# The-African-Research-Collective/karanta-ocr

Hardware: AMD Instinct MI355X
Metric: pages_per_sec (higher is better)
Workload: dtype bf16; 1 GPU; Qwen2-VL-2B bf16 greedy, batch=8 synthetic 1024x1024 pages per GPU, max_pixels=1003520 (grid 70x70, 1225 image tokens), prompt P=1394 tokens, T_out=1024 (ignore_eos), random-init weights; global_batch=8, parallelism=dp1, decode=hipGraph replay

## Files before the change

include/karanta_hip.h:

```cpp
#ifndef KARANTA_HIP_H
#define KARANTA_HIP_H

#include <stddef.h>
#include <stdint.h>

#ifdef __cplusplus
extern "C" {
#endif

typedef void* kr_stream;
typedef uint16_t kr_bf16;

#define KR_ABI_VERSION 412

#define KR_OK 0
#define KR_ERR_ARG (-1)
#define KR_ERR_HIP (-2)
#define KR_ERR_RCCL (-3)
#define KR_ERR_STATE (-4)

#define KR_EPI_NONE 0
#define KR_EPI_QUICK_GELU 1
#define KR_EPI_GELU_ERF 2
#define KR_EPI_SILU_MUL 3
#define KR_EPI_SILU_MUL8 4

int kr_version(void);
const char* kr_last_error(void);
int kr_device_info(int device, char* name64, int* compute_units, size_t* total_mem);
int kr_set_device(int device);
int kr_stream_synchronize(kr_stream s);
int kr_stream_create_cu_mask(kr_stream* out, int cus_enabled);
int kr_stream_create_cu_range(kr_stream* out, int first_cu, int n_cus);
int kr_stream_destroy(kr_stream s);

int kr_event_create(void** ev);
int kr_event_destroy(void* ev);
int kr_event_record(void* ev, kr_stream s);
int kr_stream_wait_event(kr_stream s, void* ev);
int kr_event_synchronize(void* ev);
int kr_event_elapsed_ms(void* start, void* stop, float* ms);

int kr_graph_begin_capture(kr_stream s);
int kr_graph_end_capture(kr_stream s, void** graph_exec);
int kr_graph_launch(void* graph_exec, kr_stream s);
int kr_graph_destroy(void* graph_exec);


int kr_cast_pad_f32_bf16(const float* src, kr_bf16* dst, int64_t rows, int k, int k_pad, kr_stream s);

int kr_layernorm(const kr_bf16* x, const kr_bf16* w, const kr_bf16* b, kr_bf16* y,
                 int64_t rows, int d, float eps, kr_stream s);

int kr_rmsnorm(const kr_bf16* x, int64_t ldx, const kr_bf16* w, kr_bf16* y,
               int64_t rows, int d, float eps, kr_stream s);


int kr_gemm_bf16(const kr_bf16* A, int64_t lda, const kr_bf16* W, const kr_bf16* bias,
                 const kr_bf16* residual, int64_t ldr, kr_bf16* C, int64_t ldc,
                 int64_t M, int N, int K, int epilogue, int w_packed, kr_stream s);

#define KR_GEMM_SCRATCH_BYTES ((size_t)512 * 65536)
int kr_gemm_bf16_ws(const kr_bf16* A, int64_t lda, const kr_bf16* W, const kr_bf16* bias,
                    const kr_bf16* residual, int64_t ldr, kr_bf16* C, int64_t ldc,
                    int64_t M, int N, int K, int epilogue, int w_packed, float* scratch, size_t scratch_bytes, kr_stream s);

int kr_gemm_fp8(const kr_bf16* A, int64_t lda, const uint8_t* w_packed_fp8, const float* w_scale, const kr_bf16* bias,
                const kr_bf16* residual, int64_t ldr, kr_bf16* C, int64_t ldc, int64_t M, int N, int K, int epilogue,
                kr_stream s);

int kr_quantize_rows_fp8(const kr_bf16* x, int64_t ldx, uint8_t* q, int64_t ldq, float* scale, int64_t rows, int K, kr_stream s);
int kr_gemm_fp8a(const uint8_t* A8, int64_t lda, const float* a_scale, const uint8_t* w_packed_fp8, const float* w_scale,
                 const kr_bf16* bias, const kr_bf16* residual, int64_t ldr, kr_bf16* C, int64_t ldc, int64_t M, int N, int K,
                 int epilogue, kr_stream s);

int kr_gemv_bf16(const kr_bf16* x, int64_t ldx, const kr_bf16* W, const kr_bf16* bias,
                 const kr_bf16* residual, int64_t ldr, kr_bf16* out, float* out_f32, int64_t ldc,
                 int M, int N, int K, int epilogue,
                 const kr_bf16* norm_w, float norm_eps, kr_stream s);


int kr_qkv_prep(const kr_bf16* qkv, int64_t ld_qkv, int q_off, int k_off, int v_off,
                const float* cos, const float* sin,
                const int32_t* blk_tok0, const int32_t* blk_ntok,
                const int64_t* blk_k_row0, const int64_t* blk_vt_blk, int n_blk,
                kr_bf16* q_out, int64_t q_head_stride, kr_bf16* k_out, int64_t k_head_stride,
                kr_bf16* vt_out, int64_t vt_head_stride, int q_heads, int kv_heads, int hd,
                kr_stream s);

int kr_rope2d_vision(kr_bf16* x, const float* cos, const float* sin, int64_t n, int heads, int hd,
                     int64_t row_stride, kr_stream s);

int kr_attn_varlen(const kr_bf16* q, const kr_bf16* k, const kr_bf16* vt, kr_bf16* out,
                   const int32_t* qblk, const int32_t* qblk_len, int n_qblk,
                   int64_t nq_total, int q_heads, int kv_heads, int hd,
                   int64_t k_head_stride, int64_t vt_head_stride, float scale, int causal,
                   kr_stream s);
int kr_attn_varlen_q(const kr_bf16* q, const kr_bf16* k, const kr_bf16* vt, kr_bf16* out,
                     const int32_t* qblk, const int32_t* qblk_len, int n_qblk,
                     int64_t nq_total, int q_heads, int kv_heads, int hd,
                     int64_t k_head_stride, int64_t vt_head_stride, float scale, int causal,
                     int q_block, kr_stream s);


int kr_embed_scatter(const int32_t* src, const kr_bf16* table, const kr_bf16* image_embeds,
                     kr_bf16* out, int64_t rows, int d, kr_stream s);


int kr_mrope(kr_bf16* x, const float* cos, const float* sin, int64_t n, int heads, int hd,
             int64_t row_stride, kr_stream s);
int kr_kv_append(const kr_bf16* k, const kr_bf16* v, int64_t row_stride,
                 const int32_t* tok_seq, const int32_t* tok_pos,
                 kr_bf16* kcache, kr_bf16* vtcache,
                 int64_t n, int kv_heads, int hd, int layer, int batch, int s_max, kr_stream s);

int kr_decode_qkv_prep(const kr_bf16* qkv, const float* inv_freq, const int32_t* ctx_len,
                       const int32_t* rope_delta, kr_bf16* q_out, kr_bf16* kcache, kr_bf16* vtcache,
                       int batch, int heads, int kv_heads, int hd, int layer, int s_max, kr_stream s);

int kr_attn_decode_gqa(const kr_bf16* q, const kr_bf16* kcache, const kr_bf16* vtcache,
                       const int32_t* ctx_len, kr_bf16* out, float* workspace,
                       int batch, int heads, int kv_heads, int hd, int layer, int s_max,
                       int n_split, float scale, kr_stream s);

int kr_argmax_embed(const float* logits, int64_t ld_logits, int vocab,
                    const kr_bf16* embed_table, int d,
                    int32_t* tokens_out, int32_t* history, int32_t* step_ptr, int32_t* ctx_len,
                    int32_t* finished, const int32_t* eos, int n_eos, int pad_id, int ignore_eos,
                    kr_bf16* x_next, int batch, int hist_stride, kr_stream s);

int kr_argmax(const float* logits, int64_t ld_logits, int vocab, int32_t* out, int batch, kr_stream s);

#define KR_DEC_PLAIN 0
#define KR_DEC_SILU 1
#define KR_DEC_ROPE_KV 2
#define KR_DEC_ARGMAX 3
#define KR_DEC_SILU8 4
#define KR_DEC_OUT_XP 0x100
int kr_linear_decode(int mode, const kr_bf16* x, int64_t ldx, const kr_bf16* w_packed, const kr_bf16* bias,
                     const kr_bf16* norm_w, float norm_eps, const kr_bf16* residual, int64_t ldr,
                     kr_bf16* out, float* out_f32, int64_t ldc, int M, int N, int K, int waves, int max_blocks, int ksplit,
                     float* ws, int32_t* counters, const float* attn_partials, int attn_split,
                     const float* cs_table, int cs_stride, const int32_t* prompt_len, const int32_t* ctx_len,
                     kr_bf16* q_out, kr_bf16* kcache, kr_bf16* vtcache, int heads, int kv_heads, int s_max,
                     float* amax_val, int32_t* amax_idx, kr_stream s);

int kr_linear_decode_wide(int mode, const kr_bf16* x, int64_t ldx, const kr_bf16* w_packed, const kr_bf16* bias,
                          const kr_bf16* norm_w, float norm_eps, const kr_bf16* residual, int64_t ldr,
                          kr_bf16* out, float* out_f32, int64_t ldc, int M, int N, int K, int blocks, int waves,
                          float* amax_val, int32_t* amax_idx, kr_stream s);

typedef struct kr_narrow_opts {
    float* zero_ptr;
    uint64_t zero_bytes;
    int32_t atomic_out;
    int32_t part_rows;
    int32_t w_resident;
} kr_narrow_opts;

int kr_linear_decode_narrow(int mode, const kr_bf16* x, int64_t ldx, const float* part_in, int n_part_in,
                            kr_bf16* x_out, int64_t ldxo, const kr_bf16* w_packed, const kr_bf16* bias,
                            const kr_bf16* norm_w, float norm_eps, const kr_bf16* residual, int64_t ldr,
                            kr_bf16* out, float* out_f32, int64_t ldc, int M, int N, int K, int waves, int ksplit,
                            const float* cs_table, int cs_stride, const int32_t* prompt_len, const int32_t* ctx_len,
                            kr_bf16* q_out, kr_bf16* kcache, kr_bf16* vtcache, int heads, int kv_heads, int s_max,
                            const kr_narrow_opts* opts, kr_stream s);

int kr_decode_resnorm(const kr_bf16* x, int64_t ldx, const float* part_in, int n_part_in, int part_rows, kr_bf16* x_out,
                      int64_t ldxo, const kr_bf16* norm_w, float norm_eps, kr_bf16* h, int64_t ldh, int M, int K, kr_stream s);

int kr_linear_decode_wide_fp8(int mode, const kr_bf16* x, int64_t ldx, const uint8_t* w_packed_fp8, const float* w_scale,
                              const kr_bf16* bias, const kr_bf16* norm_w, float norm_eps, const kr_bf16* residual,
                              int64_t ldr, kr_bf16* out, float* out_f32, int64_t ldc, int M, int N, int K, int blocks,
                              int waves, float* amax_val, int32_t* amax_idx, kr_stream s);
int kr_linear_decode_narrow_fp8(int mode, const kr_bf16* x, int64_t ldx, const float* part_in, int n_part_in,
                                kr_bf16* x_out, int64_t ldxo, const uint8_t* w_packed_fp8, const float* w_scale,
                                const kr_bf16* bias, const kr_bf16* norm_w, float norm_eps, const kr_bf16* residual,
                                int64_t ldr, kr_bf16* out, float* out_f32, int64_t ldc, int M, int N, int K, int waves,
                                int ksplit, const float* cs_table, int cs_stride, const int32_t* prompt_len,
                                const int32_t* ctx_len, kr_bf16* q_out, kr_bf16* kcache, kr_bf16* vtcache, int heads,
                                int kv_heads, int s_max, const kr_narrow_opts* opts, kr_stream s);
int kr_pack_rows32(const kr_bf16* x, int64_t ldx, int M, int K, kr_bf16* xp, kr_stream s);

typedef struct kr_dec32 {
    const kr_bf16* xp;
    const void* w_packed;
    const float* w_scale;
    const kr_bf16* bias;
    const kr_bf16* residual;
    int64_t ldr;
    kr_bf16* out;
    float* out_f32;
    int64_t ldc;
    int32_t M, N, K;
    int32_t waves_ref, ksplit;
    int32_t atomic_out;
    int32_t tiles_per_wg;
    int32_t group_split;
    int32_t reserved0;
    float* zero_ptr;
    uint64_t zero_bytes;
    const float* cs_table; int32_t cs_stride; const int32_t* prompt_len; const int32_t* ctx_len;
    kr_bf16* q_out; kr_bf16* kcache; kr_bf16* vtcache; int32_t heads, kv_heads, s_max;
} kr_dec32;
int kr_linear_decode32(int mode, const kr_dec32* args, kr_stream s);

int kr_decode_resnorm32(const kr_bf16* x, int64_t ldx, const float* part_in, int n_part_in, int part_rows, kr_bf16* x_out,
                        int64_t ldxo, const kr_bf16* norm_w, float norm_eps, kr_bf16* h_xp, int M, int K, int sum_slabs_first,
                        kr_stream s);

int kr_fp8_to_bf16(const uint8_t* src, kr_bf16* dst, int64_t n, kr_stream s);

int kr_attn_decode_fused(const kr_bf16* q, const kr_bf16* kcache, const kr_bf16* vtcache,
                         const int32_t* ctx_len, kr_bf16* out, float* workspace, int32_t* counters,
                         int batch, int heads, int kv_heads, int hd, int s_max, int n_split,
                         float scale, kr_stream s);
int kr_attn_decode_slots(const kr_bf16* q, const kr_bf16* kcache, const kr_bf16* vtcache, const int32_t* ctx_len,
                         const int32_t* finished, float* workspace, int batch, int heads, int kv_heads, int hd, int s_max,
                         int n_split, float scale, kr_stream s);

int kr_attn_decode_merge(const float* workspace, kr_bf16* out, int batch, int heads, int hd, int n_split,
                         kr_stream s);

int kr_attn_decode_merge32(const float* workspace, kr_bf16* out_xp, int batch, int heads, int hd, int n_split,
                           kr_stream s);

int kr_image_resize_bicubic_u8(const uint8_t* src, int h, int w, uint8_t* dst, int rh, int rw, uint8_t* tmp,
                               const int32_t* h_bounds, const int32_t* h_coeffs, int h_ksize,
                               const int32_t* v_bounds, const int32_t* v_coeffs, int v_ksize, kr_stream s);
int kr_image_normalize_patchify(const uint8_t* img, int rh, int rw, const float* mean3, const float* std3,
                                int patch, int merge, int temporal, float* out, kr_stream s);

int kr_gumbel_argmax(const float* logits, int64_t ld_logits, int vocab, const float* temperature,
                     const uint32_t* seed, const int32_t* ctx_len, const int32_t* prompt_len, float* amax_val,
                     int32_t* amax_idx, int n_part, int batch, kr_stream s);

int kr_guide_build_masks(const uint16_t* trans, const uint8_t* accept, int n_states, const int32_t* vocab_off,
                         const uint8_t* vocab_bytes, int vocab, const int32_t* eos, int n_eos, uint32_t* masks,
                         int mask_words, kr_stream s);

int kr_gumbel_argmax_guided(const float* logits, int64_t ld_logits, int vocab, const float* temperature,
                            const uint32_t* seed, const int32_t* ctx_len, const int32_t* prompt_len, float* amax_val,
                            int32_t* amax_idx, int n_part, int batch, const uint64_t* guide_masks,
                            const int32_t* guide_state, int mask_words, int fallback_token, kr_stream s);

int kr_sample_threshold(const float* logits, int64_t ld_logits, int vocab, const float* temperature, const float* params,
                        const int32_t* counts, int64_t ld_counts, const uint32_t* prompt_bits, int bits_words,
                        const uint64_t* guide_masks, const int32_t* guide_state, int mask_words, const int32_t* finished,
                        int ignore_eos, float* work, int64_t ld_work, uint32_t* threshold, int32_t* live, int batch,
                        kr_stream s);

int kr_gumbel_argmax_processed(const float* logits, int64_t ld_logits, int vocab, const float* temperature,
                               const uint32_t* seed, const int32_t* ctx_len, const int32_t* prompt_len, float* amax_val,
                               int32_t* amax_idx, int n_part, int batch, const uint64_t* guide_masks,
                               const int32_t* guide_state, int mask_words, int fallback_token, const float* params,
                               const int32_t* counts, int64_t ld_counts, const uint32_t* prompt_bits, int bits_words,
                               const uint32_t* threshold, kr_stream s);

int kr_sample_count(const int32_t* tokens, const int32_t* live, int32_t* counts, int64_t ld_counts, int vocab, int batch,
                    kr_stream s);

int kr_sample_threshold_rows(const float* logits, int64_t ld_logits, int vocab, const float* temperature, const float* params,
                             const int32_t* counts, int64_t ld_counts, const uint32_t* prompt_bits, int bits_words,
                             const uint64_t* guide_masks, const int32_t* guide_state, int mask_words, const int32_t* finished,
                             int ignore_eos, float* work, int64_t ld_work, uint32_t* threshold, int32_t* live, int batch,
                             const int32_t* row_slot, const int32_t* depth, const int32_t* draft_tok, int k, int slots, kr_stream s);
int kr_gumbel_argmax_processed_rows(const float* logits, int64_t ld_logits, int vocab, const float* temperature,
                                    const uint32_t* seed, const int32_t* ctx_len, const int32_t* prompt_len, float* amax_val,
                                    int32_t* amax_idx, int n_part, int batch, const uint64_t* guide_masks,
                                    const int32_t* guide_state, int mask_words, int fallback_token, const float* params,
                                    const int32_t* counts, int64_t ld_counts, const uint32_t* prompt_bits, int bits_words,
                                    const uint32_t* threshold, const int32_t* row_slot, const int32_t* depth,
                                    const int32_t* draft_tok, int k, int slots, kr_stream s);

#define KR_ADJ_CAP 320
int kr_logits_adjust(float* logits, int64_t ld_logits, int vocab, const int32_t* adj_ids, const float* adj_val,
                     const int32_t* adj_flag, const int32_t* adj_meta, const int32_t* ctx_len, const int32_t* prompt_len,
                     float* saved, int batch, kr_stream s);

int kr_logits_adjust_rows(float* logits, int64_t ld_logits, int vocab, const int32_t* adj_ids, const float* adj_val,
                          const int32_t* adj_flag, const int32_t* adj_meta, const int32_t* ctx_len, const int32_t* prompt_len,
                          float* saved, int batch, const int32_t* row_slot, int slots, kr_stream s);

int kr_logits_restore(float* logits, int64_t ld_logits, int vocab, const int32_t* adj_ids, const int32_t* adj_meta,
                      const float* saved, int batch, kr_stream s);

int kr_stop_tokens(const int32_t* tokens, const int32_t* adj_ids, const int32_t* adj_flag, const int32_t* adj_meta,
                   int32_t* finished, int ignore_eos, int batch, kr_stream s);

int kr_guide_advance(const int32_t* tokens, const int32_t* finished, const uint64_t* guide_trans, int32_t* guide_state,
                     const int32_t* vocab_off, const uint8_t* vocab_bytes, int vocab, int batch, kr_stream s);

int kr_logprobs_topk(const float* logits, int64_t ld_logits, int vocab, int k, int n_part, float* part_val,
                     int32_t* part_idx, float* part_ms, const int32_t* tokens, const int32_t* ctx_len,
                     const int32_t* prompt_len, const int32_t* finished, float* out_lp, int32_t* out_idx, int hist_len,
                     int hist_batch, int k_stride, int batch, kr_stream s);

#define KR_FORK_MAX_GROUPS 32
#define KR_FORK_MAX_SLOTS 32
typedef struct kr_fork_group {
    int32_t src;
    int32_t n_tokens;
    int32_t n_dst;
    int32_t dst[KR_FORK_MAX_SLOTS];
} kr_fork_group;
typedef struct kr_fork_plan {
    int32_t n_groups;
// ... 160 lines not shown
```

karanta_ocr_amd/_lib.py:

```python
from __future__ import annotations

import ctypes as C
import os
from typing import Optional

_HERE = os.path.dirname(os.path.abspath(__file__))
LIB_PATH = os.path.join(_HERE, "libkaranta_hip.so")

c_p = C.c_void_p
i32, i64, f32 = C.c_int, C.c_int64, C.c_float


class KarantaHipError(RuntimeError):
    pass


SIGNATURES = {
    "kr_version": [],
    "kr_last_error": [],
    "kr_device_info": [i32, C.c_char_p, C.POINTER(i32), C.POINTER(C.c_size_t)],
    "kr_set_device": [i32],
    "kr_stream_synchronize": [c_p],
    "kr_stream_create_cu_mask": [C.POINTER(c_p), i32],
    "kr_stream_create_cu_range": [C.POINTER(c_p), i32, i32],
    "kr_stream_destroy": [c_p],
    "kr_event_create": [C.POINTER(c_p)],
    "kr_event_destroy": [c_p],
    "kr_event_record": [c_p, c_p],
    "kr_event_synchronize": [c_p],
    "kr_stream_wait_event": [c_p, c_p],
    "kr_event_elapsed_ms": [c_p, c_p, C.POINTER(f32)],
    "kr_graph_begin_capture": [c_p],
    "kr_graph_end_capture": [c_p, C.POINTER(c_p)],
    "kr_graph_launch": [c_p, c_p],
    "kr_graph_destroy": [c_p],
    "kr_cast_pad_f32_bf16": [c_p, c_p, i64, i32, i32, c_p],
    "kr_layernorm": [c_p, c_p, c_p, c_p, i64, i32, f32, c_p],
    "kr_rmsnorm": [c_p, i64, c_p, c_p, i64, i32, f32, c_p],
    "kr_gemm_bf16": [c_p, i64, c_p, c_p, c_p, i64, c_p, i64, i64, i32, i32, i32, i32, c_p],
    "kr_decode_resnorm": [c_p, i64, c_p, i32, i32, c_p, i64, c_p, f32, c_p, i64, i32, i32, c_p],
    "kr_decode_resnorm32": [c_p, i64, c_p, i32, i32, c_p, i64, c_p, f32, c_p, i32, i32, i32, c_p],
    "kr_pack_rows32": [c_p, i64, i32, i32, c_p, c_p],
    "kr_linear_decode32": [i32, c_p, c_p],
    "kr_attn_decode_merge32": [c_p, c_p, i32, i32, i32, i32, c_p],
    "kr_quantize_rows_fp8": [c_p, i64, c_p, i64, c_p, i64, i32, c_p],
    "kr_gemm_fp8a": [c_p, i64, c_p, c_p, c_p, c_p, c_p, i64, c_p, i64, i64, i32, i32, i32, c_p],
    "kr_gemm_bf16_ws": [c_p, i64, c_p, c_p, c_p, i64, c_p, i64, i64, i32, i32, i32, i32, c_p, C.c_size_t, c_p],
    "kr_gemv_bf16": [c_p, i64, c_p, c_p, c_p, i64, c_p, c_p, i64, i32, i32, i32, i32, c_p, f32, c_p],
    "kr_qkv_prep": [c_p, i64, i32, i32, i32, c_p, c_p, c_p, c_p, c_p, c_p, i32, c_p, i64, c_p, i64, c_p, i64,
                    i32, i32, i32, c_p],
    "kr_rope2d_vision": [c_p, c_p, c_p, i64, i32, i32, i64, c_p],
    "kr_attn_varlen": [c_p, c_p, c_p, c_p, c_p, c_p, i32, i64, i32, i32, i32, i64, i64, f32, i32, c_p],
    "kr_attn_varlen_q": [c_p, c_p, c_p, c_p, c_p, c_p, i32, i64, i32, i32, i32, i64, i64, f32, i32, i32, c_p],
    "kr_embed_scatter": [c_p, c_p, c_p, c_p, i64, i32, c_p],
    "kr_mrope": [c_p, c_p, c_p, i64, i32, i32, i64, c_p],
    "kr_kv_append": [c_p, c_p, i64, c_p, c_p, c_p, c_p, i64, i32, i32, i32, i32, i32, c_p],
    "kr_decode_qkv_prep": [c_p, c_p, c_p, c_p, c_p, c_p, c_p, i32, i32, i32, i32, i32, i32, c_p],
    "kr_attn_decode_gqa": [c_p, c_p, c_p, c_p, c_p, c_p, i32, i32, i32, i32, i32, i32, i32, f32, c_p],
    "kr_argmax_embed": [c_p, i64, i32, c_p, i32, c_p, c_p, c_p, c_p, c_p, c_p, i32, i32, i32, c_p, i32, i32, c_p],
    "kr_argmax": [c_p, i64, i32, c_p, i32, c_p],
    "kr_linear_decode": [i32, c_p, i64, c_p, c_p, c_p, f32, c_p, i64, c_p, c_p, i64, i32, i32, i32, i32, i32, i32, c_p, c_p,
                         c_p, i32, c_p, i32, c_p, c_p, c_p, c_p, c_p, i32, i32, i32, c_p, c_p, c_p],
    "kr_linear_decode_wide": [i32, c_p, i64, c_p, c_p, c_p, f32, c_p, i64, c_p, c_p, i64, i32, i32, i32, i32, i32, c_p, c_p, c_p],
    "kr_image_resize_bicubic_u8": [c_p, i32, i32, c_p, i32, i32, c_p, c_p, c_p, i32, c_p, c_p, i32, c_p],
    "kr_image_normalize_patchify": [c_p, i32, i32, c_p, c_p, i32, i32, i32, c_p, c_p],
    "kr_linear_decode_wide_fp8": [i32, c_p, i64, c_p, c_p, c_p, c_p, f32, c_p, i64, c_p, c_p, i64, i32, i32, i32, i32, i32, c_p, c_p, c_p],
    "kr_linear_decode_narrow_fp8": [i32, c_p, i64, c_p, i32, c_p, i64, c_p, c_p, c_p, c_p, f32, c_p, i64, c_p, c_p, i64,
                                    i32, i32, i32, i32, i32, c_p, i32, c_p, c_p, c_p, c_p, c_p, i32, i32, i32, c_p, c_p],
    "kr_fp8_to_bf16": [c_p, c_p, i64, c_p],
    "kr_gemm_fp8": [c_p, i64, c_p, c_p, c_p, c_p, i64, c_p, i64, i64, i32, i32, i32, c_p],
    "kr_gumbel_argmax": [c_p, i64, i32, c_p, c_p, c_p, c_p, c_p, c_p, i32, i32, c_p],
    "kr_gumbel_argmax_guided": [c_p, i64, i32, c_p, c_p, c_p, c_p, c_p, c_p, i32, i32, c_p, c_p, i32, i32, c_p],
    "kr_guide_build_masks": [c_p, c_p, i32, c_p, c_p, i32, c_p, i32, c_p, i32, c_p],
    "kr_sample_threshold": [c_p, i64, i32, c_p, c_p, c_p, i64, c_p, i32, c_p, c_p, i32, c_p, i32, c_p, i64, c_p, c_p, i32, c_p],
    "kr_gumbel_argmax_processed": [c_p, i64, i32, c_p, c_p, c_p, c_p, c_p, c_p, i32, i32, c_p, c_p, i32, i32, c_p, c_p, i64, c_p,
                                   i32, c_p, c_p],
    "kr_sample_threshold_rows": [c_p, i64, i32, c_p, c_p, c_p, i64, c_p, i32, c_p, c_p, i32, c_p, i32, c_p, i64, c_p, c_p, i32, c_p, c_p,
                                 c_p, i32, i32, c_p],
    "kr_gumbel_argmax_processed_rows": [c_p, i64, i32, c_p, c_p, c_p, c_p, c_p, c_p, i32, i32, c_p, c_p, i32, i32, c_p, c_p, i64, c_p,
                                        i32, c_p, c_p, c_p, c_p, i32, i32, c_p],
    "kr_sample_count": [c_p, c_p, c_p, i64, i32, i32, c_p],
    "kr_logits_adjust": [c_p, i64, i32, c_p, c_p, c_p, c_p, c_p, c_p, c_p, i32, c_p],
    "kr_logits_adjust_rows": [c_p, i64, i32, c_p, c_p, c_p, c_p, c_p, c_p, c_p, i32, c_p, i32, c_p],
    "kr_logits_restore": [c_p, i64, i32, c_p, c_p, c_p, i32, c_p],
    "kr_stop_tokens": [c_p, c_p, c_p, c_p, c_p, i32, i32, c_p],
    "kr_guide_advance": [c_p, c_p, c_p, c_p, c_p, c_p, i32, i32, c_p],
    "kr_kv_fork": [c_p, c_p, i64, i64, i64, i64, i64, i64, i32, i32, i32, i32, i32, c_p, c_p],
    "kr_logprobs_topk": [c_p, i64, i32, i32, i32, c_p, c_p, c_p, c_p, c_p, c_p, c_p, c_p, c_p, i32, i32, i32, i32, c_p],
    "kr_linear_decode_narrow": [i32, c_p, i64, c_p, i32, c_p, i64, c_p, c_p, c_p, f32, c_p, i64, c_p, c_p, i64,
                                i32, i32, i32, i32, i32, c_p, i32, c_p, c_p, c_p, c_p, c_p, i32, i32, i32, c_p, c_p],
    "kr_attn_decode_fused": [c_p, c_p, c_p, c_p, c_p, c_p, c_p, i32, i32, i32, i32, i32, i32, f32, c_p],
    "kr_attn_decode_slots": [c_p, c_p, c_p, c_p, c_p, c_p, i32, i32, i32, i32, i32, i32, f32, c_p],
    "kr_attn_decode_merge": [c_p, c_p, i32, i32, i32, i32, c_p],
    "kr_sample_greedy": [c_p, c_p, i32, c_p, i32, c_p, c_p, i32, c_p, c_p, c_p, c_p, i32, i32, i32, c_p, i32, c_p],
    "kr_spec_propose": [c_p, c_p],
    "kr_spec_accept": [c_p, c_p, c_p, i32, c_p, c_p, i32, i32, c_p],
    "kr_spec_lookup": [c_p, c_p, c_p],
    "kr_spec_deal": [c_p, c_p, c_p, c_p],
    "kr_spec_accept_rows": [c_p, c_p, c_p, c_p, i32, c_p, c_p, i32, i32, c_p],
    "kr_spec_guide_trim": [c_p, c_p, c_p, c_p],
    "kr_spec_guide_rows": [c_p, c_p, c_p, c_p],
    "kr_spec_guide_advance": [c_p, c_p, c_p],
    "kr_spec_controls_trim": [c_p, c_p, c_p, c_p],
    "kr_spec_controls_rows": [c_p, c_p, c_p, c_p],
    "kr_spec_controls_count": [c_p, c_p, c_p],
    "kr_repeat_detect": [c_p, c_p],
    "kr_linear_decode32_rows": [i32, c_p, c_p, c_p],
    "kr_attn_decode_rows": [c_p, c_p, c_p, c_p, c_p, c_p, c_p, i32, i32, i32, i32, i32, i32, f32, c_p],
    "kr_kv_quantize": [c_p, c_p, c_p, i32, i32, i32, i32, c_p, c_p, c_p],
    "kr_kv_absmax": [c_p, c_p, i32, i32, i32, i32, c_p, f32, f32, c_p, c_p, c_p],
    "kr_kv_fork8": [c_p, c_p, i64, i64, i64, i64, i64, i64, i32, i32, i32, i32, i32, c_p, c_p],
    "kr_attn_decode_slots_kv8": [c_p, c_p, c_p, c_p, c_p, i32, i32, i32, i32, i32, i32, f32, c_p],
    "kr_attn_decode_rows_kv8": [c_p, c_p, c_p, c_p, c_p, c_p, i32, i32, i32, i32, i32, i32, f32, c_p],
    "kr_linear_decode_narrow_kv8": [c_p, i64, c_p, i32, c_p, i64, c_p, c_p, c_p, c_p, f32, i32, i32, i32, i32, c_p, i32, c_p, c_p,
                                    c_p, c_p, i32, i32, i32, c_p, c_p],
    "kr_linear_decode32_kv8": [c_p, c_p, c_p, c_p],
    "kr_comm_unique_id": [c_p],
    "kr_comm_init": [C.POINTER(c_p), i32, i32, c_p],
    "kr_comm_count": [c_p, C.POINTER(i32)],
    "kr_comm_destroy": [c_p],
    "kr_rccl_version": [C.POINTER(i32)],
    "kr_bcast_weights": [c_p, c_p, C.c_size_t, i32, c_p],
    "kr_selftest_mfma": [c_p],
    "kr_probe_launch_floor": [c_p, i32, i32, i32, C.POINTER(f32)],
    "kr_probe_stream_read": [c_p, C.c_size_t, i32, i32, c_p, C.POINTER(f32)],
    "kr_launch_null": [c_p],
}
_RESTYPES = {"kr_last_error": C.c_char_p}

EXPERIMENT_SIGNATURES = {
    "kr_linear_decode_narrow_x32": [i32, c_p, i64, c_p, i32, c_p, i64, c_p, i64, c_p, c_p, c_p, c_p, f32, c_p, i64, c_p, c_p, i64,
                                    i32, i32, i32, i32, i32, c_p, i32, c_p, c_p, c_p, c_p, c_p, i32, i32, i32, c_p,
                                    c_p, C.c_size_t, i32, c_p],
    "kr_oproj_heads": [c_p, i32, c_p, c_p, c_p, i64, i32, i32, i32, c_p],
    "kr_linear_decode_wide_x32": [i32, c_p, i64, c_p, i64, c_p, c_p, c_p, f32, c_p, c_p, i64, i32, i32, i32, i32, i32, c_p, c_p, c_p],
    "kr_prefetch": [c_p, C.c_size_t, i32, c_p],
}


class NarrowOpts(C.Structure):
    _fields_ = [("zero_ptr", c_p), ("zero_bytes", C.c_uint64), ("atomic_out", C.c_int32), ("part_rows", C.c_int32),
                ("w_resident", C.c_int32)]


def narrow_opts(zero_ptr: int = 0, zero_bytes: int = 0, atomic_out: bool = False, part_rows: int = 0, w_resident: bool = False):
    if not (zero_bytes or atomic_out or part_rows or w_resident):
        return None
    return C.byref(NarrowOpts(zero_ptr or None, int(zero_bytes), 1 if atomic_out else 0, int(part_rows), 1 if w_resident else 0))

class Dec32(C.Structure):
    _fields_ = [("xp", c_p), ("w_packed", c_p), ("w_scale", c_p), ("bias", c_p), ("residual", c_p), ("ldr", C.c_int64),
                ("out", c_p), ("out_f32", c_p), ("ldc", C.c_int64), ("M", C.c_int32), ("N", C.c_int32), ("K", C.c_int32),
                ("waves_ref", C.c_int32), ("ksplit", C.c_int32), ("atomic_out", C.c_int32), ("tiles_per_wg", C.c_int32),
                ("group_split", C.c_int32), ("reserved0", C.c_int32), ("zero_ptr", c_p), ("zero_bytes", C.c_uint64),
                ("cs_table", c_p), ("cs_stride", C.c_int32), ("prompt_len", c_p), ("ctx_len", c_p),
                ("q_out", c_p), ("kcache", c_p), ("vtcache", c_p), ("heads", C.c_int32), ("kv_heads", C.c_int32), ("s_max", C.c_int32)]


class Spec(C.Structure):
    _fields_ = [("slots", C.c_int32), ("k", C.c_int32), ("rows", C.c_int32), ("ngram_min", C.c_int32), ("ngram_max", C.c_int32),
                ("s_max", C.c_int32), ("prompt_ids", c_p), ("prompt_stride", C.c_int64), ("history", c_p), ("hist_stride", C.c_int32),
                ("hist_rows", C.c_int32), ("script", c_p), ("script_len", c_p), ("row_slot", c_p), ("ctx_len", c_p),
                ("prompt_len", c_p), ("finished", c_p), ("temperature", c_p), ("seed", c_p), ("n_draft", c_p), ("draft_tok", c_p),
                ("embed_table", c_p), ("d", C.c_int32), ("pad_id", C.c_int32), ("vocab", C.c_int32), ("x", c_p), ("ldx", C.c_int64),
                ("proposed", c_p), ("accepted", c_p)]


class SpecGuide(C.Structure):
    _fields_ = [("guide_trans", c_p), ("guide_masks", c_p), ("guide_state", c_p), ("mask_words", C.c_int32), ("vocab_off", c_p),
                ("vocab_bytes", c_p), ("draft_state", c_p), ("ctx_before", c_p)]


class SpecControls(C.Structure):
    _fields_ = [("adj_ids", c_p), ("adj_flag", c_p), ("adj_meta", c_p), ("counts", c_p), ("ld_counts", C.c_int64), ("depth", c_p),
                ("ctx_before", c_p)]


REP_MAX_PERIOD = 1024


class Repeat(C.Structure):
    _fields_ = [("slots", C.c_int32), ("history", c_p), ("hist_stride", C.c_int32), ("hist_rows", C.c_int32), ("ctx_len", c_p),
                ("prompt_len", c_p), ("finished", c_p), ("cfg", c_p), ("run", c_p), ("seen", c_p), ("rep_at", c_p),
                ("flags", C.c_int32)]


class Kv8(C.Structure):
    _fields_ = [("k", c_p), ("vt", c_p), ("scale", c_p)]


def kv8(k: int, vt: int, scale: int):
    return C.byref(Kv8(k, vt, scale))


KVQ_MAX_ROWS = 32


class KvqPlan(C.Structure):
    _fields_ = [("n", C.c_int32), ("slot", C.c_int32 * KVQ_MAX_ROWS), ("len", C.c_int32 * KVQ_MAX_ROWS)]


def kvq_plan(rows):
    p = KvqPlan()
    p.n = len(rows) if len(rows) <= KVQ_MAX_ROWS else -1
    for i, (slot, n) in enumerate(list(rows)[:KVQ_MAX_ROWS]):
        p.slot[i], p.len[i] = int(slot), int(n)
    return C.byref(p)


FORK_MAX_GROUPS = FORK_MAX_SLOTS = 32


class ForkGroup(C.Structure):
    _fields_ = [("src", C.c_int32), ("n_tokens", C.c_int32), ("n_dst", C.c_int32), ("dst", C.c_int32 * FORK_MAX_SLOTS)]


class ForkPlan(C.Structure):
    _fields_ = [("n_groups", C.c_int32), ("groups", ForkGroup * FORK_MAX_GROUPS)]


def fork_plan(groups):
    p = ForkPlan()
    p.n_groups = len(groups) if len(groups) <= FORK_MAX_GROUPS else -1
    for g, (src, n_tokens, dst) in zip(p.groups, groups):
        g.src, g.n_tokens = int(src), int(n_tokens)
        g.n_dst = len(dst) if len(dst) <= FORK_MAX_SLOTS else -1
        for i, j in enumerate(list(dst)[:FORK_MAX_SLOTS]):
            g.dst[i] = int(j)
    return C.byref(p)


ABI_MAJOR = 4
DEC_OUT_XP = 0x100
ADJ_CAP = 320
EPI_NONE, EPI_QUICK_GELU, EPI_GELU_ERF, EPI_SILU_MUL, EPI_SILU_MUL8 = 0, 1, 2, 3, 4
DEC_PLAIN, DEC_SILU, DEC_ROPE_KV, DEC_ARGMAX, DEC_SILU8 = 0, 1, 2, 3, 4


class _Lib:
    def __init__(self, path: str):
        if not os.path.exists(path):
            raise KarantaHipError(
                f"{path} not found: build it with `python -m karanta_ocr_amd.build` "
                "(the MI355X engine has no CPU fallback)")
        import torch

        try:
            self._dll = C.CDLL(path, mode=C.RTLD_GLOBAL)
        except OSError as e:
            raise KarantaHipError(f"cannot load {path}: {e}") from e
        self.path = path
        for name, argtypes in SIGNATURES.items():
            try:
                fn = getattr(self._dll, name)
            except AttributeError as e:
                raise KarantaHipError(f"{path} does not export {name}") from e
            fn.argtypes = argtypes
            fn.restype = _RESTYPES.get(name, C.c_int)
            if name in ("kr_version", "kr_last_error"):
                setattr(self, name, fn)
            else:
                setattr(self, name, self._checked(name, fn))
        if self.kr_version() // 100 != ABI_MAJOR:
            raise KarantaHipError(f"{path} reports kr_version() = {self.kr_version()}, this binding is written against ABI major "
                                  f"{ABI_MAJOR} (include/karanta_hip.h): rebuild with `python -m karanta_ocr_amd.build`")
        self.experiments = hasattr(self._dll, "kr_oproj_heads")
        for name, argtypes in EXPERIMENT_SIGNATURES.items():
            if self.experiments:
                fn = getattr(self._dll, name)
                fn.argtypes, fn.restype = argtypes, C.c_int
                setattr(self, name, self._checked(name, fn))
            else:
                setattr(self, name, self._absent(name))

    @staticmethod
    def _absent(name):
        def call(*_):
            raise KarantaHipError(f"{name} is an experiment entry point (include/karanta_hip_experiments.h): this library was built "
                                  "without -DKR_EXPERIMENTS (csrc/tools/build_variant.py; load it through KARANTA_HIP_LIB)")
        call.__name__ = name
        return call

    def _checked(self, name, fn):
        def call(*args):
            rc = fn(*args)
            if rc != 0:
                msg = self._dll.kr_last_error()
                raise KarantaHipError(f"{name} -> {rc}: {msg.decode() if msg else ''}")
            return rc

        call.__name__ = name
        call.raw = fn
        return call


_LIB: Optional[_Lib] = None


def lib() -> _Lib:
    global _LIB
    if _LIB is None:
        _LIB = _Lib(os.environ.get("KARANTA_HIP_LIB", LIB_PATH))
    return _LIB


def ptr(t) -> int:
    return 0 if t is None else t.data_ptr()
```

karanta_ocr_amd/csrc/kr_attn_decode.hip:

```cpp
#include "kr_decode_common.h"

namespace {

#ifndef KR_ATTN_DEC_LD
#define KR_ATTN_DEC_LD ld8_nt
#endif
template <bool KV8> struct KvElem { using T = kr_bf16; };
template <> struct KvElem<true> { using T = uint8_t; };

template <int WAVES, bool ROWS = false, bool KV8 = false>
__global__ void __launch_bounds__(WAVES * 64) attn_decode2_kernel(const kr_bf16* __restrict__ q, const typename KvElem<KV8>::T* __restrict__ kcache,
                                                                  const typename KvElem<KV8>::T* __restrict__ vtcache,
                                                                  const int32_t* __restrict__ ctx_len,
                                                                  const int32_t* __restrict__ finished, int heads, int kv_heads,
                                                                  int group, int n_split, int s_max, float scale_log2e,
                                                                  kr_bf16* __restrict__ out, float* __restrict__ ws,
                                                                  int* __restrict__ counters, int ws_bytes,
                                                                  const int32_t* __restrict__ row_slot,
                                                                  const float* __restrict__ kv_scale) {
    constexpr int HD = 128, DT = HD / 16, REC = HD + 4;
    __shared__ __attribute__((aligned(16))) float o_s[WAVES][16][HD];
    __shared__ float m_s[WAVES][16], l_s[WAVES][16];
    __shared__ int last_s;
    const int tid = threadIdx.x, lane = tid & 63, wave = __builtin_amdgcn_readfirstlane(tid >> 6);
// ... 190 lines not shown
            }
        }
    }
    auto store_out = [&](int t, const f32x4& a, float l) {
        const float inv = l > 0.f ? 1.0f / l : 0.f;
        bf16x4 ov;
#pragma unroll
        for (int j = 0; j < 4; ++j) ov[j] = f2bf(a[j] * inv);
        *reinterpret_cast<bf16x4*>(out + (int64_t)(bh0 + (t >> 5)) * HD + ((t & 31) << 2)) = ov;
    };
    auto rec_of = [&](int t) { return ((int64_t)(bh0 + (t >> 5)) * n_split) * REC; };
    if (n_split == 1 && out) {
#pragma unroll
        for (int it = 0; it < IT; ++it)
            if (tid + it * NTHR < nq) store_out(tid + it * NTHR, acc4[it], ll[it]);
        return;
    }
    if (!KR_EXP || !out) {
#pragma unroll
        for (int it = 0; it < IT; ++it) {
            const int t = tid + it * NTHR, d4 = (t & 31) << 2;
            if (t < nq) {
                float* w = ws + rec_of(t) + (int64_t)split * REC;
                *reinterpret_cast<f32x4*>(w + d4) = acc4[it];
                if (d4 == 0) *reinterpret_cast<f32x4*>(w + HD) = (f32x4){mm[it], ll[it], 0.f, 0.f};
            }
        }
        return;
    }
    const auto rsrc = __builtin_amdgcn_make_buffer_rsrc(ws, 0, ws_bytes, 0x00020000);
#pragma unroll
    for (int it = 0; it < IT; ++it) {
        const int t = tid + it * NTHR, d4 = (t & 31) << 2;
        if (t < nq) {
            const int off = (int)((rec_of(t) + (int64_t)split * REC + d4) * 4);
            __builtin_amdgcn_raw_buffer_store_b128(__builtin_bit_cast(u32x4, acc4[it]), rsrc, off, 0, 16);
            if (d4 == 0)
                __builtin_amdgcn_raw_buffer_store_b128(__builtin_bit_cast(u32x4, (f32x4){mm[it], ll[it], 0.f, 0.f}), rsrc,
                                                       (int)((rec_of(t) + (int64_t)split * REC + HD) * 4), 0, 16);
        }
    }
    asm volatile("s_waitcnt vmcnt(0)" ::: "memory");
    __syncthreads();
    if (tid == 0) {
        const int old = __hip_atomic_fetch_add(counters + b * kv_heads + kvh, 1, __ATOMIC_RELAXED, __HIP_MEMORY_SCOPE_AGENT);
        last_s = (old == n_split - 1);
        if (old == n_split - 1) __hip_atomic_store(counters + b * kv_heads + kvh, 0, __ATOMIC_RELAXED, __HIP_MEMORY_SCOPE_AGENT);
    }
    __syncthreads();
    if (!last_s) return;
    constexpr int MAXS = 16;
    for (int it = 0; it < IT; ++it) {
        const int t = tid + it * NTHR, d4 = (t & 31) << 2;
        if (t >= nq) continue;
        u32x4 ro[MAXS], rm[MAXS];
#pragma unroll
        for (int p = 0; p < MAXS; ++p) {
            if (p < n_split) {
                ro[p] = __builtin_amdgcn_raw_buffer_load_b128(rsrc, (int)((rec_of(t) + (int64_t)p * REC + d4) * 4), 0, 16);
                rm[p] = __builtin_amdgcn_raw_buffer_load_b128(rsrc, (int)((rec_of(t) + (int64_t)p * REC + HD) * 4), 0, 16);
            }
        }
        float mt = -1e30f;
#pragma unroll
        for (int p = 0; p < MAXS; ++p)
            if (p < n_split) mt = fmaxf(mt, __builtin_bit_cast(f32x4, rm[p])[0]);
        f32x4 at = {0.f, 0.f, 0.f, 0.f};
        float lt = 0.f;
#pragma unroll
        for (int p = 0; p < MAXS; ++p) {
            if (p < n_split) {
                const f32x4 mlp = __builtin_bit_cast(f32x4, rm[p]), op = __builtin_bit_cast(f32x4, ro[p]);
                const float sc = __builtin_amdgcn_exp2f(mlp[0] - mt);
#pragma unroll
                for (int j = 0; j < 4; ++j) at[j] += op[j] * sc;
                lt += mlp[1] * sc;
            }
        }
        store_out(t, at, lt);
    }
}

template <int NS>
__global__ void __launch_bounds__(128) attn_merge_kernel(const float* __restrict__ ws, kr_bf16* __restrict__ out, int n_split, int heads_xp) {
    constexpr int HD = 128, REC = HD + 4;
    const int bh = blockIdx.x, d = threadIdx.x;
    float acc = 0.f, ll = 0.f;
    if constexpr (NS > 0) {
        const float* w = ws + (int64_t)bh * NS * REC;
        float m[NS], l[NS], o[NS];
#pragma unroll
        for (int p = 0; p < NS; ++p) {
            m[p] = w[p * REC + HD];
            l[p] = w[p * REC + HD + 1];
            o[p] = w[p * REC + d];
        }
        float mm = -1e30f;
#pragma unroll
        for (int p = 0; p < NS; ++p) mm = fmaxf(mm, m[p]);
#pragma unroll
        for (int p = 0; p < NS; ++p) {
            const float sc = __builtin_amdgcn_exp2f(m[p] - mm);
            acc += o[p] * sc;
            ll += l[p] * sc;
        }
    } else {
        const float* w = ws + (int64_t)bh * n_split * REC;
        float mm = -1e30f;
        for (int p = 0; p < n_split; ++p) mm = fmaxf(mm, w[p * REC + HD]);
        for (int p = 0; p < n_split; ++p) {
            const float sc = __builtin_amdgcn_exp2f(w[p * REC + HD] - mm);
            acc += w[p * REC + d] * sc;
            ll += w[p * REC + HD + 1] * sc;
        }
    }
    const kr_bf16 r = __builtin_bit_cast(kr_bf16, f2bf(ll > 0.f ? acc / ll : 0.f));
    if (heads_xp > 0) {
        const int b = bh / heads_xp, hh = bh - b * heads_xp;
        *reinterpret_cast<kr_bf16*>(reinterpret_cast<char*>(out) + kr_xp_byte_offset(b, hh * HD + d)) = r;
    } else {
        out[(int64_t)bh * HD + d] = r;
    }
}

}

template <bool ROWS = false, bool KV8 = false>
static int attn_decode_impl(const kr_bf16* q, const typename KvElem<KV8>::T* kcache, const typename KvElem<KV8>::T* vtcache,
                            const int32_t* ctx_len, const int32_t* finished, kr_bf16* out, float* workspace, int32_t* counters,
                            int batch, int heads, int kv_heads, int hd, int s_max, int n_split, float scale, kr_stream s,
                            const int32_t* row_slot = nullptr, const float* kv_scale = nullptr) {
    KR_CHECK_ARG(q && kcache && vtcache && ctx_len && (out || workspace), "kr_attn_decode_fused: null pointer");
    KR_CHECK_ARG(hd == 128, "kr_attn_decode_fused: hd=%d (only 128)", hd);
    KR_CHECK_ARG(heads % kv_heads == 0 && heads / kv_heads <= 16, "kr_attn_decode_fused: GQA group must be <= 16");
    KR_CHECK_ARG(batch > 0 && n_split > 0 && s_max % 64 == 0, "kr_attn_decode_fused: bad sizes");
    KR_CHECK_ARG(KR_EXP || !out || n_split == 1,
                 "kr_attn_decode_fused: the in-launch merge (out != NULL with n_split > 1) is an experiment build (-DKR_EXPERIMENTS); "
                 "pass out = NULL and run kr_attn_decode_merge");
    KR_CHECK_ARG(!out || n_split <= 16, "kr_attn_decode_fused: the in-launch merge takes at most 16 splits");
    KR_CHECK_ARG(!out || n_split == 1 || (workspace && counters), "kr_attn_decode_fused: split needs workspace + counters");
    KR_CHECK_ARG(workspace || n_split == 1, "kr_attn_decode_fused: the split partials need a workspace");
    static const int waves_env = [] { const char* e = getenv("KARANTA_ATTN_WAVES"); return e ? atoi(e) : 0; }();
    const int waves = waves_env ? waves_env : (n_split <= 8 ? 8 : n_split <= 16 ? 4 : 2);
    KR_CHECK_ARG(waves == 2 || waves == 4 || waves == 8, "kr_attn_decode_fused: KARANTA_ATTN_WAVES=%d (2, 4 or 8)", waves);
    const int64_t ws_bytes = (int64_t)batch * heads * n_split * (hd + 4) * 4;
    KR_CHECK_ARG(ws_bytes < ((int64_t)1 << 31), "kr_attn_decode_fused: workspace of %lld bytes", (long long)ws_bytes);
    const dim3 grid(n_split, kv_heads, batch);
    const float sl2 = scale * 1.4426950408889634f;
    const int group = heads / kv_heads;
    if (waves == 8)
        attn_decode2_kernel<8, ROWS, KV8><<<grid, 512, 0, kr_hs(s)>>>(q, kcache, vtcache, ctx_len, finished, heads, kv_heads, group, n_split, s_max,
                                                                      sl2, out, workspace, counters, (int)ws_bytes, row_slot, kv_scale);
    else if (waves == 4)
        attn_decode2_kernel<4, ROWS, KV8><<<grid, 256, 0, kr_hs(s)>>>(q, kcache, vtcache, ctx_len, finished, heads, kv_heads, group, n_split, s_max,
                                                                      sl2, out, workspace, counters, (int)ws_bytes, row_slot, kv_scale);
    else
        attn_decode2_kernel<2, ROWS, KV8><<<grid, 128, 0, kr_hs(s)>>>(q, kcache, vtcache, ctx_len, finished, heads, kv_heads, group, n_split, s_max,
                                                                      sl2, out, workspace, counters, (int)ws_bytes, row_slot, kv_scale);
    KR_CHECK_LAUNCH();
    return KR_OK;
}

extern "C" int kr_attn_decode_fused(const kr_bf16* q, const kr_bf16* kcache, const kr_bf16* vtcache, const int32_t* ctx_len,
                                    kr_bf16* out, float* workspace, int32_t* counters, int batch, int heads, int kv_heads,
                                    int hd, int s_max, int n_split, float scale, kr_stream s) {
    return attn_decode_impl(q, kcache, vtcache, ctx_len, nullptr, out, workspace, counters, batch, heads, kv_heads, hd, s_max, n_split, scale, s);
}

extern "C" int kr_attn_decode_slots(const kr_bf16* q, const kr_bf16* kcache, const kr_bf16* vtcache, const int32_t* ctx_len,
                                    const int32_t* finished, float* workspace, int batch, int heads, int kv_heads, int hd, int s_max,
                                    int n_split, float scale, kr_stream s) {
    KR_CHECK_ARG(finished && workspace, "kr_attn_decode_slots: null pointer");
    return attn_decode_impl(q, kcache, vtcache, ctx_len, finished, nullptr, workspace, nullptr, batch, heads, kv_heads, hd, s_max, n_split, scale, s);
}

extern "C" int kr_attn_decode_rows(const kr_bf16* q, const kr_bf16* kcache, const kr_bf16* vtcache, const int32_t* ctx_len,
                                   const int32_t* finished, const int32_t* row_slot, float* workspace, int rows, int heads, int kv_heads,
                                   int hd, int s_max, int n_split, float scale, kr_stream s) {
    KR_CHECK_ARG(finished && workspace && row_slot, "kr_attn_decode_rows: null pointer");
    return attn_decode_impl<true>(q, kcache, vtcache, ctx_len, finished, nullptr, workspace, nullptr, rows, heads, kv_heads, hd, s_max, n_split,
                                  scale, s, row_slot);
}

extern "C" int kr_attn_decode_slots_kv8(const kr_bf16* q, const kr_kv8* kv, const int32_t* ctx_len, const int32_t* finished,
                                        float* workspace, int batch, int heads, int kv_heads, int hd, int s_max, int n_split,
                                        float scale, kr_stream s) {
    KR_CHECK_ARG(finished && workspace && kv && kv->k && kv->vt && kv->scale, "kr_attn_decode_slots_kv8: null pointer");
    KR_CHECK_ARG((((uintptr_t)kv->k | (uintptr_t)kv->vt) & 15) == 0, "kr_attn_decode_slots_kv8: the cache must be 16-byte aligned");
    return attn_decode_impl<false, true>(q, kv->k, kv->vt, ctx_len, finished, nullptr, workspace, nullptr, batch, heads, kv_heads, hd,
                                         s_max, n_split, scale, s, nullptr, kv->scale);
}

extern "C" int kr_attn_decode_rows_kv8(const kr_bf16* q, const kr_kv8* kv, const int32_t* ctx_len, const int32_t* finished,
                                       const int32_t* row_slot, float* workspace, int rows, int heads, int kv_heads, int hd,
                                       int s_max, int n_split, float scale, kr_stream s) {
    KR_CHECK_ARG(finished && workspace && row_slot && kv && kv->k && kv->vt && kv->scale, "kr_attn_decode_rows_kv8: null pointer");
    KR_CHECK_ARG((((uintptr_t)kv->k | (uintptr_t)kv->vt) & 15) == 0, "kr_attn_decode_rows_kv8: the cache must be 16-byte aligned");
    return attn_decode_impl<true, true>(q, kv->k, kv->vt, ctx_len, finished, nullptr, workspace, nullptr, rows, heads, kv_heads, hd,
                                        s_max, n_split, scale, s, row_slot, kv->scale);
}

static int merge_impl(const float* workspace, kr_bf16* out, int batch, int heads, int hd, int n_split, int xp, kr_stream s) {
    KR_CHECK_ARG(workspace && out && batch > 0 && heads > 0 && n_split > 0, "kr_attn_decode_merge: bad args");
    KR_CHECK_ARG(hd == 128, "kr_attn_decode_merge: hd=%d (only 128)", hd);
    KR_CHECK_ARG(!xp || (batch <= 32 && ((uintptr_t)out & 15) == 0), "kr_attn_decode_merge32: batch=%d (<= 32)", batch);
    const int hx = xp ? heads : 0;
    switch (n_split) {
        case 4: attn_merge_kernel<4><<<batch * heads, 128, 0, kr_hs(s)>>>(workspace, out, n_split, hx); break;
        case 8: attn_merge_kernel<8><<<batch * heads, 128, 0, kr_hs(s)>>>(workspace, out, n_split, hx); break;
        case 16: attn_merge_kernel<16><<<batch * heads, 128, 0, kr_hs(s)>>>(workspace, out, n_split, hx); break;
        case 32: attn_merge_kernel<32><<<batch * heads, 128, 0, kr_hs(s)>>>(workspace, out, n_split, hx); break;
        default: attn_merge_kernel<0><<<batch * heads, 128, 0, kr_hs(s)>>>(workspace, out, n_split, hx);
    }
    KR_CHECK_LAUNCH();
    return KR_OK;
}

extern "C" int kr_attn_decode_merge(const float* workspace, kr_bf16* out, int batch, int heads, int hd, int n_split,
                                    kr_stream s) {
    return merge_impl(workspace, out, batch, heads, hd, n_split, 0, s);
}

extern "C" int kr_attn_decode_merge32(const float* workspace, kr_bf16* out_xp, int batch, int heads, int hd, int n_split,
                                      kr_stream s) {
    return merge_impl(workspace, out_xp, batch, heads, hd, n_split, 1, s);
}

namespace {

__global__ void __launch_bounds__(256) decode_qkv_prep_kernel(const kr_bf16* __restrict__ qkv,
                                                              const float* __restrict__ inv_freq,
                                                              const int32_t* __restrict__ ctx_len,
                                                              const int32_t* __restrict__ rope_delta,
                                                              kr_bf16* __restrict__ q_out, kr_bf16* __restrict__ kcache,
                                                              kr_bf16* __restrict__ vtcache, int heads, int kv_heads,
                                                              int hd, int layer, int batch, int s_max) {
    const int b = blockIdx.x;
    const int pos = ctx_len[b];
    const float rp = (float)(pos + rope_delta[b]);
    const int half = hd >> 1;
    const int qkv_dim = (heads + 2 * kv_heads) * hd;
    const kr_bf16* row = qkv + (int64_t)b * qkv_dim;
    const int64_t kv_base = ((int64_t)layer * batch + b) * kv_heads;
    for (int e = threadIdx.x; e < (heads + kv_heads) * half; e += blockDim.x) {
        const int h = e / half, i = e - h * half;
        const float ang = rp * inv_freq[i];
        const float c = bfround(cosf(ang)), s = bfround(sinf(ang));
        const float x0 = bfbits2f(row[h * hd + i]), x1 = bfbits2f(row[h * hd + i + half]);
        const __bf16 y0 = f2bf(x0 * c - x1 * s), y1 = f2bf(x1 * c + x0 * s);
        kr_bf16* dst;
        if (h < heads) {
            dst = q_out + ((int64_t)b * heads + h) * hd;
        } else {
            dst = kcache + ((kv_base + (h - heads)) * s_max + pos) * hd;
        }
        dst[i] = __builtin_bit_cast(kr_bf16, y0);
        dst[i + half] = __builtin_bit_cast(kr_bf16, y1);
    }
    const kr_bf16* vrow = row + (heads + kv_heads) * hd;
    for (int e = threadIdx.x; e < kv_heads * hd; e += blockDim.x) {
        const int h = e / hd, d = e - h * hd;
        vtcache[((kv_base + h) * (s_max >> 6) + (pos >> 6)) * (hd * 64) + kr_vt_off(d, pos & 63, hd)] = vrow[e];
    }
}

template <int HD>
__global__ void __launch_bounds__(256) attn_decode_kernel(const kr_bf16* __restrict__ q, const kr_bf16* __restrict__ kcache,
                                                          const kr_bf16* __restrict__ vtcache,
                                                          const int32_t* __restrict__ ctx_len, float* __restrict__ ws,
                                                          int heads, int kv_heads, int layer, int batch, int s_max,
                                                          float scale_log2e) {
    constexpr int DT = HD / 16;
    const int lane = threadIdx.x & 63, wave = threadIdx.x >> 6;
    const int fr = lane & 15, fg = lane >> 4;
    const int kvh = blockIdx.y, b = blockIdx.z;
    const int group = heads / kv_heads;
    const int n_part = gridDim.x * 4;
    const int part = blockIdx.x * 4 + wave;
    const int ctx = ctx_len[b] + 1;
    const int nb = (ctx + 63) >> 6;

    const int g = fr < group ? fr : 0;
    const kr_bf16* qp = q + ((int64_t)b * heads + kvh * group + g) * HD + fg * 32;
    bf16x8 qf[4];
#pragma unroll
    for (int i = 0; i < 4; ++i) qf[i] = ld8(qp + i * 8);

    const int64_t kv_base = ((int64_t)layer * batch + b) * kv_heads + kvh;
    const kr_bf16* kc = kcache + kv_base * s_max * HD;
    const kr_bf16* vc = vtcache + kv_base * (int64_t)(s_max >> 6) * (HD * 64);

    f32x4 o[DT];
#pragma unroll
    for (int t = 0; t < DT; ++t) o[t] = (f32x4){0.f, 0.f, 0.f, 0.f};
    float m_run = -1e30f, l_run = 0.f;

    for (int blk = part; blk < nb; blk += n_part) {
#pragma unroll
        for (int hf = 0; hf < 2; ++hf) {
            const int key0 = blk * 64 + hf * 32;
            if (key0 >= ctx) break;
            bf16x8 kf[2][4];
#pragma unroll
            for (int kt = 0; kt < 2; ++kt) {
                const kr_bf16* kp = kc + (int64_t)(key0 + 8 * (fr >> 2) + 4 * kt + (fr & 3)) * HD + fg * 32;
#pragma unroll
                for (int i = 0; i < 4; ++i) kf[kt][i] = ld8_nt(kp + i * 8);
            }
// ... 134 lines not shown
```

karanta_ocr_amd/csrc/kr_common.h:

```cpp
#pragma once
#include <hip/hip_runtime.h>
#include <stdint.h>
#include <stdio.h>

#include "../../include/karanta_hip.h"
#ifdef KR_EXPERIMENTS
#include "../../include/karanta_hip_experiments.h"
#endif

typedef __attribute__((ext_vector_type(8))) __bf16 bf16x8;
typedef __attribute__((ext_vector_type(4))) __bf16 bf16x4;
typedef __attribute__((ext_vector_type(2))) __bf16 bf16x2;
typedef __attribute__((ext_vector_type(4))) float f32x4;
typedef __attribute__((ext_vector_type(8))) float f32x8;
typedef __attribute__((ext_vector_type(16))) float f32x16;
typedef __attribute__((ext_vector_type(4))) unsigned int u32x4;
typedef __attribute__((ext_vector_type(2))) unsigned int u32x2;

#define KR_WAVE 64

void kr_set_error(const char* fmt, ...);

#define KR_CHECK_ARG(cond, ...)                 \
    do {                                        \
        if (!(cond)) {                          \
            kr_set_error(__VA_ARGS__);          \
            return KR_ERR_ARG;                  \
        }                                       \
    } while (0)

#define KR_CHECK_HIP(expr)                                                              \
    do {                                                                                \
        hipError_t _e = (expr);                                                         \
        if (_e != hipSuccess) {                                                         \
            kr_set_error("%s failed: %s (%s:%d)", #expr, hipGetErrorString(_e), __FILE__, __LINE__); \
            return KR_ERR_HIP;                                                          \
        }                                                                               \
    } while (0)

#define KR_CHECK_LAUNCH()                                                               \
    do {                                                                                \
        hipError_t _e = hipGetLastError();                                              \
        if (_e != hipSuccess) {                                                         \
            kr_set_error("kernel launch failed: %s (%s:%d)", hipGetErrorString(_e), __FILE__, __LINE__); \
            return KR_ERR_HIP;                                                          \
        }                                                                               \
    } while (0)

static inline hipStream_t kr_hs(kr_stream s) { return reinterpret_cast<hipStream_t>(s); }

#define KR_MAX_DEVICES 64
struct KrPerDeviceOnce {
    bool done[KR_MAX_DEVICES] = {};
    bool need() {
        int dev = 0;
        if (hipGetDevice(&dev) != hipSuccess || dev < 0 || dev >= KR_MAX_DEVICES) return true;
        if (done[dev]) return false;
        done[dev] = true;
        return true;
    }
};

__device__ __forceinline__ float bf2f(__bf16 v) { return (float)v; }
__device__ __forceinline__ __bf16 f2bf(float v) { return (__bf16)v; }
__device__ __forceinline__ float bfbits2f(unsigned short b) { return __uint_as_float(((unsigned int)b) << 16); }
__device__ __forceinline__ float bfround(float v) { return (float)((__bf16)v); }

__device__ __forceinline__ bf16x8 ld8(const kr_bf16* p) { return *reinterpret_cast<const bf16x8*>(p); }
__device__ __forceinline__ void st8(kr_bf16* p, bf16x8 v) { *reinterpret_cast<bf16x8*>(p) = v; }
__device__ __forceinline__ bf16x8 ld8_nt(const kr_bf16* p) {
    return __builtin_nontemporal_load(reinterpret_cast<const bf16x8*>(p));
}

__host__ __device__ __forceinline__ int64_t kr_xp_byte_offset(int b, int k) {
    return (int64_t)(k >> 6) * 4096 + (b >> 4) * 2048 + ((k >> 5) & 1) * 1024 + ((((k >> 3) & 3) * 16 + (b & 15)) * 16) + (k & 7) * 2;
}

__host__ __device__ __forceinline__ int kr_vt_off(int d, int key, int hd) { return ((key >> 5) * hd + d) * 32 + (key & 31); }

__device__ __forceinline__ float wave_sum(float v) {
#pragma unroll
    for (int o = 32; o > 0; o >>= 1) v += __shfl_xor(v, o, 64);
    return v;
}
__device__ __forceinline__ float wave_max(float v) {
#pragma unroll
    for (int o = 32; o > 0; o >>= 1) v = fmaxf(v, __shfl_xor(v, o, 64));
    return v;
}

__device__ __forceinline__ float act_quick_gelu(float x) { return x * __builtin_amdgcn_rcpf(1.0f + __expf(-1.702f * x)); }
__device__ __forceinline__ float act_gelu_erf(float x) { return 0.5f * x * (1.0f + erff(x * 0.70710678118654752f)); }
__device__ __forceinline__ float act_silu(float x) { return x * __builtin_amdgcn_rcpf(1.0f + __expf(-x)); }

__device__ __forceinline__ unsigned xcd_remap(unsigned bid, unsigned nwg) {
    const unsigned q = nwg >> 3, r = nwg & 7u, xcd = bid & 7u;
    const unsigned base = xcd < r ? xcd * (q + 1) : r * (q + 1) + (xcd - r) * q;
    return base + (bid >> 3);
}
```

karanta_ocr_amd/csrc/kr_decode.hip:

```cpp
#include "kr_decode_common.h"

namespace {

struct DecLinArgs {
    const kr_bf16* x; int64_t ldx;
    const kr_bf16* wp;
    const kr_bf16* bias;
    const kr_bf16* norm_w; float norm_eps;
    const kr_bf16* residual; int64_t ldr;
    kr_bf16* out; float* out_f32; int64_t ldc;
    int M, N, K, ksplit;
    int groups;
    float* ws; int* counters;
    const float* attn_ws; int attn_split;
    int xmode;
    const float* cs_table;
    const int32_t* prompt_len; int cs_stride;
    const int32_t* ctx_len;
    kr_bf16* q_out; kr_bf16* kcache; kr_bf16* vtcache;
    int heads, kv_heads, s_max;
    float* amax_val; int32_t* amax_idx;
    int wide_blocks, wide_waves;
    const float* part_in; kr_bf16* x_out; int64_t ldxo;
    const float* w_scale;
    float* x_out_f32; int64_t ldxf;
    kr_bf16* wide_x_out; int64_t wide_ldxo;
    int x_is_f32;
    const char* pf_ptr; int64_t pf_bytes; int pf_blocks;
    int part_rows;
    int n_part;
    int part_atomic;
    float* zero_ptr; int zero_n16;
    int w_resident;
    int out_xp;
    Kv8 kv8;
};

template <int NT, int EPI, int WAVES>
__global__ void __launch_bounds__(WAVES * 64) dec_linear_kernel(const DecLinArgs a) {
    extern __shared__ __attribute__((aligned(16))) char smem[];
    constexpr int U = (WAVES == 16 ? 4 : 8) / NT;
    constexpr int NTHR = WAVES * 64;
    const int tid = threadIdx.x, lane = tid & 63;
    const int wave = __builtin_amdgcn_readfirstlane(tid >> 6);
    const int fr = lane & 15, fg = lane >> 4;
    const int ks = blockIdx.y;
    const int M = a.M, K = a.K;
    const int nchunks = K >> 6, ntiles = a.N >> 4;
    const int cpb = (nchunks + a.ksplit - 1) / a.ksplit;
    const int cb0 = min(ks * cpb, nchunks), cb1 = min(cb0 + cpb, nchunks);
    const int nblk = cb1 - cb0;
    const int per = (nblk + WAVES - 1) / WAVES;
    const int c0 = min(cb0 + wave * per, cb1), c1 = min(c0 + per, cb1);

    int tile[NT];
    const kr_bf16* wp[NT];
    bf16x8 wbuf[U][NT][2];
    auto set_item = [&](int g) {
        if (EPI == DEPI_ROPE_KV) {
            tile[0] = (g >> 2) * 8 + (g & 3);
            tile[NT - 1] = tile[0] + 4;
        } else {
#pragma unroll
            for (int t = 0; t < NT; ++t) tile[t] = g * NT + t;
        }
#pragma unroll
        for (int t = 0; t < NT; ++t) {
            const int tt = tile[t] < ntiles ? tile[t] : ntiles - 1;
            wp[t] = a.wp + ((int64_t)tt * nchunks) * 1024 + lane * 8;
        }
#pragma unroll
        for (int u = 0; u < U; ++u) {
            const int c = c0 + u;
            if (c < c1) {
#pragma unroll
                for (int t = 0; t < NT; ++t) {
                    wbuf[u][t][0] = ld8_nt(wp[t] + (int64_t)c * 1024);
                    wbuf[u][t][1] = ld8_nt(wp[t] + (int64_t)c * 1024 + 512);
                }
            }
        }
    };
    int g = blockIdx.x;
    set_item(g);

    const bool xlds = a.xmode != 0;
    const int xrow = nblk * 128 + 16;
    float* red = reinterpret_cast<float*>(smem + (xlds ? ((M * xrow + 127) & ~127) : 0));
    if (a.xmode == 2) {
        const int kc = K >> 3;
        for (int b = wave; b < M; b += WAVES) {
            bf16x8 v[8];
            float ss = 0.f;
#pragma unroll
            for (int i = 0; i < 8; ++i) {
                const int c = lane + i * 64;
                if (c < kc) {
                    v[i] = ld8(a.x + (int64_t)b * a.ldx + c * 8);
#pragma unroll
                    for (int j = 0; j < 8; ++j) ss += bf2f(v[i][j]) * bf2f(v[i][j]);
                }
            }
            ss = wave_sum(ss);
            const float rs = rsqrtf(ss / (float)K + a.norm_eps);
#pragma unroll
            for (int i = 0; i < 8; ++i) {
                const int c = lane + i * 64;
                if (c < kc && c >= cb0 * 8 && c < cb1 * 8) {
                    const bf16x8 nw = ld8(a.norm_w + c * 8);
                    bf16x8 o;
#pragma unroll
                    for (int j = 0; j < 8; ++j) o[j] = f2bf(bf2f(nw[j]) * bfround(bf2f(v[i][j]) * rs));
                    *reinterpret_cast<bf16x8*>(smem + b * xrow + (c - cb0 * 8) * 16) = o;
                }
            }
        }
        __syncthreads();
// ... 393 lines not shown
        ss = wave_sum(ss);
        const float rs = h.norm_w ? rsqrtf(ss / (float)K + h.norm_eps) : 1.f;
#pragma unroll
        for (int i = 0; i < RL; ++i) {
            const int c = lane + i * 64;
            if (c < kc) {
                bf16x8 o = v[i];
                if (h.norm_w) {
                    const bf16x8 nw = ld8(h.norm_w + c * 8);
#pragma unroll
                    for (int j = 0; j < 8; ++j) o[j] = f2bf(bf2f(nw[j]) * bfround(bf2f(v[i][j]) * rs));
                }
                *reinterpret_cast<bf16x8*>(smem + b * xrow + c * 16) = o;
            }
        }
    }
    __syncthreads();
    if (!ACTIVE) {
        if (EPI == DEPI_ARGMAX && fg == 0) {
#pragma unroll
            for (int mt = 0; mt < MT; ++mt) {
                const int b = fr + 16 * mt;
                if (b < M) {
                    a.amax_val[(int64_t)b * stride + t] = -INFINITY;
                    a.amax_idx[(int64_t)b * stride + t] = 0x7fffffff;
                }
            }
        }
        return;
    }
    const char* xl[MT];
#pragma unroll
    for (int mt = 0; mt < MT; ++mt) xl[mt] = smem + min(fr + 16 * mt, M - 1) * xrow;
    const int pidx = t;
    float rbv[MT];
    int rbi[MT];
#pragma unroll
    for (int mt = 0; mt < MT; ++mt) {
        rbv[mt] = -INFINITY;
        rbi[mt] = 0x7fffffff;
    }

    for (; t < ntiles; t += stride) {
        const int tn = t + stride;
        const bool more = tn < ntiles;
        const char* wpn = wbase + ((int64_t)(more ? tn : t) * nchunks) * WC::BYTES;
        f32x4 acc[MT];
#pragma unroll
        for (int mt = 0; mt < MT; ++mt) acc[mt] = (f32x4){0.f, 0.f, 0.f, 0.f};
        for (int cc = 0; cc < nchunks; cc += U) {
#pragma unroll
            for (int u = 0; u < U; ++u) {
                const int c = cc + u;
                if ((u & (MT == 1 ? 3 : 1)) == 0) __builtin_amdgcn_sched_barrier(0);
                const bf16x8 w0 = wbuf[u].frag(0), w1 = wbuf[u].frag(1);
#pragma unroll
                for (int mt = 0; mt < MT; ++mt) {
                    const bf16x8 x0 = *reinterpret_cast<const bf16x8*>(xl[mt] + c * 128 + WC::x_byte(0, fg));
                    const bf16x8 x1 = *reinterpret_cast<const bf16x8*>(xl[mt] + c * 128 + WC::x_byte(1, fg));
                    acc[mt] = __builtin_amdgcn_mfma_f32_16x16x32_bf16(w0, x0, acc[mt], 0, 0, 0);
                    acc[mt] = __builtin_amdgcn_mfma_f32_16x16x32_bf16(w1, x1, acc[mt], 0, 0, 0);
                }
                const int cn = c + U;
                if (cn < nchunks) {
                    wbuf[u].load(wp, cn);
                } else if (more) {
                    wbuf[u].load(wpn, cn - nchunks);
                }
            }
        }
        wp = wpn;
#pragma unroll
        for (int mt = 0; mt < MT; ++mt) {
            const int b = fr + 16 * mt;
            apply_w_scale(a.w_scale, t * 16 + fg * 4, acc[mt]);
            if (EPI == DEPI_SILU8) {
                float u4[4];
#pragma unroll
                for (int j = 0; j < 4; ++j) u4[j] = __shfl_xor(acc[mt][j], 32, 64);
                if (b < M && fg < 2) {
                    bf16x4 o;
#pragma unroll
                    for (int j = 0; j < 4; ++j) o[j] = f2bf(act_silu(acc[mt][j]) * u4[j]);
                    if (MT == 2 && a.out_xp)
                        *reinterpret_cast<bf16x4*>(reinterpret_cast<char*>(a.out) + kr_xp_byte_offset(b, t * 8 + fg * 4)) = o;
                    else
                        *reinterpret_cast<bf16x4*>(a.out + (int64_t)b * a.ldc + t * 8 + fg * 4) = o;
                }
            } else if (EPI == DEPI_ARGMAX) {
                const int n = t * 16 + fg * 4;
#pragma unroll
                for (int j = 0; j < 4; ++j) better(rbv[mt], rbi[mt], acc[mt][j], n + j);
                if (a.out_f32 && b < M) *reinterpret_cast<f32x4*>(a.out_f32 + (int64_t)b * a.ldc + n) = acc[mt];
            } else if (b < M) {
                const int n = t * 16 + fg * 4;
                float v[4];
#pragma unroll
                for (int j = 0; j < 4; ++j) v[j] = acc[mt][j];
                if (a.bias) {
                    const bf16x4 bv = *reinterpret_cast<const bf16x4*>(a.bias + n);
#pragma unroll
                    for (int j = 0; j < 4; ++j) v[j] += bf2f(bv[j]);
                }
                if (a.residual) {
                    const bf16x4 rv = *reinterpret_cast<const bf16x4*>(a.residual + (int64_t)b * a.ldr + n);
#pragma unroll
                    for (int j = 0; j < 4; ++j) v[j] += bf2f(rv[j]);
                }
                if (a.out_f32) {
                    *reinterpret_cast<f32x4*>(a.out_f32 + (int64_t)b * a.ldc + n) = (f32x4){v[0], v[1], v[2], v[3]};
                } else {
                    bf16x4 o;
#pragma unroll
                    for (int j = 0; j < 4; ++j) o[j] = f2bf(v[j]);
                    *reinterpret_cast<bf16x4*>(a.out + (int64_t)b * a.ldc + n) = o;
                }
            }
        }
    }
    if (EPI == DEPI_ARGMAX) {
#pragma unroll
        for (int mt = 0; mt < MT; ++mt) {
            const int b = fr + 16 * mt;
#pragma unroll
            for (int o = 16; o < 64; o <<= 1) {
                const float ov = __shfl_xor(rbv[mt], o, 64);
                const int oi = __shfl_xor(rbi[mt], o, 64);
                better(rbv[mt], rbi[mt], ov, oi);
            }
            if (fg == 0 && b < M) {
                a.amax_val[(int64_t)b * stride + pidx] = rbv[mt];
                a.amax_idx[(int64_t)b * stride + pidx] = rbi[mt];
            }
        }
    }
}

template <int EPI, int NCH, bool W8, int MT, bool XF32>
__global__ void __launch_bounds__(512) dec_wide_kernel(const kr_bf16* x, const kr_bf16* wp, const kr_bf16* norm_w, int64_t ldx, int M,
                                                       int N, int wide_blocks, int wide_waves, float norm_eps, const DecLinArgs a) {
    extern __shared__ __attribute__((aligned(16))) char smem[];
    const WideHot h{x, wp, norm_w, ldx, M, N, wide_blocks, wide_waves, norm_eps};
    const int wave = __builtin_amdgcn_readfirstlane(threadIdx.x >> 6);
    if ((int)blockIdx.x + wide_blocks * wave < (N >> 4)) dec_wide_body<EPI, NCH, true, W8, MT, XF32>(h, a, smem);
    else dec_wide_body<EPI, NCH, false, W8, MT, XF32>(h, a, smem);
}

template <int EPI, int NCH, bool W8, int MT, bool XF32>
int launch_wide_x(DecLinArgs& a, int blocks, int waves, kr_stream s) {
    const size_t lds = (size_t)a.M * (a.K * 2 + 16);
    KR_CHECK_ARG(lds <= 160 * 1024, "kr_linear_decode_wide: x (%d rows, K=%d) needs %zu bytes of LDS", a.M, a.K, lds);
    auto fn = &dec_wide_kernel<EPI, NCH, W8, MT, XF32>;
    static KrPerDeviceOnce attr;
    if (attr.need()) {
        KR_CHECK_HIP(hipFuncSetAttribute(reinterpret_cast<const void*>(fn), hipFuncAttributeMaxDynamicSharedMemorySize, 160 * 1024));
    }
    fn<<<blocks, waves * 64, lds, kr_hs(s)>>>(a.x, a.wp, a.norm_w, a.ldx, a.M, a.N, a.wide_blocks, a.wide_waves, a.norm_eps, a);
    KR_CHECK_LAUNCH();
    return KR_OK;
}

template <int EPI, int NCH, bool W8, int MT>
int launch_wide_m(DecLinArgs& a, int blocks, int waves, kr_stream s) {
    if (a.x_is_f32) {
        if constexpr (KR_EXP && (EPI == DEPI_SILU8 || EPI == DEPI_ARGMAX)) {
            return launch_wide_x<EPI, NCH, W8, MT, true>(a, blocks, waves, s);
        } else {
            kr_set_error("kr_linear_decode_wide: f32 x rows (experiment builds: SILU8 and ARGMAX modes only)");
// ... 176 lines not shown
                        *reinterpret_cast<bf16x4*>(reinterpret_cast<char*>(a.out) + kr_xp_byte_offset(b, t * 8 + fg * 4)) = o;
                    else
                        *reinterpret_cast<bf16x4*>(a.out + (int64_t)b * a.ldc + t * 8 + fg * 4) = o;
                }
            } else {
                const int n = t * 16 + fg * 4;
#pragma unroll
                for (int j = 0; j < 4; ++j) better(rbv[mt], rbi[mt], acc[i][mt][j], n + j);
                if (a.out_f32 && b < M) *reinterpret_cast<f32x4*>(a.out_f32 + (int64_t)b * a.ldc + n) = acc[i][mt];
            }
        }
    }
    if (EPI == DEPI_ARGMAX) {
#pragma unroll
        for (int mt = 0; mt < MT; ++mt) {
            const int b = fr + 16 * mt;
#pragma unroll
            for (int o = 16; o < 64; o <<= 1) {
                const float ov = __shfl_xor(rbv[mt], o, 64);
                const int oi = __shfl_xor(rbi[mt], o, 64);
                better(rbv[mt], rbi[mt], ov, oi);
            }
            if (fg == 0 && b < M) {
                a.amax_val[(int64_t)b * stride + t0] = rbv[mt];
                a.amax_idx[(int64_t)b * stride + t0] = rbi[mt];
            }
        }
    }
}

template <int EPI, bool W8>
int launch_wide_kh(DecLinArgs& a, int blocks, int waves, kr_stream s) {
    if constexpr (EPI == DEPI_SILU8 || EPI == DEPI_ARGMAX) {
        KR_CHECK_ARG(waves == 8, "kr_linear_decode_wide: 17..32 rows at K = 3584 run 8 waves per workgroup (got %d)", waves);
        const int tiles_per_wave = ((a.N >> 4) + blocks * waves - 1) / (blocks * waves);
        KR_CHECK_ARG(tiles_per_wave <= 5, "kr_linear_decode_wide: %d tiles over %d x %d waves is more than 5 tiles per wave", a.N >> 4,
                     blocks, waves);
        KR_CHECK_ARG(!a.x_is_f32 && !a.bias && !a.residual, "kr_linear_decode_wide: K-halves take bf16 x, no bias / residual");
        const size_t lds = (size_t)32 * (28 * 64 * 2 + 16);
        auto fn = tiles_per_wave <= 2 ? &dec_wide_kh_kernel<EPI, W8, true> : &dec_wide_kh_kernel<EPI, W8, false>;
        static KrPerDeviceOnce attr;
        if (attr.need()) {
            KR_CHECK_HIP(hipFuncSetAttribute(reinterpret_cast<const void*>(&dec_wide_kh_kernel<EPI, W8, true>),
                                             hipFuncAttributeMaxDynamicSharedMemorySize, 160 * 1024));
            KR_CHECK_HIP(hipFuncSetAttribute(reinterpret_cast<const void*>(&dec_wide_kh_kernel<EPI, W8, false>),
                                             hipFuncAttributeMaxDynamicSharedMemorySize, 160 * 1024));
        }
        fn<<<blocks, 512, lds, kr_hs(s)>>>(a.x, a.wp, a.norm_w, a.ldx, a.M, a.N, a.wide_blocks, a.wide_waves, a.norm_eps, a);
        KR_CHECK_LAUNCH();
        return KR_OK;
    } else {
        kr_set_error("kr_linear_decode_wide: M=%d > 16 at K = 3584 is built for the SILU8 and ARGMAX modes", a.M);
        return KR_ERR_ARG;
    }
}

template <int EPI, int NCH, bool W8>
int launch_wide_w(DecLinArgs& a, int blocks, int waves, kr_stream s) {
    if (a.M > 16) {
        if constexpr (NCH == 56) {
            return launch_wide_kh<EPI, W8>(a, blocks, waves, s);
        } else {
            return launch_wide_m<EPI, NCH, W8, 2>(a, blocks, waves, s);
        }
    }
    return launch_wide_m<EPI, NCH, W8, 1>(a, blocks, waves, s);
}

template <int EPI, int NCH>
int launch_wide_n(DecLinArgs& a, int blocks, int waves, kr_stream s) {
    return a.w_scale ? launch_wide_w<EPI, NCH, true>(a, blocks, waves, s) : launch_wide_w<EPI, NCH, false>(a, blocks, waves, s);
}

template <int EPI>
int launch_wide(DecLinArgs& a, int blocks, int waves, kr_stream s) {
    switch (a.K >> 6) {
        case 24: return launch_wide_n<EPI, 24>(a, blocks, waves, s);
        case 32: return launch_wide_n<EPI, 32>(a, blocks, waves, s);
        case 56: return launch_wide_n<EPI, 56>(a, blocks, waves, s);
        default: return launch_wide_n<EPI, 0>(a, blocks, waves, s);
    }
}

template <int NCH> struct NarrowCfg { static constexpr int RL = 8; };
template <> struct NarrowCfg<24> { static constexpr int RL = 3; };
template <> struct NarrowCfg<32> { static constexpr int RL = 4; };
template <> struct NarrowCfg<56> { static constexpr int RL = 7; };

template <int NT, int EPI, int WAVES, int NCH, int PKS, bool NORM, int U, bool W8, int MT, bool RES>
__global__ void __launch_bounds__(WAVES * 64) dec_narrow_kernel(const kr_bf16* hx, const kr_bf16* hwp, const kr_bf16* hnorm_w, const float* hpart_in,
                                                                int64_t hldx, int hM, int hN, int hK, int hcpb, float hnorm_eps,
                                                                int hprows, const DecLinArgs a) {
    extern __shared__ __attribute__((aligned(16))) char smem[];
    using WC = WChunk<W8>;
    constexpr int RL = NarrowCfg<NCH>::RL;
    constexpr bool FULL = NCH != 0;
    const int tid = threadIdx.x, lane = tid & 63;
    const int wave = __builtin_amdgcn_readfirstlane(tid >> 6);
    const int fr = lane & 15, fg = lane >> 4;
    const int g = blockIdx.x, ks = blockIdx.y;
    if (KR_EXP && a.pf_blocks > 0 && (int)blockIdx.x >= (int)gridDim.x - a.pf_blocks) {
        const int pb = blockIdx.x - ((int)gridDim.x - a.pf_blocks);
        const int64_t n16 = a.pf_bytes >> 4, stride = (int64_t)a.pf_blocks * (WAVES * 64);
        const u32x4* p = reinterpret_cast<const u32x4*>(a.pf_ptr);
        u32x4 acc = {0u, 0u, 0u, 0u};
        int64_t i = (int64_t)pb * (WAVES * 64) + threadIdx.x;
        for (; i + 15 * stride < n16; i += 16 * stride) {
            u32x4 v[16];
#pragma unroll
            for (int k = 0; k < 16; ++k) v[k] = p[i + k * stride];
#pragma unroll
            for (int k = 0; k < 16; ++k) acc ^= v[k];
        }
        for (; i < n16; i += stride) acc ^= p[i];
        asm volatile("" ::"v"(acc[0] ^ acc[1] ^ acc[2] ^ acc[3]));
        return;
    }
    const int M = hM, K = hK;
    const int nchunks = NCH ? NCH : (K >> 6), ntiles = hN >> 4, kc = K >> 3;
    const int cpb = hcpb;
    const int cb0 = min(ks * cpb, nchunks), cb1 = min(cb0 + cpb, nchunks);
    const int nblk = cb1 - cb0;
    const int c0 = cb0 + (wave * nblk) / WAVES, c1 = cb0 + ((wave + 1) * nblk) / WAVES;
    const int xrow = nblk * 128 + 16;
    float* red = reinterpret_cast<float*>(smem + (NORM ? ((M * xrow + 127) & ~127) : 0));

    int tile[NT];
    if (depi_rope(EPI)) {
        tile[0] = (g >> 2) * 8 + (g & 3);
        tile[NT - 1] = tile[0] + 4;
    } else {
#pragma unroll
        for (int t = 0; t < NT; ++t) tile[t] = g * NT + t;
    }
    const char* wp[NT];
#pragma unroll
    for (int t = 0; t < NT; ++t)
        wp[t] = reinterpret_cast<const char*>(hwp) + ((int64_t)min(tile[t], ntiles - 1) * nchunks) * WC::BYTES + lane * 16;
    int rb[MT];
#pragma unroll
    for (int mt = 0; mt < MT; ++mt) rb[mt] = min(fr + 16 * mt, M - 1);

    bf16x8 xv[NORM ? RL : 1], nwv[NORM ? RL : 1];
    f32x4 pv[PKS ? PKS : 1][NORM ? RL : 1][2];
    bf16x8 xf[NORM ? 1 : U][MT][2];
    const char* xg[MT];
#pragma unroll
    for (int mt = 0; mt < MT; ++mt) xg[mt] = reinterpret_cast<const char*>(hx + (int64_t)rb[mt] * hldx);
    if (NORM) {
        const int b = wave < M ? wave : 0;
#pragma unroll
        for (int i = 0; i < RL; ++i) {
            const int c = lane + i * 64;
            if (FULL || c < kc) {
                xv[i] = ld8(hx + (int64_t)b * hldx + c * 8);
#pragma unroll
                for (int k = 0; k < PKS; ++k) {
                    const float* pp = hpart_in + ((int64_t)k * hprows + b) * K + c * 8;
                    pv[k][i][0] = *reinterpret_cast<const f32x4*>(pp);
                    pv[k][i][1] = *reinterpret_cast<const f32x4*>(pp + 4);
                }
                nwv[i] = ld8(hnorm_w + c * 8);
            }
        }
    } else {
#pragma unroll
        for (int u = 0; u < U; ++u) {
            const int c = min(max(min(c0 + u, c1 - 1), cb0), nchunks - 1);
#pragma unroll
            for (int mt = 0; mt < MT; ++mt) {
                xf[u][mt][0] = *reinterpret_cast<const bf16x8*>(xg[mt] + c * 128 + WC::x_byte(0, fg));
                xf[u][mt][1] = *reinterpret_cast<const bf16x8*>(xg[mt] + c * 128 + WC::x_byte(1, fg));
            }
        }
    }
    int pos[MT], plen[MT];
#pragma unroll
    for (int mt = 0; mt < MT; ++mt) {
        pos[mt] = plen[mt] = 0;
        if (depi_rope(EPI)) {
            pos[mt] = a.ctx_len[rb[mt]];
            plen[mt] = a.prompt_len[rb[mt]];
        }
    }
    WC wbuf[U][NT];
#pragma unroll
    for (int u = 0; u < U; ++u) {
        const int c = min(max(min(c0 + u, c1 - 1), cb0), nchunks - 1);
#pragma unroll
        for (int t = 0; t < NT; ++t) wbuf[u][t].template load<RES>(wp[t], c);
    }
    __builtin_amdgcn_sched_barrier(0);
    if (a.zero_ptr) {
        const int zgx = (int)gridDim.x - (KR_EXP ? a.pf_blocks : 0);
        const int zstep = zgx * (int)gridDim.y * (WAVES * 64);
        for (int zi = ((int)blockIdx.y * zgx + (int)blockIdx.x) * (WAVES * 64) + tid; zi < a.zero_n16; zi += zstep)
            reinterpret_cast<f32x4*>(a.zero_ptr)[zi] = (f32x4){0.f, 0.f, 0.f, 0.f};
    }

    if constexpr (NORM) {
        auto norm_row = [&](const int b, bf16x8 (&xr)[RL], const bf16x8 (&nw)[RL]) {
            float ss = 0.f;
#pragma unroll
            for (int i = 0; i < RL; ++i) {
                if (FULL || lane + i * 64 < kc) {
#pragma unroll
                    for (int j = 0; j < 8; ++j) ss += bf2f(xr[i][j]) * bf2f(xr[i][j]);
                }
            }
            ss = wave_sum(ss);
            const float rs = rsqrtf(ss / (float)K + hnorm_eps);
#pragma unroll
            for (int i = 0; i < RL; ++i) {
                const int c = lane + i * 64;
                if ((FULL || c < kc) && c >= cb0 * 8 && c < cb1 * 8) {
                    bf16x8 o;
#pragma unroll
                    for (int j = 0; j < 8; ++j) o[j] = f2bf(bf2f(nw[i][j]) * bfround(bf2f(xr[i][j]) * rs));
                    *reinterpret_cast<bf16x8*>(smem + b * xrow + (c - cb0 * 8) * 16) = o;
                }
            }
        };
        if (PKS) {
#pragma unroll
            for (int i = 0; i < RL; ++i) {
                if (FULL || lane + i * 64 < kc) {
#pragma unroll
                    for (int j = 0; j < 8; ++j) {
                        float v = bf2f(xv[i][j]);
#pragma unroll
                        for (int k = 0; k < PKS; ++k) v += pv[k][i][j >> 2][j & 3];
                        xv[i][j] = f2bf(v);
                    }
                    if (g == 0 && ks == 0 && wave < M)
                        *reinterpret_cast<bf16x8*>(a.x_out + (int64_t)wave * a.ldxo + (lane + i * 64) * 8) = xv[i];
                }
            }
        }
        if (KR_EXP && a.x_out_f32 && g == 0 && ks == 0 && wave < M) {
#pragma unroll
            for (int i = 0; i < RL; ++i) {
                if (FULL || lane + i * 64 < kc) {
                    float* xo = a.x_out_f32 + (int64_t)wave * a.ldxf + (lane + i * 64) * 8;
                    *reinterpret_cast<f32x4*>(xo) = (f32x4){bf2f(xv[i][0]), bf2f(xv[i][1]), bf2f(xv[i][2]), bf2f(xv[i][3])};
                    *reinterpret_cast<f32x4*>(xo + 4) = (f32x4){bf2f(xv[i][4]), bf2f(xv[i][5]), bf2f(xv[i][6]), bf2f(xv[i][7])};
                }
            }
        }
        if (wave < M) norm_row(wave, xv, nwv);
        for (int b = wave + WAVES; b < M; b += WAVES) {
            bf16x8 v[RL];
#pragma unroll
            for (int i = 0; i < RL; ++i) {
                const int c = lane + i * 64;
                if (FULL || c < kc) {
// ... 19 lines not shown
                    if (KR_EXP && a.x_out_f32 && g == 0 && ks == 0) {
                        float* xo = a.x_out_f32 + (int64_t)b * a.ldxf + c * 8;
                        *reinterpret_cast<f32x4*>(xo) = (f32x4){bf2f(v[i][0]), bf2f(v[i][1]), bf2f(v[i][2]), bf2f(v[i][3])};
                        *reinterpret_cast<f32x4*>(xo + 4) = (f32x4){bf2f(v[i][4]), bf2f(v[i][5]), bf2f(v[i][6]), bf2f(v[i][7])};
                    }
                }
            }
            norm_row(b, v, nwv);
        }
        __syncthreads();
    }
    float csv[MT][8];
    bf16x4 bias0 = {}, bias1 = {};
#pragma unroll
    for (int mt = 0; mt < MT; ++mt)
#pragma unroll
        for (int j = 0; j < 8; ++j) csv[mt][j] = 0.f;
    if (depi_rope(EPI)) {
        const int i0 = (tile[0] & 7) * 16 + fg * 4;
#pragma unroll
        for (int mt = 0; mt < MT; ++mt) {
            const float* cs = a.cs_table + ((int64_t)rb[mt] * a.cs_stride + (pos[mt] - plen[mt])) * 128;
            const f32x4 cv = *reinterpret_cast<const f32x4*>(cs + i0), sv = *reinterpret_cast<const f32x4*>(cs + 64 + i0);
#pragma unroll
            for (int j = 0; j < 4; ++j) {
                csv[mt][j] = cv[j];
                csv[mt][4 + j] = sv[j];
            }
        }
        bias0 = *reinterpret_cast<const bf16x4*>(a.bias + tile[0] * 16 + fg * 4);
        bias1 = *reinterpret_cast<const bf16x4*>(a.bias + tile[NT - 1] * 16 + fg * 4);
    }

    bf16x4 res_pre[MT][NT], bias_pre[NT];
    if (EPI == DEPI_PLAIN) {
#pragma unroll
        for (int t = 0; t < NT; ++t) {
            const int n = min(tile[t], ntiles - 1) * 16 + fg * 4;
            bias_pre[t] = *reinterpret_cast<const bf16x4*>(a.bias ? a.bias + n : hx);
#pragma unroll
            for (int mt = 0; mt < MT; ++mt)
                res_pre[mt][t] = *reinterpret_cast<const bf16x4*>(a.residual ? a.residual + (int64_t)rb[mt] * a.ldr + n : hx);
        }
    }

    const char* xl[MT];
#pragma unroll
    for (int mt = 0; mt < MT; ++mt) xl[mt] = smem + rb[mt] * xrow;
    f32x4 acc[MT][NT];
#pragma unroll
    for (int mt = 0; mt < MT; ++mt)
#pragma unroll
        for (int t = 0; t < NT; ++t) acc[mt][t] = (f32x4){0.f, 0.f, 0.f, 0.f};
    for (int cc = c0; cc < c1; cc += U) {
#pragma unroll
        for (int u = 0; u < U; ++u) {
            const int c = cc + u;
            if (c < c1) {
                bf16x8 x0[MT], x1[MT];
#pragma unroll
                for (int mt = 0; mt < MT; ++mt) {
                    if (NORM) {
                        x0[mt] = *reinterpret_cast<const bf16x8*>(xl[mt] + (c - cb0) * 128 + WC::x_byte(0, fg));
                        x1[mt] = *reinterpret_cast<const bf16x8*>(xl[mt] + (c - cb0) * 128 + WC::x_byte(1, fg));
                    } else {
                        x0[mt] = xf[u][mt][0];
                        x1[mt] = xf[u][mt][1];
                    }
                }
#pragma unroll
                for (int t = 0; t < NT; ++t) {
                    const bf16x8 w0 = wbuf[u][t].frag(0), w1 = wbuf[u][t].frag(1);
#pragma unroll
                    for (int mt = 0; mt < MT; ++mt) {
                        acc[mt][t] = __builtin_amdgcn_mfma_f32_16x16x32_bf16(w0, x0[mt], acc[mt][t], 0, 0, 0);
                        acc[mt][t] = __builtin_amdgcn_mfma_f32_16x16x32_bf16(w1, x1[mt], acc[mt][t], 0, 0, 0);
                    }
                }
                const int cn = c + U;
                if (cn < c1) {
                    if (!NORM) {
#pragma unroll
                        for (int mt = 0; mt < MT; ++mt) {
                            xf[u][mt][0] = *reinterpret_cast<const bf16x8*>(xg[mt] + cn * 128 + WC::x_byte(0, fg));
                            xf[u][mt][1] = *reinterpret_cast<const bf16x8*>(xg[mt] + cn * 128 + WC::x_byte(1, fg));
                        }
                    }
#pragma unroll
                    for (int t = 0; t < NT; ++t) wbuf[u][t].template load<RES>(wp[t], cn);
                }
            }
        }
    }
    auto epilogue = [&](const int mt, f32x4 (&sum)[NT]) {
        const int b = fr + 16 * mt;
        if (b >= M) return;
#pragma unroll
        for (int t = 0; t < NT; ++t) apply_w_scale(a.w_scale, min(tile[t], ntiles - 1) * 16 + fg * 4, sum[t]);
        if (depi_rope(EPI)) {
            const int hh = tile[0] >> 3;
            const int i0 = (tile[0] & 7) * 16 + fg * 4;
            float lo[4], hi[4];
#pragma unroll
            for (int j = 0; j < 4; ++j) {
                lo[j] = bfround(sum[0][j] + bf2f(bias0[j]));
                hi[j] = bfround(sum[NT - 1][j] + bf2f(bias1[j]));
            }
            if (hh < a.heads + a.kv_heads) {
                bf16x4 o0, o1;
#pragma unroll
                for (int j = 0; j < 4; ++j) {
                    o0[j] = f2bf(lo[j] * csv[mt][j] - hi[j] * csv[mt][4 + j]);
                    o1[j] = f2bf(hi[j] * csv[mt][j] + lo[j] * csv[mt][4 + j]);
                }
                if (EPI == DEPI_ROPE_KV8 && hh >= a.heads) {
                    const int kh = hh - a.heads;
                    kv8_append_k(a.kv8.k + ((int64_t)b * a.kv_heads + kh) * a.s_max * 128, pos[mt], i0, o0, o1, a.kv8.scale[kh]);
                    return;
                }
                kr_bf16* dst = hh < a.heads
                                   ? a.q_out + ((int64_t)b * a.heads + hh) * 128
                                   : a.kcache + (((int64_t)b * a.kv_heads + (hh - a.heads)) * a.s_max + pos[mt]) * 128;
                *reinterpret_cast<bf16x4*>(dst + i0) = o0;
                *reinterpret_cast<bf16x4*>(dst + 64 + i0) = o1;
            } else {
                const int kvh = hh - a.heads - a.kv_heads;
                if (EPI == DEPI_ROPE_KV8) {
                    kv8_append_v(a.kv8.vt + ((int64_t)b * a.kv_heads + kvh) * a.s_max * 128, pos[mt], i0, lo, hi, a.kv8.scale[a.kv_heads + kvh]);
                    return;
                }
                kr_bf16* vt = a.vtcache + (((int64_t)b * a.kv_heads + kvh) * (a.s_max >> 6) + (pos[mt] >> 6)) * (128 * 64) + kr_vt_off(0, pos[mt] & 63, 128);
#pragma unroll
                for (int j = 0; j < 4; ++j) {
                    vt[(i0 + j) * 32] = __builtin_bit_cast(kr_bf16, f2bf(lo[j]));
                    vt[(64 + i0 + j) * 32] = __builtin_bit_cast(kr_bf16, f2bf(hi[j]));
                }
            }
            return;
        }
#pragma unroll
        for (int t = 0; t < NT; ++t) {
            if (tile[t] >= ntiles) continue;
            const int n = tile[t] * 16 + fg * 4;
            if (EPI == DEPI_PARTIAL) {
                if (a.part_atomic) {
                    float* acc = a.out_f32 + (int64_t)b * a.ldc + n;
#pragma unroll
                    for (int j = 0; j < 4; ++j) atomicAdd(acc + j, sum[t][j]);
                } else {
                    *reinterpret_cast<f32x4*>(a.out_f32 + ((int64_t)ks * M + b) * a.ldc + n) = sum[t];
                }
                continue;
            }
            float v[4];
#pragma unroll
            for (int j = 0; j < 4; ++j) v[j] = sum[t][j];
            if (a.bias) {
                const bf16x4 bv = EPI == DEPI_PLAIN ? bias_pre[t] : *reinterpret_cast<const bf16x4*>(a.bias + n);
#pragma unroll
                for (int j = 0; j < 4; ++j) v[j] += bf2f(bv[j]);
            }
            if (a.residual) {
                const bf16x4 rv = EPI == DEPI_PLAIN ? res_pre[mt][t]
                                                    : *reinterpret_cast<const bf16x4*>(a.residual + (int64_t)b * a.ldr + n);
#pragma unroll
                for (int j = 0; j < 4; ++j) v[j] += bf2f(rv[j]);
            }
            if (a.out_f32) {
                *reinterpret_cast<f32x4*>(a.out_f32 + (int64_t)b * a.ldc + n) = (f32x4){v[0], v[1], v[2], v[3]};
            } else {
                bf16x4 o;
#pragma unroll
                for (int j = 0; j < 4; ++j) o[j] = f2bf(v[j]);
                *reinterpret_cast<bf16x4*>(a.out + (int64_t)b * a.ldc + n) = o;
            }
        }
    };
#pragma unroll
    for (int mt = 0; mt < MT; ++mt) {
        if (mt > 0) __syncthreads();
#pragma unroll
        for (int t = 0; t < NT; ++t) *reinterpret_cast<f32x4*>(red + ((wave * NT + t) * 64 + lane) * 4) = acc[mt][t];
        __syncthreads();
        if (wave == 0) {
            f32x4 sum[NT];
#pragma unroll
            for (int t = 0; t < NT; ++t) {
                f32x4 half[2];
#pragma unroll
                for (int hfi = 0; hfi < 2; ++hfi) {
                    half[hfi] = (f32x4){0.f, 0.f, 0.f, 0.f};
#pragma unroll
                    for (int w = hfi * (WAVES / 2); w < (hfi + 1) * (WAVES / 2); ++w) {
                        const f32x4 p = *reinterpret_cast<const f32x4*>(red + ((w * NT + t) * 64 + lane) * 4);
#pragma unroll
                        for (int j = 0; j < 4; ++j) half[hfi][j] += p[j];
                    }
                }
#pragma unroll
                for (int j = 0; j < 4; ++j) sum[t][j] = half[0][j] + half[1][j];
            }
            epilogue(mt, sum);
        }
    }
}

template <int NT, int EPI, int WAVES, int NCH, int PKS, bool NORM, int U, bool W8, int MT, bool RES>
int launch_narrow_m(DecLinArgs& a, int groups, kr_stream s) {
    const int nchunks = a.K >> 6, cpb = (nchunks + a.ksplit - 1) / a.ksplit;
    const size_t xbytes = NORM ? (((size_t)a.M * (cpb * 128 + 16) + 127) & ~(size_t)127) : 0;
    const size_t lds = xbytes + (size_t)WAVES * NT * 256 * 4;
    KR_CHECK_ARG(lds <= 160 * 1024, "kr_linear_decode_narrow: M=%d K=%d needs %zu bytes of LDS", a.M, a.K, lds);
    auto fn = &dec_narrow_kernel<NT, EPI, WAVES, NCH, PKS, NORM, U, W8, MT, RES>;
    static KrPerDeviceOnce attr;
    if (attr.need()) {
        KR_CHECK_HIP(hipFuncSetAttribute(reinterpret_cast<const void*>(fn), hipFuncAttributeMaxDynamicSharedMemorySize, 160 * 1024));
    }
    KR_CHECK_ARG(a.pf_blocks == 0 || a.ksplit == 1, "kr_linear_decode_narrow: prefetch workgroups need ksplit 1");
    fn<<<dim3(groups + a.pf_blocks, a.ksplit), WAVES * 64, lds, kr_hs(s)>>>(a.x, a.wp, a.norm_w, a.part_in, a.ldx, a.M, a.N, a.K, cpb,
                                                                            a.norm_eps, a.part_rows > 0 ? a.part_rows : a.M, a);
    KR_CHECK_LAUNCH();
    return KR_OK;
}

template <int NT, int EPI, int WAVES, int NCH, int PKS, bool NORM, int U, bool W8, bool RES>
int launch_narrow_w(DecLinArgs& a, int groups, kr_stream s) {
    if (a.M > 16) {
        if constexpr (WAVES == 8 && NCH != 56) {
            return launch_narrow_m<NT, EPI, WAVES, NCH, PKS, NORM, U, W8, 2, RES>(a, groups, s);
        } else {
            kr_set_error("kr_linear_decode_narrow: M=%d > 16 needs 8-wave workgroups and K != 3584", a.M);
            return KR_ERR_ARG;
        }
    }
    return launch_narrow_m<NT, EPI, WAVES, NCH, PKS, NORM, U, W8, 1, RES>(a, groups, s);
}

template <int NT, int EPI, int WAVES, int NCH, int PKS, bool NORM, int U>
int launch_narrow_u(DecLinArgs& a, int groups, kr_stream s) {
    if (a.w_resident)
        return a.w_scale ? launch_narrow_w<NT, EPI, WAVES, NCH, PKS, NORM, U, true, true>(a, groups, s)
                         : launch_narrow_w<NT, EPI, WAVES, NCH, PKS, NORM, U, false, true>(a, groups, s);
    return a.w_scale ? launch_narrow_w<NT, EPI, WAVES, NCH, PKS, NORM, U, true, false>(a, groups, s)
                     : launch_narrow_w<NT, EPI, WAVES, NCH, PKS, NORM, U, false, false>(a, groups, s);
}

inline int narrow_share(const DecLinArgs& a, int waves) {
    const int nchunks = a.K >> 6, cpb = (nchunks + a.ksplit - 1) / a.ksplit;
    return (cpb + waves - 1) / waves;
}

template <int EPI, int WAVES>
int launch_narrow_direct(DecLinArgs& a, int groups, kr_stream s) {
    const int share = narrow_share(a, WAVES);
    if constexpr (EPI == DEPI_PARTIAL) {
        const char* e = getenv("KARANTA_NARROW_NT2");
        const bool nt2 = e ? atoi(e) != 0 : groups >= 192;
        if (nt2 && (groups & 1) == 0 && (a.M <= 16 || WAVES == 8)) {
            if constexpr (WAVES == 16) return launch_narrow_u<2, EPI, WAVES, 0, 0, false, 3>(a, groups / 2, s);
            else return launch_narrow_u<2, EPI, WAVES, 0, 0, false, 5>(a, groups / 2, s);
        }
    }
    if (share <= 3) return launch_narrow_u<1, EPI, WAVES, 0, 0, false, 3>(a, groups, s);
    if constexpr (WAVES == 16) {
        return launch_narrow_u<1, EPI, WAVES, 0, 0, false, 5>(a, groups, s);
    } else {
        if (share <= 5) return launch_narrow_u<1, EPI, WAVES, 0, 0, false, 5>(a, groups, s);
        return launch_narrow_u<1, EPI, WAVES, 0, 0, false, 8>(a, groups, s);
    }
}

template <int NT, int EPI, int NCH, int PKS>
int launch_narrow_norm_u(DecLinArgs& a, int groups, kr_stream s) {
    if (narrow_share(a, 8) <= 3) return launch_narrow_u<NT, EPI, 8, NCH, PKS, true, 3>(a, groups, s);
    return launch_narrow_u<NT, EPI, 8, NCH, PKS, true, 8 / NT>(a, groups, s);
}

template <int NT, int EPI>
int launch_narrow_norm(DecLinArgs& a, int groups, kr_stream s) {
    const int nch = a.K >> 6;
    if (a.part_in && a.n_part == 1) {
        if (nch == 24) return launch_narrow_norm_u<NT, EPI, 24, 1>(a, groups, s);
        if (nch == 32) return launch_narrow_norm_u<NT, EPI, 32, 1>(a, groups, s);
        if (nch == 56) return launch_narrow_norm_u<NT, EPI, 56, 1>(a, groups, s);
        kr_set_error("kr_linear_decode_narrow: deferred partial sums need K = 1536, 2048 or 3584 (K=%d)", a.K);
        return KR_ERR_ARG;
    }
    if (a.part_in) {
        if (nch == 24) return launch_narrow_norm_u<NT, EPI, 24, 2>(a, groups, s);
        if (nch == 32) return launch_narrow_norm_u<NT, EPI, 32, 2>(a, groups, s);
        if (nch == 56) return launch_narrow_norm_u<NT, EPI, 56, 2>(a, groups, s);
        kr_set_error("kr_linear_decode_narrow: deferred partial sums need K = 1536, 2048 or 3584 (K=%d)", a.K);
        return KR_ERR_ARG;
    }
    if (nch == 24) return launch_narrow_norm_u<NT, EPI, 24, 0>(a, groups, s);
    if (nch == 32) return launch_narrow_norm_u<NT, EPI, 32, 0>(a, groups, s);
    if (nch == 56) return launch_narrow_norm_u<NT, EPI, 56, 0>(a, groups, s);
    return launch_narrow_norm_u<NT, EPI, 0, 0>(a, groups, s);
}

#ifdef KR_EXPERIMENTS
template <bool W8, int TI, int NS>
__global__ void __launch_bounds__(512) dec_oproj_heads_kernel(const float* __restrict__ ws, const char* __restrict__ wp,
                                                              const float* __restrict__ w_scale, float* __restrict__ x_acc,
                                                              int64_t ld_acc, int M, int heads, int n_split, int tw) {
    extern __shared__ __attribute__((aligned(16))) char smem[];
    using WC = WChunk<W8>;
    constexpr int HD = 128, REC = HD + 4, XROW = HD * 2 + 16;
    const int tid = threadIdx.x, lane = tid & 63;
    const int wave = __builtin_amdgcn_readfirstlane(tid >> 6);
    const int fr = lane & 15, fg = lane >> 4;
    const int tg = blockIdx.x, h = blockIdx.y;
    const int nchunks = heads * 2;
    float* outs = reinterpret_cast<float*>(smem + ((32 * XROW + 127) & ~127));

    const int ns = NS ? NS : n_split;
    constexpr int MAXS = NS ? NS : 16;
    const int b0 = tid >> 5, d4 = (tid & 31) << 2;
    f32x4 ro[2][MAXS], rm[2][MAXS];
#pragma unroll
    for (int mt = 0; mt < 2; ++mt) {
        const int b = b0 + 16 * mt;
        if (mt == 0 || M > 16) {
            const float* rec = ws + ((int64_t)(b < M ? b : 0) * heads + h) * ns * REC;
#pragma unroll
            for (int p = 0; p < MAXS; ++p) {
                if (p < ns) {
                    ro[mt][p] = *reinterpret_cast<const f32x4*>(rec + p * REC + d4);
                    rm[mt][p] = *reinterpret_cast<const f32x4*>(rec + p * REC + HD);
                }
            }
        }
    }
    WC wb[TI][2];
    int tile[TI];
#pragma unroll
    for (int i = 0; i < TI; ++i) {
        const int tl = wave + 8 * i;
        tile[i] = tg * tw + (tl < tw ? tl : tw - 1);
        const char* p = wp + ((int64_t)tile[i] * nchunks) * WC::BYTES + lane * 16;
        wb[i][0].load(p, 2 * h);
        wb[i][1].load(p, 2 * h + 1);
    }
    __builtin_amdgcn_sched_barrier(0);
#pragma unroll
    for (int mt = 0; mt < 2; ++mt) {
        const int b = b0 + 16 * mt;
        if ((mt == 0 || M > 16) && b < M) {
            float mm = -1e30f;
#pragma unroll
            for (int p = 0; p < MAXS; ++p)
                if (p < ns) mm = fmaxf(mm, rm[mt][p][0]);
// ... 96 lines not shown
    }
}

}

extern "C" int kr_linear_decode(int mode, const kr_bf16* x, int64_t ldx, const kr_bf16* w_packed, const kr_bf16* bias,
                                const kr_bf16* norm_w, float norm_eps, const kr_bf16* residual, int64_t ldr, kr_bf16* out,
                                float* out_f32, int64_t ldc, int M, int N, int K, int waves, int max_blocks, int ksplit, float* ws,
                                int32_t* counters, const float* attn_partials, int attn_split, const float* cs_table,
                                int cs_stride, const int32_t* prompt_len, const int32_t* ctx_len, kr_bf16* q_out,
                                kr_bf16* kcache, kr_bf16* vtcache, int heads, int kv_heads, int s_max, float* amax_val,
                                int32_t* amax_idx, kr_stream s) {
    KR_CHECK_ARG(w_packed && (x || attn_partials), "kr_linear_decode: null pointer");
    KR_CHECK_ARG(M >= 1 && M <= 16, "kr_linear_decode: M=%d must be in 1..16", M);
    KR_CHECK_ARG(N > 0 && N % 16 == 0 && K > 0 && K % 64 == 0, "kr_linear_decode: N=%d K=%d (N%%16, K%%64)", N, K);
    KR_CHECK_ARG(attn_partials || (ldx >= K && (ldx & 7) == 0), "kr_linear_decode: ldx");
    KR_CHECK_ARG(ksplit >= 1 && ksplit <= (K >> 6), "kr_linear_decode: ksplit=%d", ksplit);
    KR_CHECK_ARG(ksplit == 1 || (ws && counters), "kr_linear_decode: split-K needs workspace and counters");
    KR_CHECK_ARG(!norm_w || K <= 4096, "kr_linear_decode: fused RMSNorm supports K <= 4096");
    KR_CHECK_ARG(!(norm_w && attn_partials), "kr_linear_decode: norm and attention-merge prologues are exclusive");
    KR_CHECK_ARG(!attn_partials || (K % 128 == 0 && attn_split >= 1 && ksplit == 1),
                 "kr_linear_decode: attention merge needs K = heads*128, ksplit 1");
    DecLinArgs a{};
    a.x = x; a.ldx = ldx; a.wp = w_packed; a.bias = bias; a.norm_w = norm_w; a.norm_eps = norm_eps;
    a.residual = residual; a.ldr = ldr; a.out = out; a.out_f32 = out_f32; a.ldc = ldc;
    a.M = M; a.N = N; a.K = K; a.ksplit = ksplit; a.ws = ws; a.counters = counters;
    a.attn_ws = attn_partials; a.attn_split = attn_split;
    a.xmode = attn_partials ? 3 : norm_w ? 2 : 1;
    a.cs_table = cs_table; a.cs_stride = cs_stride; a.prompt_len = prompt_len; a.ctx_len = ctx_len;
    a.q_out = q_out; a.kcache = kcache; a.vtcache = vtcache;
    a.heads = heads; a.kv_heads = kv_heads; a.s_max = s_max; a.amax_val = amax_val; a.amax_idx = amax_idx;
    const int ntiles = N >> 4;
    switch (mode) {
        case DEPI_PLAIN: {
            KR_CHECK_ARG((out || out_f32) && ldc >= N && (ldc & 3) == 0, "kr_linear_decode: PLAIN output");
            KR_CHECK_ARG(!residual || (ldr & 3) == 0, "kr_linear_decode: ldr");
            if (ntiles >= 1024) return launch_dec_w<2, DEPI_PLAIN>(a, (ntiles + 1) / 2, waves, max_blocks, s);
            return launch_dec_w<1, DEPI_PLAIN>(a, ntiles, waves, max_blocks, s);
        }
        case DEPI_SILU:
            KR_CHECK_ARG(out && N % 32 == 0 && ldc >= N / 2 && (ldc & 3) == 0, "kr_linear_decode: SILU output");
            return launch_dec_w<2, DEPI_SILU>(a, ntiles / 2, waves, max_blocks, s);
        case DEPI_SILU8:
            KR_CHECK_ARG(out && ldc >= N / 2 && (ldc & 3) == 0, "kr_linear_decode: SILU8 output");
            return launch_dec_w<1, DEPI_SILU8>(a, ntiles, waves, max_blocks, s);
        case DEPI_ROPE_KV:
            KR_CHECK_ARG(bias && cs_table && prompt_len && ctx_len && q_out && kcache && vtcache && cs_stride > 0,
                         "kr_linear_decode: ROPE_KV pointers");
            KR_CHECK_ARG(N == (heads + 2 * kv_heads) * 128 && s_max % 64 == 0, "kr_linear_decode: ROPE_KV needs head_dim 128");
            return launch_dec_w<2, DEPI_ROPE_KV>(a, ntiles / 2, waves, max_blocks, s);
        case DEPI_ARGMAX:
            KR_CHECK_ARG(amax_val && amax_idx && ksplit == 1, "kr_linear_decode: ARGMAX pointers / ksplit");
            KR_CHECK_ARG(!out_f32 || ldc >= N, "kr_linear_decode: ARGMAX logits ldc");
            return launch_dec_w<2, DEPI_ARGMAX>(a, (ntiles + 1) / 2, waves, max_blocks, s);
        default:
            kr_set_error("kr_linear_decode: unknown mode %d", mode);
            return KR_ERR_ARG;
    }
}

static int wide_impl(int mode, const kr_bf16* x, int64_t ldx, const void* w_packed, const float* w_scale, const kr_bf16* bias,
                     const kr_bf16* norm_w, float norm_eps, const kr_bf16* residual, int64_t ldr,
                     kr_bf16* out, float* out_f32, int64_t ldc, int M, int N, int K, int blocks, int waves,
                     float* amax_val, int32_t* amax_idx, kr_stream s, bool x_is_f32 = false, kr_bf16* x_out = nullptr,
                     int64_t ldxo = 0) {
    KR_CHECK_ARG(x && w_packed, "kr_linear_decode_wide: null pointer");
    KR_CHECK_ARG(M >= 1 && M <= 32, "kr_linear_decode_wide: M=%d must be in 1..32", M);
    KR_CHECK_ARG(N > 0 && N % 16 == 0 && K > 0 && K % 512 == 0 && K <= 4096,
                 "kr_linear_decode_wide: N=%d K=%d (N%%16, K%%512, K<=4096)", N, K);
    KR_CHECK_ARG(ldx >= K && (ldx & 7) == 0, "kr_linear_decode_wide: ldx");
    KR_CHECK_ARG(blocks > 0 && waves >= 1 && waves <= 8, "kr_linear_decode_wide: blocks=%d waves=%d", blocks, waves);
    DecLinArgs a{};
    a.x_is_f32 = x_is_f32 ? 1 : 0; a.wide_x_out = x_out; a.wide_ldxo = ldxo;
    a.x = x; a.ldx = ldx; a.wp = reinterpret_cast<const kr_bf16*>(w_packed); a.w_scale = w_scale; a.bias = bias;
    a.norm_w = norm_w; a.norm_eps = norm_eps;
    a.residual = residual; a.ldr = ldr; a.out = out; a.out_f32 = out_f32; a.ldc = ldc;
    a.M = M; a.N = N; a.K = K; a.ksplit = 1; a.amax_val = amax_val; a.amax_idx = amax_idx;
    a.wide_blocks = blocks; a.wide_waves = waves;
    if (mode & KR_DEC_OUT_XP) {
        KR_CHECK_ARG((mode & ~KR_DEC_OUT_XP) == DEPI_SILU8 && M > 16 && (N / 2) % 64 == 0 && ((uintptr_t)out & 15) == 0,
                     "kr_linear_decode_wide: KR_DEC_OUT_XP is for SILU8 at 17..32 rows, N/2 %% 64 == 0");
        a.out_xp = 1;
        mode &= ~KR_DEC_OUT_XP;
    }
    switch (mode) {
        case DEPI_PLAIN:
            KR_CHECK_ARG((out || out_f32) && ldc >= N && (ldc & 3) == 0 && (!residual || (ldr & 3) == 0), "kr_linear_decode_wide: PLAIN output");
            return launch_wide<DEPI_PLAIN>(a, blocks, waves, s);
        case DEPI_SILU8:
            KR_CHECK_ARG(out && ldc >= N / 2 && (ldc & 3) == 0, "kr_linear_decode_wide: SILU8 output");
            return launch_wide<DEPI_SILU8>(a, blocks, waves, s);
        case DEPI_ARGMAX:
            KR_CHECK_ARG(amax_val && amax_idx && (!out_f32 || ldc >= N), "kr_linear_decode_wide: ARGMAX pointers");
            return launch_wide<DEPI_ARGMAX>(a, blocks, waves, s);
        default:
            kr_set_error("kr_linear_decode_wide: mode %d not supported (PLAIN, SILU8, ARGMAX)", mode);
            return KR_ERR_ARG;
    }
}

extern "C" int kr_linear_decode_wide(int mode, const kr_bf16* x, int64_t ldx, const kr_bf16* w_packed, const kr_bf16* bias,
                                     const kr_bf16* norm_w, float norm_eps, const kr_bf16* residual, int64_t ldr,
                                     kr_bf16* out, float* out_f32, int64_t ldc, int M, int N, int K, int blocks, int waves,
                                     float* amax_val, int32_t* amax_idx, kr_stream s) {
    return wide_impl(mode, x, ldx, w_packed, nullptr, bias, norm_w, norm_eps, residual, ldr, out, out_f32, ldc, M, N, K, blocks,
                     waves, amax_val, amax_idx, s);
}

extern "C" int kr_linear_decode_wide_fp8(int mode, const kr_bf16* x, int64_t ldx, const uint8_t* w_packed_fp8,
                                         const float* w_scale, const kr_bf16* bias, const kr_bf16* norm_w, float norm_eps,
                                         const kr_bf16* residual, int64_t ldr, kr_bf16* out, float* out_f32, int64_t ldc,
                                         int M, int N, int K, int blocks, int waves, float* amax_val, int32_t* amax_idx,
                                         kr_stream s) {
    KR_CHECK_ARG(w_scale, "kr_linear_decode_wide_fp8: w_scale is NULL");
    return wide_impl(mode, x, ldx, w_packed_fp8, w_scale, bias, norm_w, norm_eps, residual, ldr, out, out_f32, ldc, M, N, K,
                     blocks, waves, amax_val, amax_idx, s);
}

static int narrow_impl(int mode, const kr_bf16* x, int64_t ldx, const float* part_in, int n_part_in,
                                       kr_bf16* x_out, int64_t ldxo, const void* w_packed, const float* w_scale, const kr_bf16* bias,
                                       const kr_bf16* norm_w, float norm_eps, const kr_bf16* residual, int64_t ldr,
                                       kr_bf16* out, float* out_f32, int64_t ldc, int M, int N, int K, int waves, int ksplit,
                                       const float* cs_table, int cs_stride, const int32_t* prompt_len, const int32_t* ctx_len,
                                       kr_bf16* q_out, kr_bf16* kcache, kr_bf16* vtcache, int heads, int kv_heads, int s_max,
                                       const kr_narrow_opts* opts, kr_stream s, float* x_out_f32 = nullptr, int64_t ldxf = 0,
                                       const void* pf_ptr = nullptr, size_t pf_bytes = 0, int pf_blocks = 0,
                                       const kr_kv8* kv8 = nullptr) {
    KR_CHECK_ARG(x && w_packed, "kr_linear_decode_narrow: null pointer");
    const kr_narrow_opts o = opts ? *opts : kr_narrow_opts{};
    KR_CHECK_ARG((o.zero_ptr || o.zero_bytes == 0) && ((uintptr_t)o.zero_ptr & 15) == 0 && (o.zero_bytes & 15) == 0 && o.zero_bytes < (1u << 30),
                 "kr_linear_decode_narrow: opts zero range");
    KR_CHECK_ARG(o.part_rows >= 0 && o.part_rows <= 32, "kr_linear_decode_narrow: opts part_rows=%d", o.part_rows);
    KR_CHECK_ARG(M >= 1 && M <= 32, "kr_linear_decode_narrow: M=%d must be in 1..32", M);
    KR_CHECK_ARG(N > 0 && N % 16 == 0 && K > 0 && K % 64 == 0, "kr_linear_decode_narrow: N=%d K=%d (N%%16, K%%64)", N, K);
    KR_CHECK_ARG(ldx >= K && (ldx & 7) == 0, "kr_linear_decode_narrow: ldx");
    KR_CHECK_ARG(waves == 8 || waves == 16, "kr_linear_decode_narrow: waves=%d (8 or 16)", waves);
    KR_CHECK_ARG(ksplit >= 1 && ksplit <= 8 && ksplit <= (K >> 6), "kr_linear_decode_narrow: ksplit=%d", ksplit);
    KR_CHECK_ARG(!norm_w || K <= 4096, "kr_linear_decode_narrow: fused RMSNorm supports K <= 4096");
    KR_CHECK_ARG(!part_in || (norm_w && (n_part_in == 1 || n_part_in == 2) && x_out && x_out != x && ldxo >= K && (ldxo & 7) == 0),
                 "kr_linear_decode_narrow: partial sums need the norm prologue, 1 or 2 slabs and a separate x_out");
    DecLinArgs a{};
    a.x = x; a.ldx = ldx; a.wp = reinterpret_cast<const kr_bf16*>(w_packed); a.w_scale = w_scale; a.bias = bias;
    a.norm_w = norm_w; a.norm_eps = norm_eps;
    a.residual = residual; a.ldr = ldr; a.out = out; a.out_f32 = out_f32; a.ldc = ldc;
    a.M = M; a.N = N; a.K = K; a.ksplit = ksplit;
    a.part_in = part_in; a.x_out = x_out; a.ldxo = ldxo;
    a.x_out_f32 = x_out_f32; a.ldxf = ldxf;
    a.part_rows = o.part_rows;
    a.n_part = part_in ? n_part_in : 0;
    a.zero_ptr = o.zero_bytes ? o.zero_ptr : nullptr; a.zero_n16 = (int)(o.zero_bytes >> 4); a.part_atomic = o.atomic_out ? 1 : 0;
    a.w_resident = o.w_resident ? 1 : 0;
    KR_CHECK_ARG(!a.part_atomic || (ksplit == 2 && mode == DEPI_PLAIN), "kr_linear_decode_narrow: atomic_out is for ksplit 2 (order-free sum)");
    KR_CHECK_ARG(a.part_rows == 0 || (part_in && a.part_rows >= M), "kr_linear_decode_narrow: part rows %d < M %d", a.part_rows, M);
    if (KR_EXP && pf_blocks > 0) {
        KR_CHECK_ARG(ksplit == 1 && pf_ptr && ((uintptr_t)pf_ptr & 15) == 0 && pf_blocks <= 1024, "kr_linear_decode_narrow_pf: bad args");
        a.pf_ptr = reinterpret_cast<const char*>(pf_ptr); a.pf_bytes = (int64_t)pf_bytes; a.pf_blocks = pf_bytes >= 16 ? pf_blocks : 0;
    }
    a.cs_table = cs_table; a.cs_stride = cs_stride; a.prompt_len = prompt_len; a.ctx_len = ctx_len;
    a.q_out = q_out; a.kcache = kcache; a.vtcache = vtcache;
    a.heads = heads; a.kv_heads = kv_heads; a.s_max = s_max;
    const int ntiles = N >> 4;
    switch (mode) {
        case DEPI_PLAIN:
            KR_CHECK_ARG(ldc >= N && (ldc & 3) == 0 && (!residual || (ldr & 3) == 0), "kr_linear_decode_narrow: PLAIN ldc / ldr");
            if (ksplit > 1) {
                KR_CHECK_ARG(out_f32 && !out && !bias && !residual && !norm_w,
                             "kr_linear_decode_narrow: split-K writes f32 slabs only (no bias / residual / norm)");
                return waves == 16 ? launch_narrow_direct<DEPI_PARTIAL, 16>(a, ntiles, s)
                                   : launch_narrow_direct<DEPI_PARTIAL, 8>(a, ntiles, s);
            }
            KR_CHECK_ARG(out || out_f32, "kr_linear_decode_narrow: PLAIN output");
            if (norm_w) return launch_narrow_norm<1, DEPI_PLAIN>(a, ntiles, s);
            return waves == 16 ? launch_narrow_direct<DEPI_PLAIN, 16>(a, ntiles, s)
                               : launch_narrow_direct<DEPI_PLAIN, 8>(a, ntiles, s);
        case DEPI_ROPE_KV:
            if (kv8) {
                KR_CHECK_ARG(bias && cs_table && prompt_len && ctx_len && q_out && kv8->k && kv8->vt && kv8->scale && cs_stride > 0 && norm_w,
                             "kr_linear_decode_narrow_kv8: ROPE_KV8 pointers (norm_w included)");
                KR_CHECK_ARG(N == (heads + 2 * kv_heads) * 128 && s_max % 64 == 0 && ksplit == 1 && (((uintptr_t)kv8->k | (uintptr_t)kv8->vt) & 3) == 0,
                             "kr_linear_decode_narrow_kv8: ROPE_KV8 needs head_dim 128, ksplit 1, a 4-byte aligned cache");
                a.kv8 = Kv8{kv8->k, kv8->vt, kv8->scale};
                return launch_narrow_norm<2, DEPI_ROPE_KV8>(a, ntiles / 2, s);
            }
            KR_CHECK_ARG(bias && cs_table && prompt_len && ctx_len && q_out && kcache && vtcache && cs_stride > 0,
                         "kr_linear_decode_narrow: ROPE_KV pointers");
            KR_CHECK_ARG(N == (heads + 2 * kv_heads) * 128 && s_max % 64 == 0 && ksplit == 1,
                         "kr_linear_decode_narrow: ROPE_KV needs head_dim 128, ksplit 1");
            if (!norm_w) {
                KR_CHECK_ARG(!part_in && waves == 8, "kr_linear_decode_narrow: ROPE_KV without a norm takes no partial sums, 8 waves");
                if (narrow_share(a, 8) <= 3) return launch_narrow_u<2, DEPI_ROPE_KV, 8, 0, 0, false, 3>(a, ntiles / 2, s);
                return launch_narrow_u<2, DEPI_ROPE_KV, 8, 0, 0, false, 5>(a, ntiles / 2, s);
            }
            return launch_narrow_norm<2, DEPI_ROPE_KV>(a, ntiles / 2, s);
        default:
            kr_set_error("kr_linear_decode_narrow: mode %d not supported (PLAIN, ROPE_KV)", mode);
            return KR_ERR_ARG;
    }
}

extern "C" int kr_linear_decode_narrow(int mode, const kr_bf16* x, int64_t ldx, const float* part_in, int n_part_in,
                                       kr_bf16* x_out, int64_t ldxo, const kr_bf16* w_packed, const kr_bf16* bias,
                                       const kr_bf16* norm_w, float norm_eps, const kr_bf16* residual, int64_t ldr,
                                       kr_bf16* out, float* out_f32, int64_t ldc, int M, int N, int K, int waves, int ksplit,
                                       const float* cs_table, int cs_stride, const int32_t* prompt_len, const int32_t* ctx_len,
                                       kr_bf16* q_out, kr_bf16* kcache, kr_bf16* vtcache, int heads, int kv_heads, int s_max,
                                       const kr_narrow_opts* opts, kr_stream s) {
    return narrow_impl(mode, x, ldx, part_in, n_part_in, x_out, ldxo, w_packed, nullptr, bias, norm_w, norm_eps, residual, ldr, out,
                       out_f32, ldc, M, N, K, waves, ksplit, cs_table, cs_stride, prompt_len, ctx_len, q_out, kcache, vtcache,
                       heads, kv_heads, s_max, opts, s);
}

extern "C" int kr_linear_decode_narrow_fp8(int mode, const kr_bf16* x, int64_t ldx, const float* part_in, int n_part_in,
                                           kr_bf16* x_out, int64_t ldxo, const uint8_t* w_packed_fp8, const float* w_scale,
                                           const kr_bf16* bias, const kr_bf16* norm_w, float norm_eps, const kr_bf16* residual,
                                           int64_t ldr, kr_bf16* out, float* out_f32, int64_t ldc, int M, int N, int K, int waves,
                                           int ksplit, const float* cs_table, int cs_stride, const int32_t* prompt_len,
                                           const int32_t* ctx_len, kr_bf16* q_out, kr_bf16* kcache, kr_bf16* vtcache, int heads,
                                           int kv_heads, int s_max, const kr_narrow_opts* opts, kr_stream s) {
    KR_CHECK_ARG(w_scale, "kr_linear_decode_narrow_fp8: w_scale is NULL");
    return narrow_impl(mode, x, ldx, part_in, n_part_in, x_out, ldxo, w_packed_fp8, w_scale, bias, norm_w, norm_eps, residual, ldr,
                       out, out_f32, ldc, M, N, K, waves, ksplit, cs_table, cs_stride, prompt_len, ctx_len, q_out, kcache, vtcache,
                       heads, kv_heads, s_max, opts, s);
}

extern "C" int kr_linear_decode_narrow_kv8(const kr_bf16* x, int64_t ldx, const float* part_in, int n_part_in, kr_bf16* x_out,
                                           int64_t ldxo, const void* w_packed, const float* w_scale, const kr_bf16* bias,
                                           const kr_bf16* norm_w, float norm_eps, int M, int N, int K, int waves,
                                           const float* cs_table, int cs_stride, const int32_t* prompt_len, const int32_t* ctx_len,
                                           kr_bf16* q_out, const kr_kv8* kv, int heads, int kv_heads, int s_max,
                                           const kr_narrow_opts* opts, kr_stream s) {
    KR_CHECK_ARG(kv, "kr_linear_decode_narrow_kv8: kv is NULL");
    return narrow_impl(DEPI_ROPE_KV, x, ldx, part_in, n_part_in, x_out, ldxo, w_packed, w_scale, bias, norm_w, norm_eps, nullptr, 0,
                       nullptr, nullptr, 0, M, N, K, waves, 1, cs_table, cs_stride, prompt_len, ctx_len, q_out, nullptr, nullptr,
                       heads, kv_heads, s_max, opts, s, nullptr, 0, nullptr, 0, 0, kv);
}

namespace {
template <int RL, int NP>
__global__ void __launch_bounds__(256) dec_resnorm_kernel(const kr_bf16* __restrict__ x, int64_t ldx, const float* __restrict__ parts,
                                                          int n_part, int part_rows, kr_bf16* __restrict__ x_out, int64_t ldxo,
                                                          const kr_bf16* __restrict__ norm_w, float eps, kr_bf16* __restrict__ h,
                                                          int64_t ldh, int M, int K, int h_xp) {
    const int lane = threadIdx.x & 63, b = blockIdx.x * 4 + (threadIdx.x >> 6), kc = K >> 3;
    if (b >= M) return;
    constexpr int NPR = NP > 0 ? NP : 1;
    bf16x8 xv[RL], nw[RL];
    f32x4 pv[NPR][RL][2];
#pragma unroll
    for (int i = 0; i < RL; ++i) {
        const int c = min(lane + i * 64, kc - 1);
        xv[i] = ld8(x + (int64_t)b * ldx + c * 8);
        nw[i] = ld8(norm_w + c * 8);
        if constexpr (NP > 0) {
#pragma unroll
            for (int k = 0; k < NP; ++k) {
                const float* pp = parts + ((int64_t)k * part_rows + b) * K + c * 8;
                pv[k][i][0] = *reinterpret_cast<const f32x4*>(pp);
// ... 159 lines not shown
```

karanta_ocr_amd/csrc/kr_decode_common.h:

```cpp
#pragma once
#include "kr_common.h"

namespace {

#ifdef KR_EXPERIMENTS
constexpr bool KR_EXP = true;
#else
constexpr bool KR_EXP = false;
#endif

constexpr int DEPI_PLAIN = 0, DEPI_SILU = 1, DEPI_ROPE_KV = 2, DEPI_ARGMAX = 3, DEPI_SILU8 = 4;
constexpr int DEPI_PARTIAL = 16;

template <bool W8> struct WChunk;
template <> struct WChunk<false> {
    static constexpr int BYTES = 2048;
    bf16x8 v[2];
    template <bool RES = false> __device__ __forceinline__ void load(const char* p, int64_t c) {
        const kr_bf16* q = reinterpret_cast<const kr_bf16*>(p + c * BYTES);
        v[0] = RES ? ld8(q) : ld8_nt(q);
        v[1] = RES ? ld8(q + 512) : ld8_nt(q + 512);
    }
    __device__ __forceinline__ bf16x8 frag(int h) const { return v[h]; }
    static __device__ __forceinline__ int x_byte(int h, int fg) { return h * 64 + fg * 16; }
    static __device__ __forceinline__ int xp_off(int h, int fr, int fg) { return h * 1024 + (fg * 16 + fr) * 16; }
};
template <> struct WChunk<true> {
    static constexpr int BYTES = 1024;
    u32x4 q;
    template <bool RES = false> __device__ __forceinline__ void load(const char* p, int64_t c) {
        const u32x4* w = reinterpret_cast<const u32x4*>(p + c * BYTES);
        q = RES ? *w : __builtin_nontemporal_load(w);
    }
    __device__ __forceinline__ bf16x8 frag(int h) const {
        u32x4 o;
#pragma unroll
        for (int i = 0; i < 2; ++i) {
            const int w = (int)q[2 * h + i];
            o[2 * i + 0] = __builtin_bit_cast(unsigned, __builtin_amdgcn_cvt_scalef32_pk_bf16_fp8(w, 1.0f, false));
            o[2 * i + 1] = __builtin_bit_cast(unsigned, __builtin_amdgcn_cvt_scalef32_pk_bf16_fp8(w, 1.0f, true));
        }
        return __builtin_bit_cast(bf16x8, o);
    }
    static __device__ __forceinline__ int x_byte(int h, int fg) { return fg * 32 + h * 16; }
    static __device__ __forceinline__ int xp_off(int h, int fr, int fg) { return (fg >> 1) * 1024 + ((((fg & 1) << 1) | h) * 16 + fr) * 16; }
};

__device__ __forceinline__ void apply_w_scale(const float* w_scale, int n, f32x4& acc) {
    if (w_scale) {
        const f32x4 sc = *reinterpret_cast<const f32x4*>(w_scale + n);
#pragma unroll
        for (int j = 0; j < 4; ++j) acc[j] *= sc[j];
    }
}

constexpr int DEPI_ROPE_KV8 = 5;
constexpr bool depi_rope(int epi) { return epi == DEPI_ROPE_KV || epi == DEPI_ROPE_KV8; }

struct Kv8 {
    uint8_t* k; uint8_t* vt; const float* scale;
};

__device__ __forceinline__ float kv8_clamp(float x, float sc, int& clamped) {
    const float y = x / sc;
    const float c = __builtin_amdgcn_fmed3f(y, -448.f, 448.f);
    clamped += (c != y) ? 1 : 0;
    return c;
}
__device__ __forceinline__ unsigned kv8_pack4(float x0, float x1, float x2, float x3, float sc, int& clamped) {
    int w = 0;
    w = __builtin_amdgcn_cvt_pk_fp8_f32(kv8_clamp(x0, sc, clamped), kv8_clamp(x1, sc, clamped), w, false);
    w = __builtin_amdgcn_cvt_pk_fp8_f32(kv8_clamp(x2, sc, clamped), kv8_clamp(x3, sc, clamped), w, true);
    return (unsigned)w;
}
__device__ __forceinline__ uint8_t kv8_code(float x, float sc, int& clamped) {
    return (uint8_t)(__builtin_amdgcn_cvt_pk_fp8_f32(kv8_clamp(x, sc, clamped), 0.f, 0, false) & 0xff);
}
__device__ __forceinline__ bf16x8 kv8_to_bf16x8(unsigned w0, unsigned w1) {
    u32x4 o;
    o[0] = __builtin_bit_cast(unsigned, __builtin_amdgcn_cvt_scalef32_pk_bf16_fp8((int)w0, 1.0f, false));
    o[1] = __builtin_bit_cast(unsigned, __builtin_amdgcn_cvt_scalef32_pk_bf16_fp8((int)w0, 1.0f, true));
    o[2] = __builtin_bit_cast(unsigned, __builtin_amdgcn_cvt_scalef32_pk_bf16_fp8((int)w1, 1.0f, false));
    o[3] = __builtin_bit_cast(unsigned, __builtin_amdgcn_cvt_scalef32_pk_bf16_fp8((int)w1, 1.0f, true));
    return __builtin_bit_cast(bf16x8, o);
}

__device__ __forceinline__ void kv8_append_k(uint8_t* krow0, int pos, int i0, const bf16x4& o0, const bf16x4& o1, float sc) {
    int n = 0;
    uint8_t* dst = krow0 + (int64_t)pos * 128;
    *reinterpret_cast<unsigned*>(dst + i0) = kv8_pack4(bf2f(o0[0]), bf2f(o0[1]), bf2f(o0[2]), bf2f(o0[3]), sc, n);
    *reinterpret_cast<unsigned*>(dst + 64 + i0) = kv8_pack4(bf2f(o1[0]), bf2f(o1[1]), bf2f(o1[2]), bf2f(o1[3]), sc, n);
}
__device__ __forceinline__ void kv8_append_v(uint8_t* vt0, int pos, int i0, const float (&lo)[4], const float (&hi)[4], float sc) {
    int n = 0;
    uint8_t* vt = vt0 + (int64_t)(pos >> 6) * (128 * 64) + kr_vt_off(0, pos & 63, 128);
    const unsigned a = kv8_pack4(lo[0], lo[1], lo[2], lo[3], sc, n), b = kv8_pack4(hi[0], hi[1], hi[2], hi[3], sc, n);
#pragma unroll
    for (int j = 0; j < 4; ++j) {
        vt[(i0 + j) * 32] = (uint8_t)(a >> (8 * j));
        vt[(64 + i0 + j) * 32] = (uint8_t)(b >> (8 * j));
    }
}

__device__ __forceinline__ void better(float& bv, int& bi, float v, int i) {
    if (v > bv || (v == bv && i < bi)) { bv = v; bi = i; }
}

}
```

karanta_ocr_amd/engine.py:

```python
from __future__ import annotations

import ctypes as C
import os
import time
from dataclasses import dataclass, field
from typing import Dict, List, Optional, Sequence, Tuple

import numpy as np
import torch

from . import image_processing as IP
from . import positions as POS
from ._lib import (DEC_ARGMAX, DEC_OUT_XP, DEC_PLAIN, DEC_ROPE_KV, DEC_SILU8, Dec32, EPI_NONE, EPI_SILU_MUL8, KarantaHipError, Spec, lib,
                   narrow_opts, ptr)
from . import kv_cache
from .config import ModelConfig
from .kv_cache import KV_SCALES_FLAG_WINS
from .weights import KV_SCALE_RANGES, kv_cache_dtype_name
from .device_weights import DeviceWeights, _align, narrow_weight_bytes, plan_resident
from .request import GenerateResult, PageRequest, SpecConfig, children
from .sampler import DeviceGuide, Sampler
from .sampling import StepFeatures, has_penalties
from .vision import DevicePlan, VisionTower, device_plan

BF16 = torch.bfloat16
GEMM_SCRATCH_BYTES = 512 * 65536
FP8_ACT_DEFAULT = False
IC_RESIDENT_GAINS: Tuple[Tuple[str, float], ...] = (("qkv", 0.07),)
IC_RESIDENT_MB = 192
IC_RESIDENT_MIN_US = 0.1
SEQUENCE_SWITCHES = ("KARANTA_NARROW", "KARANTA_NARROW_O", "KARANTA_DEFER_DOWN", "KARANTA_WIDE", "KARANTA_ATOMIC_SLAB", "KARANTA_DEC32")

__all__ = ["Engine", "PageRequest", "SpecConfig", "DeviceWeights", "GenerateResult", "children", "SEQUENCE_SWITCHES", "DeviceGuide"]


@dataclass
class Admission:
    B: int
    slots: List[int]
    whole_batch: bool
    lens: List[int]
    M: int
    src: np.ndarray
    cos: np.ndarray
    sin: np.ndarray
    deltas: np.ndarray
    plan: POS.AttnPlan
    last_rows: np.ndarray
    cs: np.ndarray
    n_img: int
    temps: Optional[np.ndarray] = None
    seeds: Optional[np.ndarray] = None
    guides: Optional[list] = None
    procs: Optional[list] = None
    adjs: Optional[list] = None
    reps: Optional[list] = None
    need: StepFeatures = StepFeatures()
    n_pages: int = 0
    rows: list = field(default_factory=list)
    forks: list = field(default_factory=list)
    kvq: list = field(default_factory=list)

    def spans(self, width: int):
        return [(0, 0, width)] if self.whole_batch else [(b, j, 1) for b, j in enumerate(self.slots)]

    def copies(self, rows: np.ndarray, width: int):
        if self.whole_batch:
            rows = np.concatenate([rows[:self.B], np.zeros(width - self.B, rows.dtype)])
        return [(j, rows[b:b + n]) for b, j, n in self.spans(width)]


class Engine:
    def __init__(self, cfg: ModelConfig, device: str = "cuda:0", max_batch: int = 8, s_max: int = 4096,
                 max_patches: int = 8 * 5476, max_prompt_tokens: int = 8 * 2048, decode_splits: int = 16,
                 weight_dtype: str = "bf16", fp8_activations: Optional[bool] = None, admission_cus: Optional[int] = None,
                 speculative: Optional[SpecConfig] = None, ic_resident_mb: Optional[int] = None, kv_cache_dtype: str = "auto",
                 calculate_kv_scales: bool = False, kv_scale_ranges: Tuple[float, float] = KV_SCALE_RANGES):
        if not torch.cuda.is_available():
            raise KarantaHipError("no HIP device: the karanta MI355X engine has no CPU fallback")
        self.L = lib()
        self.cfg = cfg
        self.device = torch.device(device)
        torch.cuda.set_device(self.device)
        self.stream = torch.cuda.Stream(device=self.device)
        self.s = self.stream.cuda_stream
        self.B = max_batch
        if max_batch > 32:
            raise KarantaHipError("max_batch > 32: the decode kernels take at most two 16-row column tiles")
        self.spec = speculative
        if speculative is not None:
            speculative.check(max_batch)
        self.K = int(speculative.num_tokens) if speculative is not None else 0
        self.rows = speculative.rows(max_batch) if speculative is not None else max_batch
        self.share_rows = speculative is not None and bool(speculative.share_rows)
        self.spec_guided = speculative is not None and bool(speculative.guided)
        self.spec_controls = speculative is not None and bool(speculative.controls)
# ... 28 lines not shown
        self.kv_scale_ranges = tuple(float(r) for r in kv_scale_ranges)
        if len(self.kv_scale_ranges) != 2 or not all(np.isfinite(r) and r > 0 for r in self.kv_scale_ranges):
            raise KarantaHipError(f"kv_scale_ranges {kv_scale_ranges!r}: (K range, V range), finite and positive")
        if v.head_dim not in (80, 128) or t.head_dim != 128:
            raise KarantaHipError(f"unsupported head dims vit={v.head_dim} llm={t.head_dim}")
        self.w = DeviceWeights(cfg, self.device, weight_dtype)
        self.fp8 = weight_dtype == "fp8"
        self.set_resident_budget(IC_RESIDENT_MB if ic_resident_mb is None else ic_resident_mb)
        self.fp8_prefill_gemm = os.environ.get("KARANTA_FP8_PREFILL", "1") == "1"
        env = os.environ.get("KARANTA_FP8_ACT")
        self.fp8_act = self.fp8 and self.fp8_prefill_gemm and (bool(fp8_activations) if fp8_activations is not None
                                                              else (env == "1" if env is not None else FP8_ACT_DEFAULT))
        self._graphs: Dict[Tuple[int, bool], int] = {}
        self._prof_on = False
        self._prof_events: List[Tuple[C.c_void_p, C.c_void_p]] = []
        self._prof_next = 0
        self._last_batch = max_batch
        self._alloc()

    def set_resident_budget(self, mb: int, gains: Optional[Sequence[Tuple[str, float]]] = None):
        for g in getattr(self, "_graphs", {}).values():
            self.L.kr_graph_destroy(g)
        getattr(self, "_graphs", {}).clear()
        self.ic_resident_mb = int(mb)
        self.resident = plan_resident(narrow_weight_bytes(self.cfg, self.w.weight_dtype),
                                      IC_RESIDENT_GAINS if gains is None else gains, self.ic_resident_mb * 10 ** 6,
                                      IC_RESIDENT_MIN_US)

    def _refuse_retired_switches(self):
        if type(self) is Engine and any(os.environ.get(k, "0") not in ("", "0") for k in
                                        ("KARANTA_PREFETCH", "KARANTA_FAST_RESIDUAL", "KARANTA_ATTN_FUSED", "KARANTA_MERGE_IN_OPROJ")):
            raise KarantaHipError("KARANTA_PREFETCH / KARANTA_FAST_RESIDUAL / KARANTA_ATTN_FUSED / KARANTA_MERGE_IN_OPROJ are decode "
                                  "experiments: they run on csrc/tools/experiment_engine.ExperimentEngine with a -DKR_EXPERIMENTS "
                                  "library (csrc/tools/build_variant.py, KARANTA_HIP_LIB), not on the product engine")
        if os.environ.get("KARANTA_RESNORM32_QKV", "1") != "1":
            raise KarantaHipError("KARANTA_RESNORM32_QKV is retired: the packed family with the fused row-major qkv launch was "
                                  "measured and dropped (profiles/r04_decode32_chains.txt)")
        moved = [k for k in SEQUENCE_SWITCHES if os.environ.get(k, "1") != "1"] + [k for k in ("KARANTA_RESNORM_QKV",) if k in os.environ]
        if type(self) is Engine and moved:
            raise KarantaHipError(" / ".join(moved) + ": superseded decode launch sequences run on csrc/tools/experiment_engine."
                                  "ExperimentEngine (csrc/tools/decode_ab.py builds it for such a variant), not on the product engine")

    def _alloc(self):
        t, dev = self.cfg.text, self.device
        M, B, R = self.max_tokens, self.B, self.rows
        z = lambda *shape, dtype=BF16: torch.zeros(*shape, dtype=dtype, device=dev)
        self.vision = VisionTower(self)
        self.p_x = z(M, t.hidden_size)
        self.p_h = z(M, t.hidden_size)
        self.p_qkv = z(M, t.qkv_dim)
        self.p_q = z(t.num_heads, M, t.head_dim)
        self.p_o = z(M, t.q_dim)
        self.p_act = z(M, t.intermediate_size)
        self.p_cos = z(M, t.head_dim, dtype=torch.float32)
        self.p_sin = z(M, t.head_dim, dtype=torch.float32)
        self.p_src = z(M, dtype=torch.int32)
        if self.fp8_act:
            self.p_a8 = z(M, (max(t.intermediate_size, t.hidden_size, t.q_dim) + 15) // 16 * 16, dtype=torch.uint8)
            self.p_as = z(M, dtype=torch.float32)
        self.gemm_scratch = z(GEMM_SCRATCH_BYTES // 4, dtype=torch.float32)
        self.kv = kv_cache.make(self)
        self.d_x = z(R, t.hidden_size)
        self.d_x2 = z(R, t.hidden_size)
        self.d_part = z(4 if R > 16 else 2, R, t.hidden_size, dtype=torch.float32)
        if t.hidden_size // 16 >= 192:
            self.down_waves_small = 8
        self.d_qkv = z(B, t.qkv_dim)
        Bp = 32 if R > 16 else B
        self.d_h = z(Bp, t.hidden_size)
        self.d_q = z(R, t.num_heads, t.head_dim)
        self.d_o = z(Bp, t.q_dim)
        self.d_act = z(Bp, t.intermediate_size)
        self.d_logits = z(R, t.vocab_size, dtype=torch.float32)
        self.d_ws = z(R * t.num_heads * self.n_split * (t.head_dim + 4), dtype=torch.float32)
        self.wv_qkv = self._waves(t.hidden_size // 64)
        self.wv_o = self._waves(t.q_dim // 64)
        self.wv_down = self._waves(t.intermediate_size // 64)
        self.wv_wide = 4
        for name in ("qkv", "o", "down", "wide"):
            v_ = os.environ.get("KARANTA_WV_" + name.upper())
            if v_:
                setattr(self, "wv_" + name, int(v_))
        self.defer_down = t.hidden_size in (1536, 2048, 3584)
        self.wide_mode = t.hidden_size % 512 == 0 and t.hidden_size <= 4096
        self.wide_blocks = int(os.environ.get("KARANTA_WIDE_BLOCKS", "256"))
        self.wide_waves = int(os.environ.get("KARANTA_WIDE_WAVES", "0"))
        self.wide_spread32 = os.environ.get("KARANTA_WIDE_SPREAD32", "1") == "1"
        if R > 16 and not (self.wide_mode and t.intermediate_size % 64 == 0):
            raise KarantaHipError("max_batch > 16 needs the wide / narrow decode kernels (hidden_size % 512 == 0) and hidden_size <= 2048 or == 3584")
        self.row_split = self.B > 16 and t.hidden_size > 2048
        self.family32, self.resnorm_qkv = self.B > 16, self.row_split
        self.group_split_down = int(os.environ.get("KARANTA_DOWN_GS", "1"))
        if R > 16 and t.hidden_size > 2048 and t.hidden_size != 3584:
            raise KarantaHipError("max_batch > 16: hidden_size <= 2048 or == 3584 (the 7B width) only")
        if self.fp8 and not self.wide_mode:
            raise KarantaHipError("fp8 weights need the wide / narrow decode kernels: hidden_size % 512 == 0 and <= 4096")
        self.n_amax = (max(self._amax_parts(0), self._amax_parts(32)) if self.wide_mode
                       else (t.vocab_size // 16 + 1) // 2)
        self.d_amax_v = z(R, self.n_amax, dtype=torch.float32)
        self.d_amax_i = z(R, self.n_amax, dtype=torch.int32)
        self.d_plen = z(R, dtype=torch.int32)[:B]
        self.d_cs = None
        self.d_ctx = z(R, dtype=torch.int32)[:B]
        self.d_delta = z(B, dtype=torch.int32)
        self.d_tok = z(B, dtype=torch.int32)
        self.d_fin = z(R, dtype=torch.int32)[:B]
        self._snap_ring, self._snap_next, self._snap_event, self._copy_stream = None, 0, None, None
        self._rep_read = np.full(B, -1, np.int64)
        self.d_temp = z(R, dtype=torch.float32)[:B]
        self.d_seed = z(R, dtype=torch.int32)[:B]
        if self.spec is not None:
            self.d_row_slot = torch.arange(R, dtype=torch.int32, device=dev) % B
            self.d_prompt_ids = z(B, self.s_max, dtype=torch.int32)
            self.d_ndraft = z(B, dtype=torch.int32)
            self.d_draft = z(B, self.K, dtype=torch.int32)
            if self.share_rows:
                self.d_nwant = z(B, dtype=torch.int32)
                self.d_draft_row = torch.full((B, self.K), -1, dtype=torch.int32, device=dev)
            self.d_spec_count = z(2, B, dtype=torch.int32)
            self.d_script = z(B, dtype=torch.int64)
            self.d_script_len = z(B, dtype=torch.int32)
            self._scripts: Dict[int, torch.Tensor] = {}
        self.sampler = Sampler(self)
        self.max_new = 0
        self._req_max_new = 0
        self.d_hist = None
        self.d_eos = torch.tensor(list(self.cfg.eos_token_ids), dtype=torch.int32, device=dev)
        self.d_invfreq = torch.from_numpy(POS.rope_inv_freq(t.head_dim, t.rope_theta)).to(dev)
        self.d_last = z(B, dtype=torch.int32)
        self.d_prompt_x = z(B, t.hidden_size)
        self._slot_plen = [0] * B
        self.pages_prefilled = self.sequences_started = self.sequences_forked = self.sequences_reused = 0
        torch.cuda.synchronize(dev)

    @staticmethod
    def _waves(nchunks: int) -> int:
        return 16 if nchunks >= 64 else 8 if nchunks >= 16 else 4

    def set_kv_scales(self, k, v, source: str = "set_kv_scales"):
        self.kv.set_scales(k, v, source)

    def kv_scales(self) -> np.ndarray:
        return self.kv.scales()

    @property
    def kv_scales_ready(self) -> bool:
        return self.kv.scales_ready

    @property
    def kv_scales_calibrated(self) -> bool:
        return self.kv.calibrated

    @property
    def kv_clamped(self) -> int:
        return self.kv.clamped

    @property
    def kv_scale_source(self) -> str:
        return self.kv.scale_source

    def kv_cache_bytes(self) -> int:
        return self.kv.nbytes()

    kcache = property(lambda self: self.kv.kcache)
    vtcache = property(lambda self: self.kv.vtcache)
    d_kv_scale = property(lambda self: self.kv.d_kv_scale)
    d_kv_work = property(lambda self: self.kv.d_kv_work)

    def load_weights(self, weights: Dict[str, np.ndarray], log=None):
        self.w.load(weights)
        self.kv.load_scales(weights, log)

    def _gemm(self, A, W, C_, M, bias=None, res=None, epi=EPI_NONE, packed=False, w8=None, w_scale=None):
        N, K = W.shape
        if w8 is not None and self.fp8_act:
            ldq = self.p_a8.stride(0)
            self.L.kr_quantize_rows_fp8(ptr(A), A.stride(0), ptr(self.p_a8), ldq, ptr(self.p_as), M, K, self.s)
            self.L.kr_gemm_fp8a(ptr(self.p_a8), ldq, ptr(self.p_as), ptr(w8), ptr(w_scale), ptr(bias), ptr(res),
                                res.stride(0) if res is not None else 0, ptr(C_), C_.stride(0), M, N, K, epi, self.s)
            return
        if w8 is not None and self.fp8_prefill_gemm:
            self.L.kr_gemm_fp8(ptr(A), A.stride(0), ptr(w8), ptr(w_scale), ptr(bias), ptr(res),
                               res.stride(0) if res is not None else 0, ptr(C_), C_.stride(0), M, N, K, epi, self.s)
            return
        self.L.kr_gemm_bf16_ws(ptr(A), A.stride(0), ptr(W), ptr(bias), ptr(res), res.stride(0) if res is not None else 0,
                               ptr(C_), C_.stride(0), M, N, K, epi, 1 if packed else 0, ptr(self.gemm_scratch),
                               self.gemm_scratch.numel() * 4, self.s)

    def _dec(self, mode, x, W, M, out=None, out_f32=None, norm_w=None, waves=4):
        t = self.cfg.text
        N, K = W.shape
        o = out if out is not None else out_f32
        self.L.kr_linear_decode(mode, ptr(x), x.stride(0), ptr(W), 0, ptr(norm_w), t.rms_norm_eps, 0, 0, ptr(out), ptr(out_f32),
                                o.stride(0) if o is not None else 0, M, N, K, waves, self.persist_blocks, 1, 0, 0,
                                0, self.n_split, ptr(self.d_cs), self.max_new, ptr(self.d_plen),
                                ptr(self.d_ctx), ptr(self.d_q), 0, 0, t.num_heads, t.num_kv_heads, self.s_max,
                                ptr(self.d_amax_v), ptr(self.d_amax_i), self.s)

    def _dec_narrow(self, mode, x, W, M, out=None, out_f32=None, bias=None, norm_w=None, res=None, waves=8, ksplit=1,
                    part_in=None, x_out=None, kc=0, vc=0, w8=None, w_scale=None, zero=None, atomic_out=False,
                    resident=False, kv8=None):
        t = self.cfg.text
        N, K = W.shape
        o = out if out is not None else out_f32
        if kv8 is not None:
            self.L.kr_linear_decode_narrow_kv8(
                ptr(x), x.stride(0), ptr(part_in), int(part_in.shape[0]) if part_in is not None else 0, ptr(x_out),
                x_out.stride(0) if x_out is not None else 0, ptr(w8 if w8 is not None else W), ptr(w_scale), ptr(bias), ptr(norm_w),
                t.rms_norm_eps, M, N, K, waves, ptr(self.d_cs), self.max_new, ptr(self.d_plen), ptr(self.d_ctx), ptr(self.d_q),
                kv8, t.num_heads, t.num_kv_heads, self.s_max,
                narrow_opts(ptr(zero), zero.numel() * 4 if zero is not None else 0, atomic_out, w_resident=resident), self.s)
            return
        head = (mode, ptr(x), x.stride(0), ptr(part_in), int(part_in.shape[0]) if part_in is not None else 0, ptr(x_out),
                x_out.stride(0) if x_out is not None else 0)
        args = (ptr(bias), ptr(norm_w), t.rms_norm_eps, ptr(res), res.stride(0) if res is not None else 0, ptr(out),
                ptr(out_f32), o.stride(-2) if o is not None else 0, M, N, K, waves, ksplit, ptr(self.d_cs), self.max_new,
                ptr(self.d_plen), ptr(self.d_ctx), ptr(self.d_q), kc, vc, t.num_heads, t.num_kv_heads, self.s_max,
                narrow_opts(ptr(zero), zero.numel() * 4 if zero is not None else 0, atomic_out, w_resident=resident), self.s)
        if w8 is not None:
            self.L.kr_linear_decode_narrow_fp8(*head, ptr(w8), ptr(w_scale), *args)
        else:
            self.L.kr_linear_decode_narrow(*head, ptr(W), *args)

    def _dec32(self, mode, xp, W, M, waves_ref, out=None, out_f32=None, bias=None, res=None, ksplit=1, atomic_out=False, zero=None,
               kc=0, vc=0, w8=None, w_scale=None, tiles_per_wg=0, group_split=False, row_slot=None, kv8=None):
        t = self.cfg.text
        N, K = W.shape
        o = out if out is not None else out_f32
        a = Dec32(ptr(xp), ptr(w8 if w8 is not None else W), ptr(w_scale), ptr(bias), ptr(res), res.stride(0) if res is not None else 0,
                  ptr(out), ptr(out_f32), o.stride(-2) if o is not None else 0, M, N, K, waves_ref, ksplit, 1 if atomic_out else 0,
                  tiles_per_wg, 1 if group_split else 0, 0, ptr(zero) if zero is not None else None,
                  zero.numel() * 4 if zero is not None else 0,
                  ptr(self.d_cs), self.max_new, ptr(self.d_plen), ptr(self.d_ctx), ptr(self.d_q), kc or None, vc or None,
                  t.num_heads, t.num_kv_heads, self.s_max)
        if kv8 is not None:
            self.L.kr_linear_decode32_kv8(C.byref(a), kv8, ptr(row_slot), self.s)
        elif row_slot is not None:
            self.L.kr_linear_decode32_rows(mode, C.byref(a), ptr(row_slot), self.s)
        else:
            self.L.kr_linear_decode32(mode, C.byref(a), self.s)

    narrow_mode = narrow_o = atomic_slab = resnorm32_qkv = True

    down_waves_small = 16
    down_gs_tiles = 0
    o_waves = 8

    def _w8kw(self, name: str) -> dict:
        w8, sc = self._w8(name)
        return {} if w8 is None else {"w8": w8, "w_scale": sc}

    def _w8(self, name: str):
        if self.fp8 and self.w.has(name + "8"):
            return self.w.view_u8(name + "8"), self.w.view_f32(name[:-1] + "s")
        return None, None

    def _wide_geometry(self, N: int, M: int = 0):
        tiles = N // 16
        if M > 16 and not self.wide_waves and self.wide_spread32:
            own = min(8, -(-tiles // self.wide_blocks))
            return min(self.wide_blocks, -(-tiles // own)), 8
        waves = self.wide_waves or (8 if M > 16 else min(8, -(-tiles // self.wide_blocks)))
        return min(self.wide_blocks, -(-tiles // waves)), waves

    def _amax_parts(self, M: int) -> int:
        wb, ww = self._wide_geometry(self.cfg.text.vocab_size, M)
        return wb * ww

    def _dec_wide(self, mode, x, W, M, out=None, out_f32=None, norm_w=None, w8=None, w_scale=None):
        N, K = W.shape
        blocks, waves = self._wide_geometry(N, M)
        o = out if out is not None else out_f32
        tail = (0, ptr(norm_w), self.cfg.text.rms_norm_eps, 0, 0, ptr(out), ptr(out_f32), o.stride(0) if o is not None else 0,
                M, N, K, blocks, waves, ptr(self.d_amax_v), ptr(self.d_amax_i), self.s)
        if w8 is not None:
            self.L.kr_linear_decode_wide_fp8(mode, ptr(x), x.stride(0), ptr(w8), ptr(w_scale), *tail)
        else:
            self.L.kr_linear_decode_wide(mode, ptr(x), x.stride(0), ptr(W), *tail)

    def _h2d(self, dst: torch.Tensor, arr: np.ndarray):
        src = torch.from_numpy(np.ascontiguousarray(arr))
        dst.view(-1)[:src.numel()].copy_(src.view(-1), non_blocking=False)

    def patches_from_images(self, images, min_pixels: int = IP.MIN_PIXELS, max_pixels: int = IP.MAX_PIXELS_CLASS_DEFAULT, grids=None):
        return self.vision.patches_from_images(images, min_pixels, max_pixels, grids)

    def vit_forward(self, pixel_values, grids: Sequence[Sequence[int]]) -> torch.Tensor:
        return self.vision.vit_forward(pixel_values, grids)

    def set_vocab(self, token_bytes: Sequence[bytes]):
        self.sampler.set_vocab(token_bytes)

    def compile_guide(self, guide) -> DeviceGuide:
        return self.sampler.compile_guide(guide)

    def _attention(self, qkv, k_off, v_off, cos, sin, dp: DevicePlan, q, k, k_stride, vt, vt_stride, out, H, KVH, hd, causal):
        L, s = self.L, self.s
        L.kr_qkv_prep(ptr(qkv), qkv.shape[1], 0, k_off, v_off, ptr(cos), ptr(sin),
                      ptr(dp.blk_tok0), ptr(dp.blk_ntok), ptr(dp.blk_kr), ptr(dp.blk_vb), dp.n_blk,
                      ptr(q), q.stride(0), ptr(k), k_stride, ptr(vt), vt_stride, H, KVH, hd, s)
        L.kr_attn_varlen_q(ptr(q), ptr(k), ptr(vt), ptr(out), ptr(dp.qblk), ptr(dp.qlen), dp.host.qblk.shape[0], q.shape[1],
# ... 113 lines not shown
                self.kv.prefill_layer_done(i, adm)
                self._gemm(self.p_o, w.view(p + "o.w"), self.p_x, M, res=self.p_x, packed=True, **self._w8kw(p + "o.w"))
                L.kr_rmsnorm(ptr(self.p_x), d, ptr(w.view(p + "ln2.w")), ptr(self.p_h), M, d, t.rms_norm_eps, s)
                self._gemm(self.p_h, w.view(p + "gate_up.w"), self.p_act, M, epi=EPI_SILU_MUL8, packed=True, **self._w8kw(p + "gate_up.w"))
                self._gemm(self.p_act, w.view(p + "down.w"), self.p_x, M, res=self.p_x, packed=True, **self._w8kw(p + "down.w"))
            self.kv.prefill_done(adm)
            self.pages_prefilled += adm.n_pages
            if not defer_activation:
                self._fork(adm.forks)
                self._activate(adm, state=False)
        return adm

    def _fork(self, groups):
        if not groups:
            return
        self.kv.fork(groups)
        self.sequences_forked += sum(len(g[2]) for g in groups)

    def _admit_features(self, pages) -> StepFeatures:
        need = StepFeatures.of(pages)
        self.sampler.check_features(need)
        self._step |= need
        return need

    def _activate(self, a: Admission, src_of: Optional[Sequence[int]] = None, state: bool = True, tokens: bool = True):
        if state:
            lens = np.asarray(a.lens, np.int32)
            for j, n in zip(a.slots, a.lens):
                self._slot_plen[j] = int(n)
            self.sequences_started += a.B
            fields = ((self.d_delta, a.deltas), (self.d_ctx, lens - 1), (self.d_plen, lens),
                      (self.d_temp, a.temps), (self.d_seed, a.seeds))
            for dst, rows in fields:
                for j, part in a.copies(rows, self.B):
                    self._h2d(dst[j:], part)
            for b, j, n in a.spans(a.B):
                self._h2d(self.d_cs[j:], a.cs[b:b + n])
            for _, j, n in a.spans(self.B):
                self.d_fin[j:j + n].zero_()
            if self.spec is not None:
                for p, j in zip(a.rows, a.slots):
                    self._h2d(self.d_prompt_ids[j], np.asarray(p.input_ids, np.int64).reshape(-1).astype(np.int32))
            self.sampler.write(a)
        if tokens:
            d = self.cfg.text.hidden_size
            for b, j, n in a.spans(a.B):
                if src_of is None:
                    self.L.kr_embed_scatter(ptr(self.d_last[b:]), ptr(self.p_x), 0, ptr(self.d_x[j:]), n, d, self.s)
                    self.L.kr_embed_scatter(ptr(self.d_last[b:]), ptr(self.p_x), 0, ptr(self.d_prompt_x[j:]), n, d, self.s)
                else:
                    if j != src_of[b]:
                        self.d_prompt_x[j].copy_(self.d_prompt_x[src_of[b]])
                    self.d_x[j].copy_(self.d_prompt_x[j])
                self._lm_head_and_sample(n, slot0=j)

    def _flags(self) -> int:
        return (1 if self._ignore_eos else 0) | (2 if self._freeze_finished else 0)

    def _lm_head(self, B: int, x, j: int = 0):
        w, step = self.w, self._step
        logits = self.d_logits[j:] if (self._want_logits or step.sampling or step.processing or self._logprobs is not None) else None
        if self.wide_mode:
            self._dec_wide(DEC_ARGMAX, x[j:], w.view("llm.lm_head"), B, norm_w=w.view("llm.norm.w"), out_f32=logits)
        else:
            self._dec(DEC_ARGMAX, x[j:], w.view("llm.lm_head"), B, norm_w=w.view("llm.norm.w"), out_f32=logits,
                      waves=self.wv_wide)
        return logits, (self._amax_parts(B) if self.wide_mode else self.n_amax)

    def _lm_head_and_sample(self, B: int, x=None, slot0: int = 0):
        t, w = self.cfg.text, self.w
        j = slot0
        logits, n_part = self._lm_head(B, self.d_x if x is None else x, j)
        flags = self._flags()
        n_part = self.sampler.pre_token(logits, n_part, B, j, flags)
        self.L.kr_sample_greedy(ptr(self.d_amax_v), ptr(self.d_amax_i), n_part, ptr(w.view("llm.embed")), t.hidden_size,
                                ptr(self.d_tok[j:]), ptr(self.d_hist[:, j:]), self.d_hist.stride(0), ptr(self.d_plen[j:]),
                                ptr(self.d_ctx[j:]), ptr(self.d_fin[j:]), ptr(self.d_eos), self.d_eos.numel(),
                                self.cfg.pad_token_id, flags, ptr(self.d_x[j:]), B, self.s)
        self.sampler.post_token(logits, B, j, flags)

    def _decode_step_launches(self, B: int):
        self._lm_head_and_sample(B, self._layer_launches(B))

    def _gate_up(self, x, i: int, B: int, out_xp: bool = False):
        w, p = self.w, f"llm.{i}."
        if self.wide_mode:
            self._dec_wide(DEC_SILU8 | (DEC_OUT_XP if out_xp else 0), x, w.view(p + "gate_up.w"), B, out=self.d_act,
                           norm_w=w.view(p + "ln2.w"), **self._w8kw(p + "gate_up.w"))
        else:
            self._dec(DEC_SILU8, x, w.view(p + "gate_up.w"), B, out=self.d_act, norm_w=w.view(p + "ln2.w"), waves=self.wv_wide)

    def _layer_launches(self, B: int, row_slot=None):
        t, L, w, s = self.cfg.text, self.L, self.w, self.s
        H, hd = t.num_heads, t.head_dim
        nl = t.num_layers
        big = B > 16
        x, x_other = self.d_x, self.d_x2
        pending = False
        slabs = self.d_part.view(-1)[: 2 * B * t.hidden_size].view(2, B, t.hidden_size)
        gs = (big and self.defer_down and not self.fp8
              and (self.group_split_down == 2 or self.group_split_down == 1 and self.down_waves_small == 16)
              and (t.hidden_size // 16) % (4 if self.down_waves_small == 8 else 2) == 0)
        if gs:
            slabs = self.d_part.view(-1)[: 4 * B * t.hidden_size].view(2, 2, B, t.hidden_size)
        for i in range(nl):
            p = f"llm.{i}."
            defer = self.defer_down and i + 1 < nl
            acc = slabs[(i + 1) & 1] if defer else None
            pin = (slabs[i & 1] if gs else slabs[i & 1:(i & 1) + 1]) if pending else None
            if big:
                L.kr_decode_resnorm32(ptr(x), x.stride(0), ptr(pin), int(pin.shape[0]) if pending else 0, B, ptr(x_other),
                                      x_other.stride(0), ptr(w.view(p + "ln1.w")), t.rms_norm_eps, ptr(self.d_h), B, t.hidden_size,
                                      1 if (gs and pending) else 0, s)
                self._dec32(DEC_ROPE_KV, self.d_h, w.view(p + "qkv.w"), B, 8, bias=w.view(p + "qkv.b"), zero=acc,
                            row_slot=row_slot, **self.kv.qkv(i), **self._w8kw(p + "qkv.w"))
            else:
                self._dec_narrow(DEC_ROPE_KV, x, w.view(p + "qkv.w"), B, bias=w.view(p + "qkv.b"), norm_w=w.view(p + "ln1.w"),
                                 part_in=pin, x_out=x_other if pending else None, zero=acc,
                                 resident=(i, "qkv") in self.resident, **self.kv.qkv(i), **self._w8kw(p + "qkv.w"))
            if pending:
                x, x_other = x_other, x
            self.kv.attention(i, B, row_slot)
            (L.kr_attn_decode_merge32 if big else L.kr_attn_decode_merge)(ptr(self.d_ws), ptr(self.d_o), B, H, hd, self.n_split, s)
            if big:
                self._dec32(DEC_PLAIN, self.d_o, w.view(p + "o.w"), B, self.o_waves, out=x, res=x, **self._w8kw(p + "o.w"))
            else:
                self._dec_narrow(DEC_PLAIN, self.d_o, w.view(p + "o.w"), B, out=x, res=x, waves=self.o_waves,
                                 resident=(i, "o") in self.resident, **self._w8kw(p + "o.w"))
            if self._prof_on:
                (e0, e1), (e2, _) = self._prof_event_pair(), self._prof_event_pair()
                L.kr_event_record(e0, s)
                L.kr_event_record(e1, s)
            self._gate_up(x, i, B, out_xp=big)
            if self._prof_on:
                L.kr_event_record(e2, s)
            down = dict(ksplit=2, out_f32=acc, atomic_out=True) if defer else dict(out=x, res=x)
            if gs and defer:
                self._dec32(DEC_PLAIN, self.d_act, w.view(p + "down.w"), B, self.down_waves_small, group_split=True,
                            tiles_per_wg=self.down_gs_tiles, **down)
            elif big:
                self._dec32(DEC_PLAIN, self.d_act, w.view(p + "down.w"), B, self.down_waves_small, **down, **self._w8kw(p + "down.w"))
            else:
                self._dec_narrow(DEC_PLAIN, self.d_act, w.view(p + "down.w"), B, waves=self.down_waves_small, **down,
                                 resident=(i, "down") in self.resident, **self._w8kw(p + "down.w"))
            pending = defer
        return x

    def _spec_args(self) -> Spec:
        t, sp = self.cfg.text, self.spec
        return Spec(self.B, self.K, self.rows, int(sp.ngram_min), int(sp.ngram_max), self.s_max, ptr(self.d_prompt_ids),
                    self.d_prompt_ids.stride(0), ptr(self.d_hist), self.d_hist.stride(0), self.d_hist.shape[0], ptr(self.d_script),
                    ptr(self.d_script_len), ptr(self.d_row_slot), ptr(self.d_ctx), ptr(self.d_plen), ptr(self.d_fin), ptr(self.d_temp),
                    ptr(self.d_seed), ptr(self.d_ndraft), ptr(self.d_draft), ptr(self.w.view("llm.embed")), t.hidden_size,
                    self.cfg.pad_token_id, t.vocab_size, ptr(self.d_x), self.d_x.stride(0), ptr(self.d_spec_count[0]),
                    ptr(self.d_spec_count[1]))

    def _spec_refusal(self) -> Optional[str]:
        step = self._step
        if self.spec is None:
            return "the engine was built without speculative=SpecConfig(...)"
        if not self._freeze_finished:
            return "speculative steps run in slot mode (begin_slots)"
        controlled = (step.processing or step.adjust) and not self.spec_controls
        if self.spec_guided:
            if controlled:
                return "the step carries sampling controls or logit adjustments"
        elif step.guided or controlled:
            return ("the step carries guided decoding, sampling controls or logit adjustments"
                    + (" (guided requests speculate on an engine built with SpecConfig(guided=True))" if step.guided else ""))
        if self._logprobs is not None:
            return "log-probabilities are recorded"
        return None

    def _spec_step_launches(self):
        L, s, R = self.L, self.s, self.rows
        why = self._spec_refusal()
        if why is not None:
            raise KarantaHipError("speculative decode step refused: " + why)
        step = self._step
        a = self._spec_args()
        g = self.sampler.spec_guide_args() if step.guided else None
        c = self.sampler.spec_controls_args() if (step.processing or step.adjust) else None
        if self.share_rows:
            L.kr_spec_lookup(C.byref(a), ptr(self.d_nwant), s)
            if g is not None:
                L.kr_spec_guide_trim(C.byref(a), C.byref(g), ptr(self.d_nwant), s)
            if c is not None:
                L.kr_spec_controls_trim(C.byref(a), C.byref(c), ptr(self.d_nwant), s)
            L.kr_spec_deal(C.byref(a), ptr(self.d_nwant), ptr(self.d_draft_row), s)
            if g is not None:
                L.kr_spec_guide_rows(C.byref(a), C.byref(g), ptr(self.d_draft_row), s)
            if c is not None:
                L.kr_spec_controls_rows(C.byref(a), C.byref(c), ptr(self.d_draft_row), s)
        else:
            L.kr_spec_propose(C.byref(a), s)
            if g is not None:
                L.kr_spec_guide_trim(C.byref(a), C.byref(g), ptr(self.d_ndraft), s)
            if c is not None:
                L.kr_spec_controls_trim(C.byref(a), C.byref(c), ptr(self.d_ndraft), s)
            if g is not None:
                L.kr_spec_guide_rows(C.byref(a), C.byref(g), None, s)
            if c is not None:
                L.kr_spec_controls_rows(C.byref(a), C.byref(c), None, s)
        x = self._layer_launches(R, self.d_row_slot)
        logits, n_part = self._lm_head(R, x)
        flags = self._flags()
        n_part = self.sampler.pre_token(logits, n_part, R, 0, flags, spec=True)
        if self.share_rows:
            L.kr_spec_accept_rows(C.byref(a), ptr(self.d_draft_row), ptr(self.d_amax_v), ptr(self.d_amax_i), n_part, ptr(self.d_tok),
                                  ptr(self.d_eos), self.d_eos.numel(), flags, s)
        else:
            L.kr_spec_accept(C.byref(a), ptr(self.d_amax_v), ptr(self.d_amax_i), n_part, ptr(self.d_tok), ptr(self.d_eos),
                             self.d_eos.numel(), flags, s)
        if step.adjust:
            sm = self.sampler
            L.kr_stop_tokens(ptr(self.d_tok), ptr(sm.d_adj_ids), ptr(sm.d_adj_flag), ptr(sm.d_adj_meta), ptr(self.d_fin), flags,
                             self.B, s)
        if step.processing:
            L.kr_spec_controls_count(C.byref(a), C.byref(c), s)
        if g is not None:
            L.kr_spec_guide_advance(C.byref(a), C.byref(g), s)
        if self._step.repetition:
            self.sampler.repeat_pass(self.B, 0, flags)

    def set_draft_script(self, slot: int, tokens: Optional[Sequence[int]]):
        if self.spec is None:
            raise KarantaHipError("set_draft_script: the engine was built without speculative=SpecConfig(...)")
# ... 458 lines not shown
```

Before: 6.258 pages/s.

## Feed narrow decode GEMMs from a 16-row packed activation layout

Adds an xp16 packed activation layout for batches of 16 or fewer. The attention merge and the gate_up SiLU epilogue now write their outputs directly in this layout, and the narrow o_proj and down_proj kernels read x fragments from it through a new template mode. The aim is contiguous, coalesced fragment loads of activations in place of per-row strided loads in the decode GEMMs. It adds an extra template dimension, new buffers and an ABI bump, and it only applies when defer_down is on, narrow mode is used and kv8 is off.

```diff
diff --git a/include/karanta_hip.h b/include/karanta_hip.h
--- a/include/karanta_hip.h
+++ b/include/karanta_hip.h
@@ -11,7 +11,7 @@
 typedef void* kr_stream;
 typedef uint16_t kr_bf16;
 
-#define KR_ABI_VERSION 412
+#define KR_ABI_VERSION 500
 
 #define KR_OK 0
 #define KR_ERR_ARG (-1)
@@ -137,6 +137,7 @@
 #define KR_DEC_ARGMAX 3
 #define KR_DEC_SILU8 4
 #define KR_DEC_OUT_XP 0x100
+#define KR_DEC_OUT_XP16 0x200
 int kr_linear_decode(int mode, const kr_bf16* x, int64_t ldx, const kr_bf16* w_packed, const kr_bf16* bias,
                      const kr_bf16* norm_w, float norm_eps, const kr_bf16* residual, int64_t ldr,
                      kr_bf16* out, float* out_f32, int64_t ldc, int M, int N, int K, int waves, int max_blocks, int ksplit,
@@ -156,6 +157,7 @@
     int32_t atomic_out;
     int32_t part_rows;
     int32_t w_resident;
+    int32_t x_packed;
 } kr_narrow_opts;
 
 int kr_linear_decode_narrow(int mode, const kr_bf16* x, int64_t ldx, const float* part_in, int n_part_in,
@@ -223,6 +225,9 @@
                          kr_stream s);
 
 int kr_attn_decode_merge32(const float* workspace, kr_bf16* out_xp, int batch, int heads, int hd, int n_split,
+                           kr_stream s);
+
+int kr_attn_decode_merge16(const float* workspace, kr_bf16* out_xp16, int batch, int heads, int hd, int n_split,
                            kr_stream s);
 
 int kr_image_resize_bicubic_u8(const uint8_t* src, int h, int w, uint8_t* dst, int rh, int rw, uint8_t* tmp,
diff --git a/karanta_ocr_amd/_lib.py b/karanta_ocr_amd/_lib.py
--- a/karanta_ocr_amd/_lib.py
+++ b/karanta_ocr_amd/_lib.py
@@ -43,6 +43,7 @@
     "kr_pack_rows32": [c_p, i64, i32, i32, c_p, c_p],
     "kr_linear_decode32": [i32, c_p, c_p],
     "kr_attn_decode_merge32": [c_p, c_p, i32, i32, i32, i32, c_p],
+    "kr_attn_decode_merge16": [c_p, c_p, i32, i32, i32, i32, c_p],
     "kr_quantize_rows_fp8": [c_p, i64, c_p, i64, c_p, i64, i32, c_p],
     "kr_gemm_fp8a": [c_p, i64, c_p, c_p, c_p, c_p, c_p, i64, c_p, i64, i64, i32, i32, i32, c_p],
     "kr_gemm_bf16_ws": [c_p, i64, c_p, c_p, c_p, i64, c_p, i64, i64, i32, i32, i32, i32, c_p, C.c_size_t, c_p],
@@ -143,10 +144,16 @@
                 ("w_resident", C.c_int32)]
 
 
-def narrow_opts(zero_ptr: int = 0, zero_bytes: int = 0, atomic_out: bool = False, part_rows: int = 0, w_resident: bool = False):
-    if not (zero_bytes or atomic_out or part_rows or w_resident):
+class NarrowOptsXP(C.Structure):
+    _fields_ = NarrowOpts._fields_ + [("x_packed", C.c_int32)]
+
+
+def narrow_opts(zero_ptr: int = 0, zero_bytes: int = 0, atomic_out: bool = False, part_rows: int = 0, w_resident: bool = False,
+                x_packed: bool = False):
+    if not (zero_bytes or atomic_out or part_rows or w_resident or x_packed):
         return None
-    return C.byref(NarrowOpts(zero_ptr or None, int(zero_bytes), 1 if atomic_out else 0, int(part_rows), 1 if w_resident else 0))
+    head = (zero_ptr or None, int(zero_bytes), 1 if atomic_out else 0, int(part_rows), 1 if w_resident else 0)
+    return C.byref(NarrowOptsXP(*head, 1) if x_packed else NarrowOpts(*head))
 
 class Dec32(C.Structure):
     _fields_ = [("xp", c_p), ("w_packed", c_p), ("w_scale", c_p), ("bias", c_p), ("residual", c_p), ("ldr", C.c_int64),
@@ -230,8 +237,9 @@
     return C.byref(p)
 
 
-ABI_MAJOR = 4
+ABI_MAJOR = 5
 DEC_OUT_XP = 0x100
+DEC_OUT_XP16 = 0x200
 ADJ_CAP = 320
 EPI_NONE, EPI_QUICK_GELU, EPI_GELU_ERF, EPI_SILU_MUL, EPI_SILU_MUL8 = 0, 1, 2, 3, 4
 DEC_PLAIN, DEC_SILU, DEC_ROPE_KV, DEC_ARGMAX, DEC_SILU8 = 0, 1, 2, 3, 4
diff --git a/karanta_ocr_amd/csrc/kr_attn_decode.hip b/karanta_ocr_amd/csrc/kr_attn_decode.hip
--- a/karanta_ocr_amd/csrc/kr_attn_decode.hip
+++ b/karanta_ocr_amd/csrc/kr_attn_decode.hip
@@ -296,7 +296,8 @@
 }
 
 template <int NS>
-__global__ void __launch_bounds__(128) attn_merge_kernel(const float* __restrict__ ws, kr_bf16* __restrict__ out, int n_split, int heads_xp) {
+__global__ void __launch_bounds__(128) attn_merge_kernel(const float* __restrict__ ws, kr_bf16* __restrict__ out, int n_split, int heads_xp,
+                                                         int xp16) {
     constexpr int HD = 128, REC = HD + 4;
     const int bh = blockIdx.x, d = threadIdx.x;
     float acc = 0.f, ll = 0.f;
@@ -331,7 +332,7 @@
     const kr_bf16 r = __builtin_bit_cast(kr_bf16, f2bf(ll > 0.f ? acc / ll : 0.f));
     if (heads_xp > 0) {
         const int b = bh / heads_xp, hh = bh - b * heads_xp;
-        *reinterpret_cast<kr_bf16*>(reinterpret_cast<char*>(out) + kr_xp_byte_offset(b, hh * HD + d)) = r;
+        *reinterpret_cast<kr_bf16*>(reinterpret_cast<char*>(out) + (xp16 ? kr_xp16_byte_offset(b, hh * HD + d, xp16) : kr_xp_byte_offset(b, hh * HD + d))) = r;
     } else {
         out[(int64_t)bh * HD + d] = r;
     }
@@ -417,14 +418,15 @@
 static int merge_impl(const float* workspace, kr_bf16* out, int batch, int heads, int hd, int n_split, int xp, kr_stream s) {
     KR_CHECK_ARG(workspace && out && batch > 0 && heads > 0 && n_split > 0, "kr_attn_decode_merge: bad args");
     KR_CHECK_ARG(hd == 128, "kr_attn_decode_merge: hd=%d (only 128)", hd);
-    KR_CHECK_ARG(!xp || (batch <= 32 && ((uintptr_t)out & 15) == 0), "kr_attn_decode_merge32: batch=%d (<= 32)", batch);
-    const int hx = xp ? heads : 0;
+    KR_CHECK_ARG(!xp || (batch <= (xp == 2 ? 16 : 32) && ((uintptr_t)out & 15) == 0), "kr_attn_decode_merge%d: batch=%d (<= %d)",
+                 xp == 2 ? 16 : 32, batch, xp == 2 ? 16 : 32);
+    const int hx = xp ? heads : 0, xp16 = xp == 2 ? kr_xp16_rows(batch) : 0;
     switch (n_split) {
-        case 4: attn_merge_kernel<4><<<batch * heads, 128, 0, kr_hs(s)>>>(workspace, out, n_split, hx); break;
-        case 8: attn_merge_kernel<8><<<batch * heads, 128, 0, kr_hs(s)>>>(workspace, out, n_split, hx); break;
-        case 16: attn_merge_kernel<16><<<batch * heads, 128, 0, kr_hs(s)>>>(workspace, out, n_split, hx); break;
-        case 32: attn_merge_kernel<32><<<batch * heads, 128, 0, kr_hs(s)>>>(workspace, out, n_split, hx); break;
-        default: attn_merge_kernel<0><<<batch * heads, 128, 0, kr_hs(s)>>>(workspace, out, n_split, hx);
+        case 4: attn_merge_kernel<4><<<batch * heads, 128, 0, kr_hs(s)>>>(workspace, out, n_split, hx, xp16); break;
+        case 8: attn_merge_kernel<8><<<batch * heads, 128, 0, kr_hs(s)>>>(workspace, out, n_split, hx, xp16); break;
+        case 16: attn_merge_kernel<16><<<batch * heads, 128, 0, kr_hs(s)>>>(workspace, out, n_split, hx, xp16); break;
+        case 32: attn_merge_kernel<32><<<batch * heads, 128, 0, kr_hs(s)>>>(workspace, out, n_split, hx, xp16); break;
+        default: attn_merge_kernel<0><<<batch * heads, 128, 0, kr_hs(s)>>>(workspace, out, n_split, hx, xp16);
     }
     KR_CHECK_LAUNCH();
     return KR_OK;
@@ -438,6 +440,11 @@
 extern "C" int kr_attn_decode_merge32(const float* workspace, kr_bf16* out_xp, int batch, int heads, int hd, int n_split,
                                       kr_stream s) {
     return merge_impl(workspace, out_xp, batch, heads, hd, n_split, 1, s);
+}
+
+extern "C" int kr_attn_decode_merge16(const float* workspace, kr_bf16* out_xp16, int batch, int heads, int hd, int n_split,
+                                      kr_stream s) {
+    return merge_impl(workspace, out_xp16, batch, heads, hd, n_split, 2, s);
 }
 
 namespace {
diff --git a/karanta_ocr_amd/csrc/kr_common.h b/karanta_ocr_amd/csrc/kr_common.h
--- a/karanta_ocr_amd/csrc/kr_common.h
+++ b/karanta_ocr_amd/csrc/kr_common.h
@@ -75,6 +75,10 @@
 __host__ __device__ __forceinline__ int64_t kr_xp_byte_offset(int b, int k) {
     return (int64_t)(k >> 6) * 4096 + (b >> 4) * 2048 + ((k >> 5) & 1) * 1024 + ((((k >> 3) & 3) * 16 + (b & 15)) * 16) + (k & 7) * 2;
 }
+__host__ __device__ __forceinline__ int kr_xp16_rows(int M) { return M <= 8 ? 8 : 16; }
+__host__ __device__ __forceinline__ int64_t kr_xp16_byte_offset(int b, int k, int R) {
+    return (int64_t)(k >> 6) * (R * 128) + ((k >> 5) & 1) * (R * 64) + ((((k >> 3) & 3) * R + b) * 16) + (k & 7) * 2;
+}
 
 __host__ __device__ __forceinline__ int kr_vt_off(int d, int key, int hd) { return ((key >> 5) * hd + d) * 32 + (key & 31); }
 
diff --git a/karanta_ocr_amd/csrc/kr_decode.hip b/karanta_ocr_amd/csrc/kr_decode.hip
--- a/karanta_ocr_amd/csrc/kr_decode.hip
+++ b/karanta_ocr_amd/csrc/kr_decode.hip
@@ -33,6 +33,7 @@
     float* zero_ptr; int zero_n16;
     int w_resident;
     int out_xp;
+    int x_packed;
     Kv8 kv8;
 };
 
@@ -592,8 +593,9 @@
                     bf16x4 o;
 #pragma unroll
                     for (int j = 0; j < 4; ++j) o[j] = f2bf(act_silu(acc[mt][j]) * u4[j]);
-                    if (MT == 2 && a.out_xp)
-                        *reinterpret_cast<bf16x4*>(reinterpret_cast<char*>(a.out) + kr_xp_byte_offset(b, t * 8 + fg * 4)) = o;
+                    if (a.out_xp)
+                        *reinterpret_cast<bf16x4*>(reinterpret_cast<char*>(a.out) + (MT == 2 ? kr_xp_byte_offset(b, t * 8 + fg * 4)
+                                                                                             : kr_xp16_byte_offset(b, t * 8 + fg * 4, kr_xp16_rows(M)))) = o;
                     else
                         *reinterpret_cast<bf16x4*>(a.out + (int64_t)b * a.ldc + t * 8 + fg * 4) = o;
                 }
@@ -936,12 +938,13 @@
     }
 }
 
+enum NarrowX { NARROW_X_ROWS = 0, NARROW_X_PACKED = 1, NARROW_X_BOUND = 2 };
 template <int NCH> struct NarrowCfg { static constexpr int RL = 8; };
 template <> struct NarrowCfg<24> { static constexpr int RL = 3; };
 template <> struct NarrowCfg<32> { static constexpr int RL = 4; };
 template <> struct NarrowCfg<56> { static constexpr int RL = 7; };
 
-template <int NT, int EPI, int WAVES, int NCH, int PKS, bool NORM, int U, bool W8, int MT, bool RES>
+template <int NT, int EPI, int WAVES, int NCH, int PKS, bool NORM, int U, bool W8, int MT, bool RES, int XM>
 __global__ void __launch_bounds__(WAVES * 64) dec_narrow_kernel(const kr_bf16* hx, const kr_bf16* hwp, const kr_bf16* hnorm_w, const float* hpart_in,
                                                                 int64_t hldx, int hM, int hN, int hK, int hcpb, float hnorm_eps,
                                                                 int hprows, const DecLinArgs a) {
@@ -1001,6 +1004,15 @@
     const char* xg[MT];
 #pragma unroll
     for (int mt = 0; mt < MT; ++mt) xg[mt] = reinterpret_cast<const char*>(hx + (int64_t)rb[mt] * hldx);
+    auto xfrag = [&](const int mt, const int c, const int h) {
+        if constexpr (XM == NARROW_X_BOUND)
+            return *reinterpret_cast<const bf16x8*>(reinterpret_cast<const char*>(hx) + cb0 * 128 + WC::x_byte(h, fg));
+        else if constexpr (XM == NARROW_X_PACKED)
+            return *reinterpret_cast<const bf16x8*>(reinterpret_cast<const char*>(hx) + c * ((int)hldx * 128) +
+                                                    WC::xp16_off(h, fr & ((int)hldx - 1), fg, (int)hldx));
+        else
+            return *reinterpret_cast<const bf16x8*>(xg[mt] + c * 128 + WC::x_byte(h, fg));
+    };
     if (NORM) {
         const int b = wave < M ? wave : 0;
 #pragma unroll
@@ -1023,8 +1035,8 @@
             const int c = min(max(min(c0 + u, c1 - 1), cb0), nchunks - 1);
 #pragma unroll
             for (int mt = 0; mt < MT; ++mt) {
-                xf[u][mt][0] = *reinterpret_cast<const bf16x8*>(xg[mt] + c * 128 + WC::x_byte(0, fg));
-                xf[u][mt][1] = *reinterpret_cast<const bf16x8*>(xg[mt] + c * 128 + WC::x_byte(1, fg));
+                xf[u][mt][0] = xfrag(mt, c, 0);
+                xf[u][mt][1] = xfrag(mt, c, 1);
             }
         }
     }
@@ -1210,8 +1222,8 @@
                     if (!NORM) {
 #pragma unroll
                         for (int mt = 0; mt < MT; ++mt) {
-                            xf[u][mt][0] = *reinterpret_cast<const bf16x8*>(xg[mt] + cn * 128 + WC::x_byte(0, fg));
-                            xf[u][mt][1] = *reinterpret_cast<const bf16x8*>(xg[mt] + cn * 128 + WC::x_byte(1, fg));
+                            xf[u][mt][0] = xfrag(mt, cn, 0);
+                            xf[u][mt][1] = xfrag(mt, cn, 1);
                         }
                     }
 #pragma unroll
@@ -1333,13 +1345,13 @@
     }
 }
 
-template <int NT, int EPI, int WAVES, int NCH, int PKS, bool NORM, int U, bool W8, int MT, bool RES>
+template <int NT, int EPI, int WAVES, int NCH, int PKS, bool NORM, int U, bool W8, int MT, bool RES, int XM>
 int launch_narrow_m(DecLinArgs& a, int groups, kr_stream s) {
     const int nchunks = a.K >> 6, cpb = (nchunks + a.ksplit - 1) / a.ksplit;
     const size_t xbytes = NORM ? (((size_t)a.M * (cpb * 128 + 16) + 127) & ~(size_t)127) : 0;
     const size_t lds = xbytes + (size_t)WAVES * NT * 256 * 4;
     KR_CHECK_ARG(lds <= 160 * 1024, "kr_linear_decode_narrow: M=%d K=%d needs %zu bytes of LDS", a.M, a.K, lds);
-    auto fn = &dec_narrow_kernel<NT, EPI, WAVES, NCH, PKS, NORM, U, W8, MT, RES>;
+    auto fn = &dec_narrow_kernel<NT, EPI, WAVES, NCH, PKS, NORM, U, W8, MT, RES, XM>;
     static KrPerDeviceOnce attr;
     if (attr.need()) {
         KR_CHECK_HIP(hipFuncSetAttribute(reinterpret_cast<const void*>(fn), hipFuncAttributeMaxDynamicSharedMemorySize, 160 * 1024));
@@ -1351,26 +1363,29 @@
     return KR_OK;
 }
 
-template <int NT, int EPI, int WAVES, int NCH, int PKS, bool NORM, int U, bool W8, bool RES>
+template <int NT, int EPI, int WAVES, int NCH, int PKS, bool NORM, int U, bool W8, bool RES, int XM>
 int launch_narrow_w(DecLinArgs& a, int groups, kr_stream s) {
     if (a.M > 16) {
-        if constexpr (WAVES == 8 && NCH != 56) {
-            return launch_narrow_m<NT, EPI, WAVES, NCH, PKS, NORM, U, W8, 2, RES>(a, groups, s);
+        if constexpr (XM != NARROW_X_ROWS) {
+            kr_set_error("kr_linear_decode_narrow: opts x_packed takes M <= 16 (M=%d)", a.M);
+            return KR_ERR_ARG;
+        } else if constexpr (WAVES == 8 && NCH != 56) {
+            return launch_narrow_m<NT, EPI, WAVES, NCH, PKS, NORM, U, W8, 2, RES, XM>(a, groups, s);
         } else {
             kr_set_error("kr_linear_decode_narrow: M=%d > 16 needs 8-wave workgroups and K != 3584", a.M);
             return KR_ERR_ARG;
         }
     }
-    return launch_narrow_m<NT, EPI, WAVES, NCH, PKS, NORM, U, W8, 1, RES>(a, groups, s);
-}
-
-template <int NT, int EPI, int WAVES, int NCH, int PKS, bool NORM, int U>
+    return launch_narrow_m<NT, EPI, WAVES, NCH, PKS, NORM, U, W8, 1, RES, XM>(a, groups, s);
+}
+
+template <int NT, int EPI, int WAVES, int NCH, int PKS, bool NORM, int U, int XM = NARROW_X_ROWS>
 int launch_narrow_u(DecLinArgs& a, int groups, kr_stream s) {
     if (a.w_resident)
-        return a.w_scale ? launch_narrow_w<NT, EPI, WAVES, NCH, PKS, NORM, U, true, true>(a, groups, s)
-                         : launch_narrow_w<NT, EPI, WAVES, NCH, PKS, NORM, U, false, true>(a, groups, s);
-    return a.w_scale ? launch_narrow_w<NT, EPI, WAVES, NCH, PKS, NORM, U, true, false>(a, groups, s)
-                     : launch_narrow_w<NT, EPI, WAVES, NCH, PKS, NORM, U, false, false>(a, groups, s);
+        return a.w_scale ? launch_narrow_w<NT, EPI, WAVES, NCH, PKS, NORM, U, true, true, XM>(a, groups, s)
+                         : launch_narrow_w<NT, EPI, WAVES, NCH, PKS, NORM, U, false, true, XM>(a, groups, s);
+    return a.w_scale ? launch_narrow_w<NT, EPI, WAVES, NCH, PKS, NORM, U, true, false, XM>(a, groups, s)
+                     : launch_narrow_w<NT, EPI, WAVES, NCH, PKS, NORM, U, false, false, XM>(a, groups, s);
 }
 
 inline int narrow_share(const DecLinArgs& a, int waves) {
@@ -1378,24 +1393,36 @@
     return (cpb + waves - 1) / waves;
 }
 
-template <int EPI, int WAVES>
+template <int EPI, int WAVES, int XM>
 int launch_narrow_direct(DecLinArgs& a, int groups, kr_stream s) {
     const int share = narrow_share(a, WAVES);
     if constexpr (EPI == DEPI_PARTIAL) {
         const char* e = getenv("KARANTA_NARROW_NT2");
         const bool nt2 = e ? atoi(e) != 0 : groups >= 192;
         if (nt2 && (groups & 1) == 0 && (a.M <= 16 || WAVES == 8)) {
-            if constexpr (WAVES == 16) return launch_narrow_u<2, EPI, WAVES, 0, 0, false, 3>(a, groups / 2, s);
-            else return launch_narrow_u<2, EPI, WAVES, 0, 0, false, 5>(a, groups / 2, s);
-        }
-    }
-    if (share <= 3) return launch_narrow_u<1, EPI, WAVES, 0, 0, false, 3>(a, groups, s);
+            if constexpr (WAVES == 16) return launch_narrow_u<2, EPI, WAVES, 0, 0, false, 3, XM>(a, groups / 2, s);
+            else return launch_narrow_u<2, EPI, WAVES, 0, 0, false, 5, XM>(a, groups / 2, s);
+        }
+    }
+    if (share <= 3) return launch_narrow_u<1, EPI, WAVES, 0, 0, false, 3, XM>(a, groups, s);
     if constexpr (WAVES == 16) {
-        return launch_narrow_u<1, EPI, WAVES, 0, 0, false, 5>(a, groups, s);
+        return launch_narrow_u<1, EPI, WAVES, 0, 0, false, 5, XM>(a, groups, s);
     } else {
-        if (share <= 5) return launch_narrow_u<1, EPI, WAVES, 0, 0, false, 5>(a, groups, s);
-        return launch_narrow_u<1, EPI, WAVES, 0, 0, false, 8>(a, groups, s);
-    }
+        if (share <= 5) return launch_narrow_u<1, EPI, WAVES, 0, 0, false, 5, XM>(a, groups, s);
+        return launch_narrow_u<1, EPI, WAVES, 0, 0, false, 8, XM>(a, groups, s);
+    }
+}
+
+template <int EPI>
+int launch_narrow_direct_w(DecLinArgs& a, int groups, int waves, kr_stream s) {
+#ifdef KR_NARROW_XBOUND
+    const char* e = getenv("KARANTA_NARROW_XBOUND");
+    if (e && atoi(e) != 0)
+        return waves == 16 ? launch_narrow_direct<EPI, 16, NARROW_X_BOUND>(a, groups, s) : launch_narrow_direct<EPI, 8, NARROW_X_BOUND>(a, groups, s);
+#endif
+    if (a.x_packed)
+        return waves == 16 ? launch_narrow_direct<EPI, 16, NARROW_X_PACKED>(a, groups, s) : launch_narrow_direct<EPI, 8, NARROW_X_PACKED>(a, groups, s);
+    return waves == 16 ? launch_narrow_direct<EPI, 16, NARROW_X_ROWS>(a, groups, s) : launch_narrow_direct<EPI, 8, NARROW_X_ROWS>(a, groups, s);
 }
 
 template <int NT, int EPI, int NCH, int PKS>
@@ -1658,6 +1685,11 @@
                      "kr_linear_decode_wide: KR_DEC_OUT_XP is for SILU8 at 17..32 rows, N/2 %% 64 == 0");
         a.out_xp = 1;
         mode &= ~KR_DEC_OUT_XP;
+    } else if (mode & KR_DEC_OUT_XP16) {
+        KR_CHECK_ARG((mode & ~KR_DEC_OUT_XP16) == DEPI_SILU8 && M <= 16 && (N / 2) % 64 == 0 && ((uintptr_t)out & 15) == 0,
+                     "kr_linear_decode_wide: KR_DEC_OUT_XP16 is for SILU8 at <= 16 rows, N/2 %% 64 == 0");
+        a.out_xp = 2;
+        mode &= ~KR_DEC_OUT_XP16;
     }
     switch (mode) {
         case DEPI_PLAIN:
@@ -1726,6 +1758,10 @@
     a.n_part = part_in ? n_part_in : 0;
     a.zero_ptr = o.zero_bytes ? o.zero_ptr : nullptr; a.zero_n16 = (int)(o.zero_bytes >> 4); a.part_atomic = o.atomic_out ? 1 : 0;
     a.w_resident = o.w_resident ? 1 : 0;
+    a.x_packed = o.x_packed ? 1 : 0;
+    if (a.x_packed) a.ldx = kr_xp16_rows(M);
+    KR_CHECK_ARG(!a.x_packed || (mode == DEPI_PLAIN && !norm_w && M <= 16 && ((uintptr_t)x & 15) == 0),
+                 "kr_linear_decode_narrow: opts x_packed is for PLAIN launches without a norm prologue at M <= 16 (x 16-byte aligned)");
     KR_CHECK_ARG(!a.part_atomic || (ksplit == 2 && mode == DEPI_PLAIN), "kr_linear_decode_narrow: atomic_out is for ksplit 2 (order-free sum)");
     KR_CHECK_ARG(a.part_rows == 0 || (part_in && a.part_rows >= M), "kr_linear_decode_narrow: part rows %d < M %d", a.part_rows, M);
     if (KR_EXP && pf_blocks > 0) {
@@ -1742,13 +1778,11 @@
             if (ksplit > 1) {
                 KR_CHECK_ARG(out_f32 && !out && !bias && !residual && !norm_w,
                              "kr_linear_decode_narrow: split-K writes f32 slabs only (no bias / residual / norm)");
-                return waves == 16 ? launch_narrow_direct<DEPI_PARTIAL, 16>(a, ntiles, s)
-                                   : launch_narrow_direct<DEPI_PARTIAL, 8>(a, ntiles, s);
+                return launch_narrow_direct_w<DEPI_PARTIAL>(a, ntiles, waves, s);
             }
             KR_CHECK_ARG(out || out_f32, "kr_linear_decode_narrow: PLAIN output");
             if (norm_w) return launch_narrow_norm<1, DEPI_PLAIN>(a, ntiles, s);
-            return waves == 16 ? launch_narrow_direct<DEPI_PLAIN, 16>(a, ntiles, s)
-                               : launch_narrow_direct<DEPI_PLAIN, 8>(a, ntiles, s);
+            return launch_narrow_direct_w<DEPI_PLAIN>(a, ntiles, waves, s);
         case DEPI_ROPE_KV:
             if (kv8) {
                 KR_CHECK_ARG(bias && cs_table && prompt_len && ctx_len && q_out && kv8->k && kv8->vt && kv8->scale && cs_stride > 0 && norm_w,
diff --git a/karanta_ocr_amd/csrc/kr_decode_common.h b/karanta_ocr_amd/csrc/kr_decode_common.h
--- a/karanta_ocr_amd/csrc/kr_decode_common.h
+++ b/karanta_ocr_amd/csrc/kr_decode_common.h
@@ -24,6 +24,7 @@
     __device__ __forceinline__ bf16x8 frag(int h) const { return v[h]; }
     static __device__ __forceinline__ int x_byte(int h, int fg) { return h * 64 + fg * 16; }
     static __device__ __forceinline__ int xp_off(int h, int fr, int fg) { return h * 1024 + (fg * 16 + fr) * 16; }
+    static __device__ __forceinline__ int xp16_off(int h, int fr, int fg, int R) { return h * (R * 64) + (fg * R + fr) * 16; }
 };
 template <> struct WChunk<true> {
     static constexpr int BYTES = 1024;
@@ -44,6 +45,9 @@
     }
     static __device__ __forceinline__ int x_byte(int h, int fg) { return fg * 32 + h * 16; }
     static __device__ __forceinline__ int xp_off(int h, int fr, int fg) { return (fg >> 1) * 1024 + ((((fg & 1) << 1) | h) * 16 + fr) * 16; }
+    static __device__ __forceinline__ int xp16_off(int h, int fr, int fg, int R) {
+        return (fg >> 1) * (R * 64) + ((((fg & 1) << 1) | h) * R + fr) * 16;
+    }
 };
 
 __device__ __forceinline__ void apply_w_scale(const float* w_scale, int n, f32x4& acc) {
diff --git a/karanta_ocr_amd/engine.py b/karanta_ocr_amd/engine.py
--- a/karanta_ocr_amd/engine.py
+++ b/karanta_ocr_amd/engine.py
@@ -11,7 +11,7 @@
 
 from . import image_processing as IP
 from . import positions as POS
-from ._lib import (DEC_ARGMAX, DEC_OUT_XP, DEC_PLAIN, DEC_ROPE_KV, DEC_SILU8, Dec32, EPI_NONE, EPI_SILU_MUL8, KarantaHipError, Spec, lib,
+from ._lib import (DEC_ARGMAX, DEC_OUT_XP, DEC_OUT_XP16, DEC_PLAIN, DEC_ROPE_KV, DEC_SILU8, Dec32, EPI_NONE, EPI_SILU_MUL8, KarantaHipError, Spec, lib,
                    narrow_opts, ptr)
 from . import kv_cache
 from .config import ModelConfig
@@ -206,6 +206,10 @@
             if v_:
                 setattr(self, "wv_" + name, int(v_))
         self.defer_down = t.hidden_size in (1536, 2048, 3584)
+        self.narrow_xp = self.defer_down and self.narrow_mode and not self.kv8
+        if self.narrow_xp:
+            self.d_o_xp = z(16, t.q_dim)
+            self.d_act_xp = z(16, t.intermediate_size)
         self.wide_mode = t.hidden_size % 512 == 0 and t.hidden_size <= 4096
         self.wide_blocks = int(os.environ.get("KARANTA_WIDE_BLOCKS", "256"))
         self.wide_waves = int(os.environ.get("KARANTA_WIDE_WAVES", "0"))
@@ -323,7 +327,7 @@
 
     def _dec_narrow(self, mode, x, W, M, out=None, out_f32=None, bias=None, norm_w=None, res=None, waves=8, ksplit=1,
                     part_in=None, x_out=None, kc=0, vc=0, w8=None, w_scale=None, zero=None, atomic_out=False,
-                    resident=False, kv8=None):
+                    resident=False, kv8=None, x_packed=False):
         t = self.cfg.text
         N, K = W.shape
         o = out if out is not None else out_f32
@@ -340,7 +344,8 @@
         args = (ptr(bias), ptr(norm_w), t.rms_norm_eps, ptr(res), res.stride(0) if res is not None else 0, ptr(out),
                 ptr(out_f32), o.stride(-2) if o is not None else 0, M, N, K, waves, ksplit, ptr(self.d_cs), self.max_new,
                 ptr(self.d_plen), ptr(self.d_ctx), ptr(self.d_q), kc, vc, t.num_heads, t.num_kv_heads, self.s_max,
-                narrow_opts(ptr(zero), zero.numel() * 4 if zero is not None else 0, atomic_out, w_resident=resident), self.s)
+                narrow_opts(ptr(zero), zero.numel() * 4 if zero is not None else 0, atomic_out, w_resident=resident,
+                            x_packed=x_packed), self.s)
         if w8 is not None:
             self.L.kr_linear_decode_narrow_fp8(*head, ptr(w8), ptr(w_scale), *args)
         else:
@@ -620,11 +625,11 @@
     def _decode_step_launches(self, B: int):
         self._lm_head_and_sample(B, self._layer_launches(B))
 
-    def _gate_up(self, x, i: int, B: int, out_xp: bool = False):
+    def _gate_up(self, x, i: int, B: int, out_xp: bool = False, out_xp16: bool = False):
         w, p = self.w, f"llm.{i}."
         if self.wide_mode:
-            self._dec_wide(DEC_SILU8 | (DEC_OUT_XP if out_xp else 0), x, w.view(p + "gate_up.w"), B, out=self.d_act,
-                           norm_w=w.view(p + "ln2.w"), **self._w8kw(p + "gate_up.w"))
+            self._dec_wide(DEC_SILU8 | (DEC_OUT_XP if out_xp else DEC_OUT_XP16 if out_xp16 else 0), x, w.view(p + "gate_up.w"), B,
+                           out=self.d_act_xp if out_xp16 else self.d_act, norm_w=w.view(p + "ln2.w"), **self._w8kw(p + "gate_up.w"))
         else:
             self._dec(DEC_SILU8, x, w.view(p + "gate_up.w"), B, out=self.d_act, norm_w=w.view(p + "ln2.w"), waves=self.wv_wide)
 
@@ -633,6 +638,7 @@
         H, hd = t.num_heads, t.head_dim
         nl = t.num_layers
         big = B > 16
+        xp16 = not big and self.narrow_xp
         x, x_other = self.d_x, self.d_x2
         pending = False
         slabs = self.d_part.view(-1)[: 2 * B * t.hidden_size].view(2, B, t.hidden_size)
@@ -659,17 +665,20 @@
             if pending:
                 x, x_other = x_other, x
             self.kv.attention(i, B, row_slot)
-            (L.kr_attn_decode_merge32 if big else L.kr_attn_decode_merge)(ptr(self.d_ws), ptr(self.d_o), B, H, hd, self.n_split, s)
+            if xp16:
+                L.kr_attn_decode_merge16(ptr(self.d_ws), ptr(self.d_o_xp), B, H, hd, self.n_split, s)
+            else:
+                (L.kr_attn_decode_merge32 if big else L.kr_attn_decode_merge)(ptr(self.d_ws), ptr(self.d_o), B, H, hd, self.n_split, s)
             if big:
                 self._dec32(DEC_PLAIN, self.d_o, w.view(p + "o.w"), B, self.o_waves, out=x, res=x, **self._w8kw(p + "o.w"))
             else:
-                self._dec_narrow(DEC_PLAIN, self.d_o, w.view(p + "o.w"), B, out=x, res=x, waves=self.o_waves,
-                                 resident=(i, "o") in self.resident, **self._w8kw(p + "o.w"))
+                self._dec_narrow(DEC_PLAIN, self.d_o_xp if xp16 else self.d_o, w.view(p + "o.w"), B, out=x, res=x, waves=self.o_waves,
+                                 resident=(i, "o") in self.resident, x_packed=xp16, **self._w8kw(p + "o.w"))
             if self._prof_on:
                 (e0, e1), (e2, _) = self._prof_event_pair(), self._prof_event_pair()
                 L.kr_event_record(e0, s)
                 L.kr_event_record(e1, s)
-            self._gate_up(x, i, B, out_xp=big)
+            self._gate_up(x, i, B, out_xp=big, out_xp16=xp16)
             if self._prof_on:
                 L.kr_event_record(e2, s)
             down = dict(ksplit=2, out_f32=acc, atomic_out=True) if defer else dict(out=x, res=x)
@@ -679,8 +688,9 @@
             elif big:
                 self._dec32(DEC_PLAIN, self.d_act, w.view(p + "down.w"), B, self.down_waves_small, **down, **self._w8kw(p + "down.w"))
             else:
-                self._dec_narrow(DEC_PLAIN, self.d_act, w.view(p + "down.w"), B, waves=self.down_waves_small, **down,
-                                 resident=(i, "down") in self.resident, **self._w8kw(p + "down.w"))
+                self._dec_narrow(DEC_PLAIN, self.d_act_xp if xp16 else self.d_act, w.view(p + "down.w"), B,
+                                 waves=self.down_waves_small, **down, resident=(i, "down") in self.resident, x_packed=xp16,
+                                 **self._w8kw(p + "down.w"))
             pending = defer
         return x
 
```

New measurement: 6.359 pages/s, median of 6. 1.02x the previous value.
